# nipponjo/tts-arabic-pytorch

Hardware: AMD Instinct MI355X
Metric: audio samples/sec (FastPitch+HiFi-GAN, synthetic 64-phoneme inputs) (higher is better)
Workload: dtype f32

## Files before the change

include/ttsamd.h:

```cpp
#ifndef TTSAMD_H
#define TTSAMD_H

#include <stdint.h>

#ifdef __cplusplus
extern "C" {
#endif

#define TTSAMD_OK 0
#define TTSAMD_EINVAL (-1)
#define TTSAMD_EHIP (-2)
#define TTSAMD_ENOMEM (-3)

typedef struct ttsamd_tensor {
    const char* name;
    const float* data;
    int32_t ndim;
    int64_t shape[4];
} ttsamd_tensor;

typedef struct ttsamd_hifigan_cfg {
    int32_t num_mels;
    int32_t upsample_initial_channel;
    int32_t n_ups;
// ... 121 lines not shown
                       int32_t batch, int32_t n_max, const float* bias_spec, float strength,
                       void* workspace, int64_t workspace_bytes, void* stream);
int32_t ttsamd_denoise_rows(void* handle, float* wave, int64_t wave_stride, const int64_t* nsamples,
                            int32_t batch, int32_t n_max, const float* bias_spec, const float* strength_rows,
                            void* workspace, int64_t workspace_bytes, void* stream);

int32_t ttsamd_vocos_create(const ttsamd_tensor* weights, int32_t n_weights, int32_t input_channels,
                            int32_t dim, int32_t intermediate_dim, int32_t num_layers, void** handle);
int32_t ttsamd_vocos_destroy(void* handle);
int64_t ttsamd_vocos_workspace_bytes(void* handle, int32_t batch, int32_t t_max);
int32_t ttsamd_vocos_bias_vec(void* handle, float* bias_vec, void* workspace, int64_t workspace_bytes,
                              void* stream);
int32_t ttsamd_vocos_forward(void* handle, const float* mel, const int64_t* lens, int32_t batch,
                             int32_t t_max, float denoise, const float* bias_vec, float* wave,
                             void* workspace, int64_t workspace_bytes, void* stream);
int32_t ttsamd_vocos_forward_rows(void* handle, const float* mel, const int64_t* lens, int32_t batch,
                                  int32_t t_max, const float* denoise_rows, const float* bias_vec, float* wave,
                                  void* workspace, int64_t workspace_bytes, void* stream);

int32_t ttsamd_vocos_set_padding(void* handle, int32_t mode);

int32_t ttsamd_melspec_create(const float* fbank, int32_t n_mels, int32_t n_fft, int32_t hop_length, int32_t framing,
                              int32_t mag_mode, float log_clip, void** handle);
int32_t ttsamd_melspec_destroy(void* handle);
int32_t ttsamd_melspec_forward(void* handle, const float* wave, int64_t wave_stride, const int64_t* nsamples, int32_t batch,
                               int32_t t_max, float* mel, int64_t* frames_out, void* stream);

#define TTSAMD_OVERSMOOTH_MAX_FRAMES 4096
int32_t ttsamd_cepstral_series(const float* mel, const int64_t* lens, int32_t batch, int32_t n_mels, int32_t t_max, int32_t center,
                               int32_t hann, int32_t q_c, float hqer_scale, float* power, float* series, void* stream);
int32_t ttsamd_cepstral_series_from_power(const float* power, const int64_t* lens, int32_t batch, int32_t n_q, int32_t t_max, int32_t q_c,
                                          int32_t q1, int32_t q2, double eps, double roll_p, float hqer_scale, float* series,
                                          void* stream);
int32_t ttsamd_series_summary(const float* series, const int64_t* lens, int32_t batch, int32_t n_series, int32_t t_max, float* stats,
                              float* feat, void* stream);
int64_t ttsamd_dtw_workspace_bytes(int32_t batch, int32_t ta_max, int32_t tb_max, int32_t channels);
int32_t ttsamd_dtw(const float* a, const int64_t* lens_a, const float* b, const int64_t* lens_b, int32_t batch, int32_t channels,
                   int32_t ta_max, int32_t tb_max, int32_t metric, int32_t window, float* cost, int32_t* path, int32_t* path_len,
                   void* workspace, int64_t workspace_bytes, void* stream);
int32_t ttsamd_dtw_aligned_mae(const float* pred, const float* ref, int32_t batch, int32_t ta_max, int32_t tb_max, const int32_t* path,
                               const int32_t* path_len, float* mae, void* stream);

int32_t ttsamd_mel_cepstrum(const float* logmel, const int64_t* lens, int32_t batch, int32_t n_mels, int32_t t_max, int32_t n_coef, float* cep,
                            void* stream);
#define TTSAMD_EVAL_STATS 8
int32_t ttsamd_dtw_aligned_eval(const float* cep_a, const float* cep_b, int32_t n_coef, int32_t first_coef, const float* mel_a,
                                const float* mel_b, int32_t n_mels, const float* f0_a, const float* f0_b, int32_t batch, int32_t ta_max,
                                int32_t tb_max, const int32_t* path, const int32_t* path_len, double scale, double* stats, void* stream);

#define TTSAMD_MAS_MAX_TOKENS 1024
typedef struct ttsamd_aligner_cfg {
    int32_t n_mel;
    int32_t d_text;
    int32_t n_att;
    int32_t n_symbols;
    int32_t padding_idx;
} ttsamd_aligner_cfg;
int32_t ttsamd_aligner_create(const ttsamd_tensor* weights, int32_t n_weights, const ttsamd_aligner_cfg* cfg, void** handle);
int32_t ttsamd_aligner_destroy(void* handle);
int64_t ttsamd_aligner_workspace_bytes(void* handle, int32_t batch, int32_t n_tokens, int32_t n_frames);
int32_t ttsamd_aligner_forward(void* handle, const int64_t* ids, const int64_t* in_lens, const float* mel, const int64_t* mel_lens,
                               const float* attn_prior, int32_t batch, int32_t n_tokens, int32_t n_frames, float* attn_soft,
                               float* attn_logprob, void* workspace, int64_t workspace_bytes, void* stream);
int64_t ttsamd_mas_workspace_bytes(int32_t batch, int32_t n_frames, int32_t n_tokens);
int32_t ttsamd_mas(const float* attn, int32_t is_log, const int64_t* in_lens, const int64_t* out_lens, int32_t batch, int32_t n_frames,
                   int32_t n_tokens, float* dur, float* attn_hard, void* workspace, int64_t workspace_bytes, void* stream);
int32_t ttsamd_average_pitch(const float* pitch, const float* dur, int32_t batch, int32_t n_formants, int32_t n_frames, int32_t n_tokens,
                             float* out, void* stream);

#define TTSAMD_ATTN_PRIOR_F64 2
int32_t ttsamd_attn_prior(const int64_t* in_lens, const int64_t* mel_lens, int32_t batch, int32_t n_tokens, int32_t n_frames, int32_t mode,
                          double scaling, void* out, void* stream);
int32_t ttsamd_attn_prior_tables(int32_t n, double* lf);
int64_t ttsamd_attn_ctc_loss_workspace_bytes(int32_t batch, int32_t n_frames, int32_t n_tokens);
int32_t ttsamd_attn_ctc_loss(const float* attn_logprob, const int64_t* in_lens, const int64_t* out_lens, int32_t batch, int32_t n_frames,
                             int32_t n_tokens, double blank_logprob, double* nll, void* workspace, int64_t workspace_bytes, void* stream);
int32_t ttsamd_attn_bin_loss(const float* attn_hard, const float* attn_soft, int32_t batch, int32_t n_frames, int32_t n_tokens, double eps,
                             double* sum_log, double* count, void* stream);

#define TTSAMD_PYIN_MAX_FRAMES 8192
typedef struct ttsamd_pyin_cfg {
    int32_t sample_rate;
    int32_t frame_length;
    int32_t win_length;
    int32_t hop_length;
    double fmin, fmax;
    int32_t n_thresholds;
    int32_t beta_a, beta_b;
    double boltzmann;
    double resolution;
    double max_transition_rate;
    double switch_prob;
    double no_trough_prob;
    int32_t pad_mode;
} ttsamd_pyin_cfg;
int32_t ttsamd_pyin_tables(const ttsamd_pyin_cfg* cfg, int32_t* dims, double* beta, double* expn, double* norm, double* trans,
                           float* logtrans, float* f0);
int32_t ttsamd_pyin_create(const ttsamd_pyin_cfg* cfg, void** handle);
int32_t ttsamd_pyin_destroy(void* handle);
int64_t ttsamd_pyin_workspace_bytes(void* handle, int32_t batch, int32_t n_frames);
int32_t ttsamd_pyin_forward(void* handle, const float* wave, int64_t wave_stride, const int64_t* nsamples, int32_t batch, int32_t t_max,
                            float* f0, uint8_t* voiced_flag, double* voiced_prob, int32_t* states, int64_t* frames_out,
                            void* workspace, int64_t workspace_bytes, void* stream);
int32_t ttsamd_pyin_obs_offsets(void* handle, int32_t batch, int32_t n_frames, int64_t* obs_offsets);

int32_t ttsamd_resample_create(const float* taps, int32_t o, int32_t n, int32_t width, void** handle);
int32_t ttsamd_resample_destroy(void* handle);
int64_t ttsamd_resample_out_len(void* handle, int64_t nsamples);
int32_t ttsamd_resample_mfma_eligible(void* handle);
int32_t ttsamd_resample_forward(void* handle, const float* wave, int64_t wave_stride, const int64_t* nsamples, int32_t batch, float* out,
                                int64_t out_stride, int64_t* nout, int32_t route, void* stream);

int64_t ttsamd_trim_workspace_bytes(int32_t batch, int64_t wave_stride, int32_t hop_length);
int32_t ttsamd_trim_bounds(const float* wave, int64_t wave_stride, const int64_t* nsamples, int32_t batch, float top_db,
                           int32_t frame_length, int32_t hop_length, float gain, int64_t* bounds, float* peak, void* workspace,
                           int64_t workspace_bytes, void* stream);
int32_t ttsamd_trim_apply(const float* wave, int64_t wave_stride, const int64_t* bounds, const float* peak, float gain, int64_t tail,
                          int32_t batch, float* out, int64_t out_stride, int64_t* lens_out, void* stream);
int32_t ttsamd_frames_compact(const float* mel, const float* extra, const int64_t* lens, int32_t batch, int32_t n_channels,
                              int32_t n_extra, int32_t t_max, float thresh, float* mel_out, float* extra_out, int64_t* lens_out,
                              void* stream);

int32_t ttsamd_tacotron2_create(const ttsamd_tensor* weights, int32_t n_weights,
                                const ttsamd_tacotron2_cfg* cfg, void** handle);
int32_t ttsamd_tacotron2_destroy(void* handle);
int64_t ttsamd_tacotron2_workspace_bytes(void* handle, int32_t batch, int32_t n_tokens, int32_t max_step);
int32_t ttsamd_tacotron2_infer(void* handle, const int64_t* tokens, const int64_t* lengths,
                               const int64_t* speaker_ids, int32_t batch, int32_t n_tokens, int32_t max_step,
                               int64_t dropout_seed, float* mel_post, int32_t* mel_lens, float* alignments,
                               float* mel_raw, int32_t* n_steps, void* workspace, int64_t workspace_bytes,
                               void* stream);

int32_t ttsamd_tagger_create(const ttsamd_tensor* weights, int32_t n_weights, const ttsamd_tagger_cfg* cfg,
                             void** handle);
int32_t ttsamd_tagger_destroy(void* handle);
int64_t ttsamd_tagger_workspace_bytes(void* handle, int32_t batch, int32_t n_chars);
int32_t ttsamd_tagger_forward(void* handle, const int64_t* ids, int32_t batch, int32_t n_chars, float* probs,
                              void* workspace, int64_t workspace_bytes, void* stream);


int64_t ttsamd_conv1d_packed_floats(int32_t cout, int32_t cin, int32_t k);
int32_t ttsamd_conv1d(const float* x, const float* w, const float* bias, const int64_t* lens,
                      int32_t batch, int32_t cin, int32_t cout, int32_t k, int32_t dilation,
                      int32_t lin, float in_slope, int32_t relu_out, float* y, float* packed,
                      void* stream);
int32_t ttsamd_conv1d_ex(const float* x, const float* w, const float* bias, const float* res, const int64_t* lens, int32_t batch,
                         int32_t cin, int32_t cout, int32_t k, int32_t dilation, int32_t lin, float in_slope,
                         int32_t relu_out, int32_t mode, float div, float* y, float* packed, void* stream);
int32_t ttsamd_conv1d_splitk(const float* x, const float* w, const float* bias, const float* res, const int64_t* lens, int32_t batch,
                             int32_t cin, int32_t cout, int32_t k, int32_t dilation, int32_t lin, float in_slope,
                             int32_t relu_out, int32_t mode, float div, float* y, float* packed, float* splitk_ws, int64_t splitk_floats,
                             void* stream);
int32_t ttsamd_conv_last_launch(int32_t* route, int32_t* ksplit);
int64_t ttsamd_convt_packed_floats(int32_t cin, int32_t cout, int32_t u);
int32_t ttsamd_conv_transpose1d(const float* x, const float* w, const float* bias, const int64_t* lens, int32_t batch, int32_t cin,
                                int32_t cout, int32_t u, int32_t lin, float in_slope, float* y, float* packed, void* stream);

int64_t ttsamd_resblock_pair_packed_floats(int32_t channels, int32_t k, int32_t variant);
int32_t ttsamd_resblock_pair(const float* x, float* y, const float* w1, const float* b1, const float* w2, const float* b2,
                             int32_t channels, int32_t k, int32_t dil, const int64_t* lens, int32_t len_mul, int32_t L,
                             int32_t batch, int32_t mode, float div, float slope, int32_t variant, float* packed, int64_t packed_floats,
                             void* stream);

int64_t ttsamd_resblock2_packed_floats(int32_t channels, int32_t k, int32_t variant);
int32_t ttsamd_resblock2(const float* x, float* y, const float* w1, const float* b1, const float* w2, const float* b2, int32_t channels,
                         int32_t k, int32_t dil1, int32_t dil2, const int64_t* lens, int32_t len_mul, int32_t L, int32_t batch, int32_t mode,
                         float div, float slope, int32_t variant, float* packed, int64_t packed_floats, void* stream);

int32_t ttsamd_bfo_pack(const float* x, int32_t batch, int32_t channels, int32_t len, float slope, void* out, void* stream);
int32_t ttsamd_bfo_unpack(const void* in, int32_t batch, int32_t channels, int32_t len, float slope, float* out, void* stream);
int64_t ttsamd_bfo_weight_elems(int32_t cout, int32_t cin, int32_t k, int32_t up);
int32_t ttsamd_bfo_pack_weight(const float* w, int32_t cout, int32_t cin, int32_t k, int32_t up, uint16_t* out);
int32_t ttsamd_bfo_conv1d(const void* x, const void* w_packed, const float* bias, const void* res, const void* sum_in,
                          const int64_t* lens, int32_t len_mul, int32_t batch, int32_t cin, int32_t cout, int32_t k,
                          int32_t dilation, int32_t up, int32_t len_in, int32_t mode, float div, float res_slope,
                          float out_slope, void* y, float* y_f32, const float* res_f32, void* stream);
int32_t ttsamd_bfo_resblock_pair(const void* x, const void* w1, const float* b1, const void* w2, const float* b2,
                                 const void* sum_in, const int64_t* lens, int32_t len_mul, int32_t batch, int32_t channels,
                                 int32_t k, int32_t dilation, int32_t len, int32_t mode, float div, float in_slope,
                                 float mid_slope, float out_slope, void* y, void* stream);
int32_t ttsamd_bfo_resblock_chain(const void* x, const void* const* w1, const float* const* b1, const void* const* w2,
                                  const float* const* b2, const int32_t* dilations, const void* sum_in, const int64_t* lens,
                                  int32_t len_mul, int32_t batch, int32_t channels, int32_t len, int32_t mode, float div,
                                  float in_slope, float mid_slope, float out_slope, void* y, void* stream, int32_t k);
int32_t ttsamd_bfo_conv_post(const void* x, const float* w, const float* bias, const int64_t* lens, int32_t len_mul,
                             int32_t batch, int32_t channels, int32_t len, float* wave, int64_t wave_stride, void* stream);

int32_t ttsamd_bfo3_pack(const float* x, int32_t batch, int32_t channels, int32_t len, float slope, void* out, void* stream);
int32_t ttsamd_bfo3_unpack(const void* in, int32_t batch, int32_t channels, int32_t len, float slope, float* out, void* stream);
int64_t ttsamd_bfo3_weight_elems(int32_t cout, int32_t cin, int32_t k, int32_t up);
int32_t ttsamd_bfo3_pack_weight(const float* w, int32_t cout, int32_t cin, int32_t k, int32_t up, uint16_t* out);
int32_t ttsamd_bfo3_conv1d(const void* x, const void* w_packed, const float* bias, const void* res, const void* sum_in,
                           const int64_t* lens, int32_t len_mul, int32_t batch, int32_t cin, int32_t cout, int32_t k,
                           int32_t dilation, int32_t up, int32_t len_in, int32_t mode, float div, float res_slope,
                           float out_slope, void* y, float* y_f32, const float* res_f32, void* stream);
int32_t ttsamd_bfo3_resblock_pair(const void* x, const void* w1, const float* b1, const void* w2, const float* b2,
                                  const void* sum_in, const int64_t* lens, int32_t len_mul, int32_t batch, int32_t channels,
                                  int32_t k, int32_t dilation, int32_t len, int32_t mode, float div, float in_slope,
                                  float mid_slope, float out_slope, void* y, void* stream);
int32_t ttsamd_bfo3_resblock_chain(const void* x, const void* const* w1, const float* const* b1, const void* const* w2,
                                   const float* const* b2, const int32_t* dilations, const void* sum_in, const int64_t* lens,
                                   int32_t len_mul, int32_t batch, int32_t channels, int32_t len, int32_t mode, float div,
                                   float in_slope, float mid_slope, float out_slope, void* y, void* stream);
int32_t ttsamd_bfo3_conv_post(const void* x, const float* w, const float* bias, const int64_t* lens, int32_t len_mul,
                              int32_t batch, int32_t channels, int32_t len, float* wave, int64_t wave_stride, void* stream);

int32_t ttsamd_set_precision(int32_t precision);
int32_t ttsamd_get_precision(void);

#define TTSAMD_DP_ID_BYTES 128
#define TTSAMD_DP_HIFIGAN 0
#define TTSAMD_DP_FASTPITCH 1
int32_t ttsamd_dp_unique_id(void* id128 );
int32_t ttsamd_dp_init(int32_t rank, int32_t world, const void* id128 , void** comm);
int32_t ttsamd_dp_destroy(void* comm);
int32_t ttsamd_dp_rank(void* comm);
int32_t ttsamd_dp_world(void* comm);
int32_t ttsamd_dp_broadcast(void* comm, void* buf, int64_t nbytes, int32_t root, void* stream);
int32_t ttsamd_dp_broadcast_weights(void* comm, int32_t kind, void* handle, int32_t root, void* stream);
int32_t ttsamd_dp_allgather(void* comm, const void* send, void* recv, int64_t nbytes_per_rank, void* stream);
int32_t ttsamd_dp_pack_audio(const float* wave, int64_t wave_stride, const int64_t* nsamples, int32_t batch,
                             int64_t n_max, float* packed, void* stream);
int32_t ttsamd_dp_gather_audio(void* comm, const float* packed, float* recv, const int64_t* counts,
                               const int64_t* offsets, int32_t root, void* stream);

int32_t ttsamd_hifigan_halo_frames(void* handle, int32_t* left , int32_t* right );
int32_t ttsamd_denoiser_halo_frames(void);
#define TTSAMD_STREAM_MAX_WINDOWS 64
int32_t ttsamd_stream_gather(const float* pool, int32_t n_slots, int32_t num_mels, int32_t t_cap, const int32_t* slot ,
                             const int32_t* start , const int32_t* len , int32_t n_windows, int32_t w_max,
                             float* batch, int64_t* lens, void* stream);
int32_t ttsamd_stream_emit(const float* wave, int32_t n_windows, int32_t w_max, int32_t hop, const int32_t* core_off ,
                           const int32_t* core_len , int32_t c_max, int32_t format, void* out, void* stream);
int32_t ttsamd_stream_emit_resampled(void* resample_handle, const float* wave, int32_t n_windows, int32_t w_max, int32_t hop,
                                     const int32_t* win_start , const int32_t* win_len ,
                                     const int32_t* utt_len , const int32_t* core_start ,
                                     const int32_t* core_end , int32_t c_max, int32_t format, void* out,
                                     int32_t* nout , void* stream);
int32_t ttsamd_vocos_halo_frames(void* handle, int32_t* left , int32_t* right );
int32_t ttsamd_vocos_forward_windows(void* handle, const float* mel, const int64_t* lens, int32_t n_windows, int32_t w_max,
                                     const int32_t* need_start , const int32_t* need_len ,
                                     const float* denoise_rows , const float* bias_vec, float* wave,
                                     void* workspace, int64_t workspace_bytes, void* stream);
int32_t ttsamd_wave_encode(const float* wave, int64_t wave_stride, const int64_t* nsamples, int32_t batch, int32_t format, void* out,
                           int64_t out_stride, void* stream);

int32_t ttsamd_loudness_coefficients(int32_t sample_rate, double* out);
int64_t ttsamd_loudness_workspace_bytes(int32_t batch, int64_t wave_stride, int32_t sample_rate);
int32_t ttsamd_loudness_measure(const float* wave, int64_t wave_stride, const int64_t* nsamples, int32_t batch, int32_t sample_rate,
                                double* loudness, float* peak, void* workspace, int64_t workspace_bytes, void* stream);
int32_t ttsamd_wave_level(float* wave, int64_t wave_stride, const int64_t* nsamples, int32_t batch, const int32_t* mode,
                          const float* target, float ceiling, const double* loudness, const float* peak, float* gain_out, void* stream);

int32_t ttsamd_profile_enable(int32_t on);
int32_t ttsamd_profile_read(double* out3);

#ifdef __cplusplus
}
#endif
#endif
```

profiles/launch_classes.py:

```python
import csv
import re
import sys
from collections import defaultdict


def classes(path):
    d = defaultdict(lambda: [0, 0])
    other = 0
    with open(path) as f:
        for r in csv.DictReader(f):
            dur = int(r['End_Timestamp']) - int(r['Start_Timestamp'])
            m = re.search(r'conv1d_wino4_f32<(\d+), (\d+), (\d+), (\d+), (\d+), (\d+)>', r['Kernel_Name'])
            if not m:
                other += dur
                continue
            k, noct, nst, epi, lp, pt = map(int, m.groups())
            key = (pt, k, lp, 'residual' if epi == 3 else 'plain', int(r['Grid_Size_X']) // int(r['Workgroup_Size_X']))
            d[key][0] += 1
            d[key][1] += dur
    return d, other


a, oa = classes(sys.argv[1])
b, ob = classes(sys.argv[2])
print(f'{"groups":>6} {"k":>3} {"window":>7} {"epilogue":>9} {"blocks":>7} {"calls":>6} {"us parent":>10} {"us tree":>9} {"ratio":>6}')
ta = tb = 0
for key in sorted(set(a) | set(b), key=lambda t: (-t[0], t[1], t[2], t[3], t[4])):
    ca, da = a.get(key, (0, 0))
    cb, db = b.get(key, (0, 0))
    ta += da
    tb += db
    ua, ub = (da / ca / 1e3 if ca else float('nan')), (db / cb / 1e3 if cb else float('nan'))
    print(f'{"seven" if key[0] == 7 else "six":>6} {key[1]:3d} {"vector" if key[2] == 1 else "strip":>7} {key[3]:>9} {key[4]:7d} {max(ca, cb):6d} '
          f'{ua:10.1f} {ub:9.1f} {ub / ua:6.3f}')
print(f'sum over the conv1d_wino4_f32 launches: {ta / 1e6:.2f} -> {tb / 1e6:.2f} ms; every other kernel: {oa / 1e6:.2f} -> {ob / 1e6:.2f} ms (whole trace)')
```

tts-arabic-pytorch_amd/csrc/api.hip:

```cpp
#include <cerrno>
#include <cstdio>
#include <cstdlib>
#include <cstring>
#include <algorithm>
#include <atomic>
#include <mutex>
#include <string>
#include <vector>

#include "kernels.hpp"

namespace ttsamd {

static thread_local std::string g_err;

void set_error(const char* fmt, ...) {
    char buf[1024];
    va_list ap;
    va_start(ap, fmt);
    vsnprintf(buf, sizeof(buf), fmt, ap);
    va_end(ap);
    g_err = buf;
}

// ... 49 lines not shown
struct Vocos;
int32_t vocos_create(const ttsamd_tensor*, int32_t, int32_t, int32_t, int32_t, int32_t, Vocos**);
void vocos_destroy(Vocos*);
int64_t vocos_workspace_bytes(const Vocos*, int32_t, int32_t);
int64_t vocos_bias_workspace_bytes(const Vocos*);
int32_t vocos_bias_vec(const Vocos*, float*, void*, int64_t, hipStream_t);
int32_t vocos_forward(const Vocos*, const float*, const int64_t*, int32_t, int32_t, float, const float*, const float*, float*, void*,
                      int64_t, hipStream_t);
int32_t vocos_set_padding(Vocos*, int32_t);
int32_t vocos_halo_frames(const Vocos*, int32_t*, int32_t*);
int32_t vocos_forward_windows(const Vocos*, const float*, const int64_t*, int32_t, int32_t, const int32_t*, const int32_t*, const float*,
                              const float*, float*, void*, int64_t, hipStream_t);
struct MelSpec;
int32_t melspec_create(const float*, int32_t, int32_t, int32_t, int32_t, int32_t, float, MelSpec**);
void melspec_destroy(MelSpec*);
int32_t melspec_forward(const MelSpec*, const float*, int64_t, const int64_t*, int32_t, int32_t, float*, int64_t*, hipStream_t);
int32_t cepstral_series(const float*, const int64_t*, int32_t, int32_t, int32_t, int32_t, int32_t, int32_t, float, float*, float*, hipStream_t);
int32_t cepstral_series_from_power(const float*, const int64_t*, int32_t, int32_t, int32_t, int32_t, int32_t, int32_t, double, double, float,
                                   float*, hipStream_t);
int32_t series_summary(const float*, const int64_t*, int32_t, int32_t, int32_t, float*, float*, hipStream_t);
int64_t dtw_workspace_bytes(int32_t, int32_t, int32_t, int32_t);
int32_t dtw(const float*, const int64_t*, const float*, const int64_t*, int32_t, int32_t, int32_t, int32_t, int32_t, int32_t, float*,
            int32_t*, int32_t*, void*, int64_t, hipStream_t);
int32_t dtw_aligned_mae(const float*, const float*, int32_t, int32_t, int32_t, const int32_t*, const int32_t*, float*, hipStream_t);
int32_t mel_cepstrum(const float*, const int64_t*, int32_t, int32_t, int32_t, int32_t, float*, hipStream_t);
int32_t dtw_aligned_eval(const float*, const float*, int32_t, int32_t, const float*, const float*, int32_t, const float*, const float*, int32_t,
                         int32_t, int32_t, const int32_t*, const int32_t*, double, double*, hipStream_t);
struct Aligner;
int32_t aligner_create(const ttsamd_tensor*, int32_t, const ttsamd_aligner_cfg*, Aligner**);
void aligner_destroy(Aligner*);
int64_t aligner_workspace_bytes(const Aligner*, int32_t, int32_t, int32_t);
int32_t aligner_forward(const Aligner*, const int64_t*, const int64_t*, const float*, const int64_t*, const float*, int32_t, int32_t, int32_t,
                        float*, float*, void*, int64_t, hipStream_t);
int64_t mas_workspace_bytes(int32_t, int32_t, int32_t);
int32_t mas(const float*, int32_t, const int64_t*, const int64_t*, int32_t, int32_t, int32_t, float*, float*, void*, int64_t, hipStream_t);
int32_t average_pitch(const float*, const float*, int32_t, int32_t, int32_t, int32_t, float*, hipStream_t);
int32_t attn_prior(const int64_t*, const int64_t*, int32_t, int32_t, int32_t, int32_t, double, void*, hipStream_t);
int32_t attn_prior_tables_host(int32_t, double*);
int64_t attn_ctc_workspace_bytes(int32_t, int32_t, int32_t);
int32_t attn_ctc_loss(const float*, const int64_t*, const int64_t*, int32_t, int32_t, int32_t, double, double*, void*, int64_t, hipStream_t);
int32_t attn_bin_loss(const float*, const float*, int32_t, int32_t, int32_t, double, double*, double*, hipStream_t);
struct Pyin;
int32_t pyin_tables_host(const ttsamd_pyin_cfg*, int32_t*, double*, double*, double*, double*, float*, float*);
int32_t pyin_create(const ttsamd_pyin_cfg*, Pyin**);
void pyin_destroy(Pyin*);
int64_t pyin_workspace_bytes(const Pyin*, int32_t, int32_t);
int32_t pyin_obs_offsets(const Pyin*, int32_t, int32_t, int64_t*);
int32_t pyin_forward(const Pyin*, const float*, int64_t, const int64_t*, int32_t, int32_t, float*, uint8_t*, double*, int32_t*, int64_t*, void*,
                     int64_t, hipStream_t);
struct Taco2;
int32_t tacotron2_create(const ttsamd_tensor*, int32_t, const ttsamd_tacotron2_cfg*, Taco2**);
void tacotron2_destroy(Taco2*);
int64_t tacotron2_workspace_bytes(const Taco2*, int32_t, int32_t, int32_t);
int32_t tacotron2_infer(const Taco2*, const int64_t*, const int64_t*, const int64_t*, int32_t, int32_t, int32_t, int64_t,
                        float*, int32_t*, float*, float*, int32_t*, void*, int64_t, hipStream_t);
struct Tagger;
int32_t tagger_create(const ttsamd_tensor*, int32_t, const ttsamd_tagger_cfg*, Tagger**);
void tagger_destroy(Tagger*);
int64_t tagger_workspace_bytes(const Tagger*, int32_t, int32_t);
int32_t tagger_forward(const Tagger*, const int64_t*, int32_t, int32_t, float*, void*, int64_t, hipStream_t);
int32_t denoiser_create(Denoiser**);
void denoiser_destroy(Denoiser*);
int64_t denoiser_workspace_bytes(int32_t, int32_t);
int32_t denoiser_bias_spec(const Denoiser*, const float*, const int64_t*, int32_t, float*, void*, int64_t, hipStream_t);
int32_t denoise(const Denoiser*, float*, int64_t, const int64_t*, int32_t, int32_t, const float*, float, const float*, void*, int64_t,
                hipStream_t);
int32_t hifigan_halo_frames(const HifiGan*, int32_t*, int32_t*);
int32_t stream_gather(const float*, int32_t, int32_t, int32_t, const int32_t*, const int32_t*, const int32_t*, int32_t, int32_t, float*,
                      int64_t*, hipStream_t);
int32_t stream_emit(const float*, int32_t, int32_t, int32_t, const int32_t*, const int32_t*, int32_t, int32_t, void*, hipStream_t);
int32_t stream_emit_resampled(const Resample*, const float*, int32_t, int32_t, int32_t, const int32_t*, const int32_t*, const int32_t*,
                              const int32_t*, const int32_t*, int32_t, int32_t, void*, int32_t*, hipStream_t);
int32_t wave_encode(const float*, int64_t, const int64_t*, int32_t, int32_t, void*, int64_t, hipStream_t);
int32_t hifigan_create(const ttsamd_tensor*, int32_t, const ttsamd_hifigan_cfg*, HifiGan**);
void hifigan_destroy(HifiGan*);
int64_t hifigan_workspace_bytes(const HifiGan*, int32_t, int32_t);
int32_t hifigan_forward(const HifiGan*, const float*, const int64_t*, int32_t, int32_t, float*, void*, int64_t,
                        hipStream_t);
int32_t fastpitch_create(const ttsamd_tensor*, int32_t, const ttsamd_fastpitch_cfg*, int32_t, FastPitch**);
void fastpitch_destroy(FastPitch*);
int64_t fastpitch_encode_workspace_bytes(const FastPitch*, int32_t, int32_t);
int64_t fastpitch_decode_workspace_bytes(const FastPitch*, int32_t, int32_t);
int32_t fastpitch_encode(const FastPitch*, const int64_t*, int32_t, int32_t, int32_t, float, const float*,
                         const float*, const float*, float, float, float, float*, float*, float*, float*, int64_t*,
                         int64_t*, void*, int64_t, hipStream_t);
void fastpitch_set_batch_mode(const FastPitch*, int);
int32_t fastpitch_decode(const FastPitch*, float*, const int64_t*, int32_t, int32_t, float*, void*, int64_t,
                         hipStream_t);
int32_t fastpitch_encode_rows(const FastPitch*, const int64_t*, int32_t, int32_t, int32_t, float, const float*,
                              const float*, const float*, float, float, float, float*, float*, float*, float*, int64_t*,
                              int64_t*, void*, int64_t, const int32_t*, const float*, const float*, const float*, int32_t, hipStream_t);
int32_t fastpitch_decode_rows(const FastPitch*, float*, const int64_t*, int32_t, int32_t, float*, void*, int64_t, int32_t,
                              hipStream_t);

__global__ void pack_conv_weight_kernel(const float* __restrict__ w, int cout, int cin, int k, int cp,
                                        float* __restrict__ out) {
    const int64_t i = (int64_t)blockIdx.x * 256 + threadIdx.x;
    const int64_t n = (int64_t)cin * k * cp;
    if (i >= n) return;
    const int pq = (int)(i % 4);
    const int co = (int)((i / 4) % cp);
    const int kk = (int)((i / (4 * (int64_t)cp)) % 2);
    const int t = (int)((i / (8 * (int64_t)cp)) % k);
    const int o = (int)(i / (8 * (int64_t)cp * k));
    out[i] = co < cout ? w[((int64_t)co * cin + (8 * o + 2 * pq + kk)) * k + t] : 0.f;
}

__global__ void pack_convt_weight_kernel(const float* __restrict__ w, int cin, int cout, int u, int cp, float* __restrict__ out) {
    const int64_t i = (int64_t)blockIdx.x * 256 + threadIdx.x;
    const int64_t n = (int64_t)u * cin * 2 * cp;
    if (i >= n) return;
    const int pq = (int)(i % 4);
    const int co = (int)((i / 4) % cp);
    const int kk = (int)((i / (4 * (int64_t)cp)) % 2);
    const int t = (int)((i / (8 * (int64_t)cp)) % 2);
    const int o = (int)((i / (16 * (int64_t)cp)) % (cin / 8));
    const int rho = (int)(i / (16 * (int64_t)cp * (cin / 8)));
    const int kidx = (rho + u / 2) % u + t * u;
    out[i] = co < cout ? w[((int64_t)(8 * o + 2 * pq + kk) * cout + co) * (2 * u) + kidx] : 0.f;
}

__global__ void split_bf16_kernel(const float* __restrict__ packed, int64_t n, unsigned short* __restrict__ out) {
    const int64_t i = (int64_t)blockIdx.x * 256 + threadIdx.x;
    if (i >= n) return;
    const float f = packed[i];
    unsigned u = __float_as_uint(f);
    u += 0x7fffu + ((u >> 16) & 1u);
    const unsigned h = u >> 16;
    const float r = f - __uint_as_float(h << 16);
    unsigned v = __float_as_uint(r);
    v += 0x7fffu + ((v >> 16) & 1u);
    out[i] = (unsigned short)h;
    out[n + i] = (unsigned short)(v >> 16);
}

namespace {
struct OptDesc { const char* name; int kind; long long lo, hi; };
const OptDesc kOpts[OPT_COUNT] = {
#define TTS_OPT_DESC(name, kind, lo, hi) {"TTSAMD_" #name, kind, lo, hi},
    TTS_OPTIONS(TTS_OPT_DESC)
#undef TTS_OPT_DESC
};
std::atomic<const char*> g_opt[OPT_COUNT];
std::once_flag g_opt_once;
std::string g_opt_env_error;

bool opt_valid(const OptDesc& d, const char* v) {
    if (!v || !*v) return false;
    char* end = nullptr;
    errno = 0;
    const long long x = std::strtoll(v, &end, d.kind == 1 ? 16 : 10);
    if (!(errno == 0 && end != v && *end == '\0' && x >= d.lo && x <= d.hi)) return false;
    if (&d == &kOpts[OPT_WINO4] && (((x & 32) && !(x & 2)) || ((x & 64) && !(x & 4)))) return false;
    return true;
}
void opt_init() {
    std::call_once(g_opt_once, [] {
        for (int i = 0; i < OPT_COUNT; ++i) {
            const char* e = std::getenv(kOpts[i].name);
            if (!e || !*e) continue;
            if (!opt_valid(kOpts[i], e)) {
                if (g_opt_env_error.empty()) {
                    char buf[256];
                    std::snprintf(buf, sizeof buf, "%s='%s' in the environment is not a valid value (%s in [%llx, %llx])", kOpts[i].name, e,
                                  kOpts[i].kind == 1 ? "hex mask" : "integer", kOpts[i].lo, kOpts[i].hi);
                    g_opt_env_error = buf;
                }
                continue;
            }
            g_opt[i].store(strdup(e), std::memory_order_release);
        }
    });
}
int opt_find(const char* name) {
    if (!name) return -1;
    for (int i = 0; i < OPT_COUNT; ++i)
        if (std::strcmp(name, kOpts[i].name) == 0 || std::strcmp(name, kOpts[i].name + 7) == 0) return i;
    return -1;
}
}

int64_t opt_int(Opt o, int64_t unset) {
    opt_init();
    const char* v = g_opt[o].load(std::memory_order_acquire);
    return v ? (int64_t)std::strtoll(v, nullptr, kOpts[o].kind == 1 ? 16 : 10) : unset;
}

}

using namespace ttsamd;

extern "C" {

const char* ttsamd_last_error(void) { return g_err.c_str(); }
int32_t ttsamd_version(void) { return TTSAMD_ABI_VERSION; }

int32_t ttsamd_set_option(const char* name, const char* value) {
    opt_init();
    const int i = opt_find(name);
    TTS_REQUIRE(i >= 0, "set_option: unknown option '%s' (ttsamd_option_name lists them)", name ? name : "(null)");
    if (!value || !*value) {
        g_opt[i].store(nullptr, std::memory_order_release);
        return 0;
    }
    TTS_REQUIRE(opt_valid(kOpts[i], value), "set_option: %s='%s' is not a valid value (%s in [%llx, %llx])", kOpts[i].name, value,
                kOpts[i].kind == 1 ? "hex mask" : "integer", kOpts[i].lo, kOpts[i].hi);
    g_opt[i].store(strdup(value), std::memory_order_release);
    return 0;
}
int32_t ttsamd_get_option(const char* name, char* value, int32_t capacity) {
    opt_init();
    const int i = opt_find(name);
    TTS_REQUIRE(i >= 0 && value && capacity > 0, "get_option: unknown option '%s' or no buffer", name ? name : "(null)");
    const char* v = g_opt[i].load(std::memory_order_acquire);
    std::snprintf(value, (size_t)capacity, "%s", v ? v : "");
    return 0;
}
const char* ttsamd_option_name(int32_t index) { return (index >= 0 && index < OPT_COUNT) ? kOpts[index].name : nullptr; }
int32_t ttsamd_options_check(void) {
    opt_init();
    TTS_REQUIRE(g_opt_env_error.empty(), "%s", g_opt_env_error.c_str());
    return 0;
}

int32_t ttsamd_device_ok(void) {
    int n = 0;
    if (hipGetDeviceCount(&n) != hipSuccess || n <= 0) return 0;
    hipDeviceProp_t prop;
    if (hipGetDeviceProperties(&prop, 0) != hipSuccess) return 0;
    return std::string(prop.gcnArchName).rfind("gfx950", 0) == 0 ? 1 : 0;
}

int32_t ttsamd_hifigan_create(const ttsamd_tensor* weights, int32_t n, const ttsamd_hifigan_cfg* cfg, void** handle) {
    HifiGan* h = nullptr;
    const int32_t rc = hifigan_create(weights, n, cfg, &h);
    if (rc == 0) *handle = h;
    return rc;
}
int32_t ttsamd_hifigan_destroy(void* handle) {
    hifigan_destroy((HifiGan*)handle);
    return 0;
}
int64_t ttsamd_hifigan_workspace_bytes(void* handle, int32_t batch, int32_t t_max) {
    if (!handle || batch < 1 || t_max < 1) return 0;
    return hifigan_workspace_bytes((HifiGan*)handle, batch, t_max);
}
int32_t ttsamd_hifigan_forward(void* handle, const float* mel, const int64_t* lens, int32_t batch, int32_t t_max,
                               float* wave, void* workspace, int64_t workspace_bytes, void* stream) {
    return hifigan_forward((HifiGan*)handle, mel, lens, batch, t_max, wave, workspace, workspace_bytes,
                           (hipStream_t)stream);
}

int32_t ttsamd_hifigan_halo_frames(void* handle, int32_t* left, int32_t* right) {
    return hifigan_halo_frames((HifiGan*)handle, left, right);
}
int32_t ttsamd_denoiser_halo_frames(void) { return 3; }
int32_t ttsamd_stream_gather(const float* pool, int32_t n_slots, int32_t num_mels, int32_t t_cap, const int32_t* slot, const int32_t* start,
                             const int32_t* len, int32_t n_windows, int32_t w_max, float* batch, int64_t* lens, void* stream) {
    return stream_gather(pool, n_slots, num_mels, t_cap, slot, start, len, n_windows, w_max, batch, lens, (hipStream_t)stream);
}
int32_t ttsamd_stream_emit(const float* wave, int32_t n_windows, int32_t w_max, int32_t hop, const int32_t* core_off, const int32_t* core_len,
                           int32_t c_max, int32_t format, void* out, void* stream) {
    return stream_emit(wave, n_windows, w_max, hop, core_off, core_len, c_max, format, out, (hipStream_t)stream);
}
int32_t ttsamd_stream_emit_resampled(void* resample_handle, const float* wave, int32_t n_windows, int32_t w_max, int32_t hop,
                                     const int32_t* win_start, const int32_t* win_len, const int32_t* utt_len, const int32_t* core_start,
                                     const int32_t* core_end, int32_t c_max, int32_t format, void* out, int32_t* nout, void* stream) {
    return stream_emit_resampled((const Resample*)resample_handle, wave, n_windows, w_max, hop, win_start, win_len, utt_len, core_start,
                                 core_end, c_max, format, out, nout, (hipStream_t)stream);
}
int32_t ttsamd_wave_encode(const float* wave, int64_t wave_stride, const int64_t* nsamples, int32_t batch, int32_t format, void* out,
                           int64_t out_stride, void* stream) {
    return wave_encode(wave, wave_stride, nsamples, batch, format, out, out_stride, (hipStream_t)stream);
}

int32_t ttsamd_fastpitch_create(const ttsamd_tensor* weights, int32_t n, const ttsamd_fastpitch_cfg* cfg,
                                void** handle) {
    FastPitch* h = nullptr;
    const int32_t rc = fastpitch_create(weights, n, cfg, 16384, &h);
    if (rc == 0) *handle = h;
    return rc;
}
int32_t ttsamd_fastpitch_destroy(void* handle) {
    fastpitch_destroy((FastPitch*)handle);
    return 0;
}
int64_t ttsamd_fastpitch_encode_workspace_bytes(void* handle, int32_t batch, int32_t n_tokens) {
    if (!handle || batch < 1 || n_tokens < 1) return 0;
    return fastpitch_encode_workspace_bytes((FastPitch*)handle, batch, n_tokens);
}
int64_t ttsamd_fastpitch_decode_workspace_bytes(void* handle, int32_t batch, int32_t t_max) {
    if (!handle || batch < 1 || t_max < 1) return 0;
    return fastpitch_decode_workspace_bytes((FastPitch*)handle, batch, t_max);
}
int32_t ttsamd_fastpitch_encode(void* handle, const int64_t* ids, int32_t batch, int32_t n_tokens, int32_t speaker,
                                float pace, const float* dur_tgt, const float* pitch_tgt, const float* energy_tgt,
                                float pitch_mul, float pitch_add, float max_duration, float* enc_cond,
                                float* dur_pred, float* pitch_pred, float* energy_pred, int64_t* reps,
                                int64_t* dec_lens, void* workspace, int64_t workspace_bytes, void* stream) {
    return fastpitch_encode((FastPitch*)handle, ids, batch, n_tokens, speaker, pace, dur_tgt, pitch_tgt, energy_tgt,
                            pitch_mul, pitch_add, max_duration, enc_cond, dur_pred, pitch_pred, energy_pred, reps,
                            dec_lens, workspace, workspace_bytes, (hipStream_t)stream);
}
int32_t ttsamd_length_regulate(const float* enc, const int64_t* reps, int32_t batch, int32_t n_tokens,
                               int32_t channels, int32_t t_max, float* out, int32_t* idx, void* stream) {
    TTS_REQUIRE(enc && reps && out && batch >= 1 && n_tokens >= 1 && channels >= 1 && t_max >= 0,
// ... 325 lines not shown
    const int ng = k == 3 ? 6 : (k == 7 ? 16 : 24), nsf = k == 3 ? 1 : (k == 7 ? 2 : 4);
    const int64_t i = (int64_t)blockIdx.x * 256 + threadIdx.x;
    const int64_t n = (int64_t)cin * ng * cp;
    if (i >= n) return;
    const int pq = (int)(i & 3);
    const int64_t r = i >> 2;
    const int co = (int)(r % cp);
    const int64_t r2 = r / cp;
    const int kk = (int)(r2 & 1);
    const int64_t r3 = r2 >> 1;
    const int t = (int)(r3 % ng), o = (int)(r3 / ng);
    float v = 0.f;
    if (co < cout) {
        const float* g = w + ((int64_t)co * cin + (8 * o + 2 * pq + kk)) * k;
        if (t < 6 * nsf) {
            const int s = t / 6, j = t % 6;
            const double g0 = g[3 * s], g1 = 3 * s + 1 < k ? g[3 * s + 1] : 0.0, g2 = 3 * s + 2 < k ? g[3 * s + 2] : 0.0;
            v = j == 0 ? (float)(g0 / 4) : (j == 1 ? (float)(-(g0 + g1 + g2) / 6) : (j == 2 ? (float)(-(g0 - g1 + g2) / 6) :
                (j == 3 ? (float)(g0 / 24 + g1 / 12 + g2 / 6) : (j == 4 ? (float)(g0 / 24 - g1 / 12 + g2 / 6) : (float)g2))));
        } else {
            v = g[6];
        }
    }
    out[i] = v;
}

__global__ void pack_wino44_weight_kernel(const float* __restrict__ w, int cout, int cin, int k, int cp, float* __restrict__ out) {
    const int ng = k == 7 ? 13 : 20;
    const int64_t i = (int64_t)blockIdx.x * 256 + threadIdx.x;
    const int64_t n = (int64_t)cin * ng * cp;
    if (i >= n) return;
    const int pq = (int)(i & 3);
    const int64_t r = i >> 2;
    const int co = (int)(r % cp);
    const int64_t r2 = r / cp;
    const int kk = (int)(r2 & 1);
    const int64_t r3 = r2 >> 1;
    const int t = (int)(r3 % ng), o = (int)(r3 / ng);
    float v = 0.f;
    if (co < cout) {
        const float* g = w + ((int64_t)co * cin + (8 * o + 2 * pq + kk)) * k;
        const int s = t / 7, j = t % 7;
        const double g0 = g[4 * s], g1 = g[4 * s + 1], g2 = g[4 * s + 2], g3 = 4 * s + 3 < k ? g[4 * s + 3] : 0.0;
        v = j == 0 ? (float)(g0 / 4) : (j == 1 ? (float)((g0 + g1 + g2 + g3) / 6) : (j == 2 ? (float)((g0 - g1 + g2 - g3) / 18) :
            (j == 3 ? (float)((g0 + 2 * g1 + 4 * g2 + 8 * g3) / 72) : (j == 4 ? (float)((g0 - 2 * g1 + 4 * g2 - 8 * g3) / 120) :
            (j == 5 ? (float)((32 * g0 + 16 * g1 + 8 * g2 + 4 * g3) / 45) : (float)(g3 / 2))))));
    }
    out[i] = v;
}

__global__ void pack_wino2_weight_kernel(const float* __restrict__ w, int cout, int cin, int k, int cp, float* __restrict__ out) {
    const int ns = k / 3, ng = 4 * ns + 2 * (k - 3 * ns);
    const int64_t i = (int64_t)blockIdx.x * 256 + threadIdx.x;
    const int64_t n = (int64_t)cin * ng * cp;
    if (i >= n) return;
    const int pq = (int)(i & 3);
    const int64_t r = i >> 2;
    const int co = (int)(r % cp);
    const int64_t r2 = r / cp;
    const int kk = (int)(r2 & 1);
    const int64_t r3 = r2 >> 1;
    const int t = (int)(r3 % ng), o = (int)(r3 / ng);
    float v = 0.f;
    if (co < cout) {
        const float* g = w + ((int64_t)co * cin + (8 * o + 2 * pq + kk)) * k;
        if (t < 4 * ns) {
            const int s = t >> 2, j = t & 3;
            const double g0 = g[3 * s], g1 = g[3 * s + 1], g2 = g[3 * s + 2];
            v = j == 0 ? (float)g0 : (j == 1 ? (float)((g0 + g1 + g2) * 0.5) : (j == 2 ? (float)((g0 - g1 + g2) * 0.5) : (float)g2));
        } else {
            const int l = (t - 4 * ns) >> 1;
            v = ((t - 4 * ns) & 1) ? -g[3 * ns + l] : g[3 * ns + l];
        }
    }
    out[i] = v;
}

int32_t ttsamd_conv1d_ex(const float* x, const float* w, const float* bias, const float* res, const int64_t* lens, int32_t batch,
                         int32_t cin, int32_t cout, int32_t k, int32_t dilation, int32_t lin, float in_slope,
                         int32_t relu_out, int32_t mode, float div, float* y, float* packed, void* stream) {
    return ttsamd_conv1d_splitk(x, w, bias, res, lens, batch, cin, cout, k, dilation, lin, in_slope, relu_out, mode, div, y, packed, nullptr,
                                0, stream);
}

int32_t ttsamd_conv1d_splitk(const float* x, const float* w, const float* bias, const float* res, const int64_t* lens, int32_t batch,
                             int32_t cin, int32_t cout, int32_t k, int32_t dilation, int32_t lin, float in_slope,
                             int32_t relu_out, int32_t mode, float div, float* y, float* packed, float* splitk_ws, int64_t splitk_floats,
                             void* stream) {
    TTS_REQUIRE(x && w && y && packed, "conv1d: null argument");
    TTS_REQUIRE(splitk_floats >= 0 && (splitk_ws != nullptr || splitk_floats == 0), "conv1d: %lld split-K floats without a workspace",
                (long long)splitk_floats);
    TTS_REQUIRE(mode >= 0 && mode <= 2 && (mode != 2 || div != 0.f), "conv1d: bad mode / div");
    TTS_REQUIRE(relu_out == 0 || mode == 0, "conv1d: relu_out with an accumulate mode (mode %d) is not defined", mode);
    hipStream_t s = (hipStream_t)stream;
    const int cp = cout_padded(cout);
    const int64_t n = (int64_t)cin * k * cp;
    hipLaunchKernelGGL(pack_conv_weight_kernel, dim3((unsigned)((n + 255) / 256)), dim3(256), 0, s, w, cout, cin, k,
                       cp, packed);
    TTS_CHECK_HIP(hipGetLastError());
    ConvParams p;
    std::memset(&p, 0, sizeof(p));
    p.x = x; p.x_bs = (int64_t)cin * lin; p.x_cs = lin;
    p.w = packed; p.bias = bias;
    p.precision = default_precision();
    if (p.precision != 0) {
        unsigned short* planes = reinterpret_cast<unsigned short*>(packed + n);
        hipLaunchKernelGGL(split_bf16_kernel, dim3((unsigned)((n + 255) / 256)), dim3(256), 0, s, packed, n, planes);
        TTS_CHECK_HIP(hipGetLastError());
        p.w_bf16 = planes;
    }
    if ((k == 3 || k == 7 || k == 11) && p.precision == 0 && cin % 8 == 0) {
        float* wino = packed + 2 * n;
        const int64_t nw = (int64_t)cin * wino2_groups(k) * cp;
        hipLaunchKernelGGL(pack_wino2_weight_kernel, dim3((unsigned)((nw + 255) / 256)), dim3(256), 0, s, w, cout, cin, k, cp, wino);
        TTS_CHECK_HIP(hipGetLastError());
        p.w_wino = wino;
        float* wino4 = wino + nw;
        const int64_t nw4 = (int64_t)cin * wino4_groups(k) * cp;
        hipLaunchKernelGGL(pack_wino4_weight_kernel, dim3((unsigned)((nw4 + 255) / 256)), dim3(256), 0, s, w, cout, cin, k, cp, wino4);
        TTS_CHECK_HIP(hipGetLastError());
        p.w_wino4 = wino4;
        if (wino44_groups(k) != 0) {
            float* wino44 = wino4 + nw4;
            const int64_t nw44 = (int64_t)cin * wino44_groups(k) * cp;
            hipLaunchKernelGGL(pack_wino44_weight_kernel, dim3((unsigned)((nw44 + 255) / 256)), dim3(256), 0, s, w, cout, cin, k, cp, wino44);
            TTS_CHECK_HIP(hipGetLastError());
            p.w_wino44 = wino44;
        }
    }
    p.y = y; p.y_bs = (int64_t)cout * lin; p.y_cs = lin; p.y_ts = 1;
    p.lens_in = lens; p.lens_out = lens; p.len_in_mul = 1; p.len_out_mul = 1;
    p.Lin = lin; p.Nout = lin; p.Cin = cin; p.Cout = cout; p.CoutP = cp; p.K = k;
    p.dil = dilation; p.pad = (k * dilation - dilation) / 2;
    p.res = res; p.r_bs = (int64_t)cout * lin; p.r_cs = lin;
    p.n_phase = 1; p.in_slope = in_slope; p.relu_out = relu_out; p.mode = mode; p.div = div; p.batch = batch;
    if (splitk_ws != nullptr && splitk_floats > 0) { p.splitk_ws = splitk_ws; p.splitk_floats = splitk_floats; }
    prof_begin(s, 2.0 * cout * cin * k);
    const int32_t rc = launch_conv(p, s);
    prof_end(s);
    return rc;
}

int32_t ttsamd_conv1d(const float* x, const float* w, const float* bias, const int64_t* lens, int32_t batch,
                      int32_t cin, int32_t cout, int32_t k, int32_t dilation, int32_t lin, float in_slope,
                      int32_t relu_out, float* y, float* packed, void* stream) {
    return ttsamd_conv1d_ex(x, w, bias, nullptr, lens, batch, cin, cout, k, dilation, lin, in_slope, relu_out, 0, 1.f, y, packed, stream);
}

int32_t ttsamd_conv_last_launch(int32_t* route, int32_t* ksplit) {
    TTS_REQUIRE(route && ksplit, "conv_last_launch: null argument");
    last_conv_launch(route, ksplit);
    return 0;
}

int64_t ttsamd_convt_packed_floats(int32_t cin, int32_t cout, int32_t u) {
    if (cin < 1 || cout < 1 || u < 1) return 0;
    return 2 * (int64_t)u * cin * 2 * cout_padded(cout);
}

int32_t ttsamd_conv_transpose1d(const float* x, const float* w, const float* bias, const int64_t* lens, int32_t batch, int32_t cin,
                                int32_t cout, int32_t u, int32_t lin, float in_slope, float* y, float* packed, void* stream) {
    TTS_REQUIRE(x && w && y && packed, "conv_transpose1d: null argument");
    TTS_REQUIRE(batch >= 1 && cin >= 8 && cin % 8 == 0 && cout >= 1 && lin >= 1, "conv_transpose1d: batch %d, cin %d (a multiple of 8), cout %d, lin %d",
                batch, cin, cout, lin);
    TTS_REQUIRE(u >= 2 && u % 2 == 0, "conv_transpose1d: stride %d (kernel 2 u, padding u / 2: u even)", u);
    TTS_REQUIRE((int64_t)lin * u < ((int64_t)1 << 31) / 4 / cout, "conv_transpose1d: %d x %d x %d outputs per row", cout, lin, u);
    hipStream_t s = (hipStream_t)stream;
    const int cp = cout_padded(cout);
    const int64_t n = (int64_t)u * cin * 2 * cp;
    hipLaunchKernelGGL(pack_convt_weight_kernel, dim3((unsigned)((n + 255) / 256)), dim3(256), 0, s, w, cin, cout, u, cp, packed);
    TTS_CHECK_HIP(hipGetLastError());
    unsigned short* planes = nullptr;
    if (default_precision() != 0) {
        planes = reinterpret_cast<unsigned short*>(packed + n);
        hipLaunchKernelGGL(split_bf16_kernel, dim3((unsigned)((n + 255) / 256)), dim3(256), 0, s, packed, n, planes);
        TTS_CHECK_HIP(hipGetLastError());
    }
    ConvParams p;
    std::memset(&p, 0, sizeof(p));
    p.batch = batch;
    p.lens_in = lens; p.lens_out = lens;
    prof_begin(s, 2.0 * cout * cin * 2 * u);
    const int32_t rc = launch_upsampler(p, x, packed, planes, bias, y, cin, cout, u, 2 * u, lin, 1, in_slope, opt_int(OPT_CONVT, 1) != 0, s);
    prof_end(s);
    return rc;
}

int64_t ttsamd_resblock_pair_packed_floats(int32_t channels, int32_t k, int32_t variant) {
    if (channels < 1 || k < 1) return 0;
    const int64_t n = 2 * (int64_t)channels * k * channels;
    const int nwino = (variant == 4 ? 1 : (variant == 5 ? 2 : 0));
    if (variant == 6) return n + ((k == 3 || k == 7 || k == 11) ? 2 * (int64_t)channels * wino4_groups(k) * channels : 0);
    return n + ((k == 3 || k == 7 || k == 11) ? nwino * (int64_t)channels * wino2_groups(k) * channels : 0);
}

int32_t ttsamd_resblock_pair(const float* x, float* y, const float* w1, const float* b1, const float* w2, const float* b2,
                             int32_t channels, int32_t k, int32_t dil, const int64_t* lens, int32_t len_mul, int32_t L,
                             int32_t batch, int32_t mode, float div, float slope, int32_t variant, float* packed, int64_t packed_floats,
                             void* stream) {
    TTS_REQUIRE(x && y && w1 && b1 && w2 && b2 && packed && channels % 32 == 0 && k >= 1 && batch >= 1 && L >= 1 && len_mul >= 1 &&
                mode >= 0 && mode <= 2, "resblock_pair: bad argument");
    TTS_REQUIRE(packed_floats >= ttsamd_resblock_pair_packed_floats(channels, k, variant),
                "resblock_pair: `packed` holds %lld floats, variant %d at C = %d, k = %d needs %lld (ttsamd_resblock_pair_packed_floats)",
                (long long)packed_floats, variant, channels, k, (long long)ttsamd_resblock_pair_packed_floats(channels, k, variant));
    hipStream_t s = (hipStream_t)stream;
    const int64_t n = (int64_t)channels * k * channels;
    for (int i = 0; i < 2; ++i) {
        hipLaunchKernelGGL(pack_conv_weight_kernel, dim3((unsigned)((n + 255) / 256)), dim3(256), 0, s, i == 0 ? w1 : w2, channels,
                           channels, k, channels, packed + i * n);
        TTS_CHECK_HIP(hipGetLastError());
    }
    const double fl = 2.0 * (2.0 * channels * channels * k);
    int32_t rc;
    prof_begin(s, fl);
    if (variant == 1) {
        rc = launch_fused_pair(channels, x, y, packed, b1, packed + n, b2, k, dil, lens, len_mul, L, batch, mode, div, slope, s);
    } else if (variant >= 2 && variant <= 5) {
        const float *w2w = nullptr, *w1w = nullptr;
        if (variant >= 4) {
            TTS_REQUIRE((k == 3 || k == 7 || k == 11) && (channels <= 64 || (variant == 5 && channels == 128)),
                        "resblock_pair: variants 4 / 5 are built for C = 32 / 64 (5: and 128), k = 3 / 7 / 11");
            const int64_t nw = (int64_t)channels * wino2_groups(k) * channels;
            for (int i = 0; i < (variant == 5 ? 2 : 1); ++i) {
                float* wino = packed + 2 * n + i * nw;
                hipLaunchKernelGGL(pack_wino2_weight_kernel, dim3((unsigned)((nw + 255) / 256)), dim3(256), 0, s, i == 0 ? w2 : w1, channels,
                                   channels, k, channels, wino);
                TTS_CHECK_HIP(hipGetLastError());
                (i == 0 ? w2w : w1w) = wino;
            }
        }
        rc = launch_fused_pair2(channels, x, y, packed, b1, packed + n, b2, k, dil, lens, len_mul, L, batch, mode, div, slope,
                                variant == 3 ? 1 : 2, s, w2w, w1w);
    } else if (variant == 6) {
        TTS_REQUIRE(channels == 32 && (k == 3 || k == 7 || k == 11), "resblock_pair: variant 6 is built for C = 32, k = 3 / 7 / 11");
        const int64_t nw4 = (int64_t)channels * wino4_groups(k) * channels;
        for (int i = 0; i < 2; ++i) {
            hipLaunchKernelGGL(pack_wino4_weight_kernel, dim3((unsigned)((nw4 + 255) / 256)), dim3(256), 0, s, i == 0 ? w1 : w2, channels,
                               channels, k, channels, packed + 2 * n + i * nw4);
            TTS_CHECK_HIP(hipGetLastError());
        }
        rc = launch_fused_pair4(channels, x, y, packed + 2 * n, b1, packed + 2 * n + nw4, b2, k, dil, lens, len_mul, L, batch, mode, div,
                                slope, s);
    } else if (variant == -1) {
        rc = 0;
    } else {
        set_error("resblock_pair: variant %d (1: first generation, 2 / 3: second generation with 256- / 128-column blocks, 4 / 5: 256 columns + Winograd phase B / both phases, 6: C = 32 with both phases on Winograd F(4,3))", variant);
        rc = TTSAMD_EINVAL;
    }
    prof_end(s);
    return rc;
}

int64_t ttsamd_resblock2_packed_floats(int32_t channels, int32_t k, int32_t variant) {
    if (channels < 1 || k < 1 || (variant != 1 && variant != 2)) return 0;
    return 2 * (int64_t)channels * k * channels;
}

int32_t ttsamd_resblock2(const float* x, float* y, const float* w1, const float* b1, const float* w2, const float* b2, int32_t channels,
                         int32_t k, int32_t dil1, int32_t dil2, const int64_t* lens, int32_t len_mul, int32_t L, int32_t batch, int32_t mode,
                         float div, float slope, int32_t variant, float* packed, int64_t packed_floats, void* stream) {
    TTS_REQUIRE(x && y && w1 && b1 && w2 && b2 && packed && channels % 32 == 0 && channels >= 32 && k >= 1 && batch >= 1 && L >= 1 &&
                len_mul >= 1 && mode >= 0 && mode <= 2 && x != y, "resblock2: bad argument");
    TTS_REQUIRE(variant == 1 || variant == 2, "resblock2: variant %d (1: two single-conv launches, 2: both convs in one launch)", variant);
    TTS_REQUIRE(packed_floats >= ttsamd_resblock2_packed_floats(channels, k, variant),
                "resblock2: `packed` holds %lld floats, C = %d, k = %d needs %lld (ttsamd_resblock2_packed_floats)", (long long)packed_floats,
                channels, k, (long long)ttsamd_resblock2_packed_floats(channels, k, variant));
    if (variant == 1) {
        TTS_REQUIRE(resblock2_conv_supported(channels, k, dil1, L, x, y) && resblock2_conv_supported(channels, k, dil2, L, x, y),
                    "resblock2: variant 1 does not cover C = %d, k = %d, dilations %d / %d (C = 32 / 64 / 128, k = 3 / 5 / 7 / 11, "
                    "dilation 1..16)", channels, k, dil1, dil2);
    } else {
        TTS_REQUIRE(resblock2_pair_supported(channels, k, dil1, dil2, L, x, y),
                    "resblock2: variant 2 does not cover C = %d, k = %d, dilations %d / %d (C = 32 / 64, k = 3 / 5 / 7 / 11, dilation "
                    "1..16, (k - 1) * dil2 <= 256)", channels, k, dil1, dil2);
    }
    hipStream_t s = (hipStream_t)stream;
    const int64_t n = (int64_t)channels * k * channels;
    for (int i = 0; i < 2; ++i) {
        hipLaunchKernelGGL(pack_conv_weight_kernel, dim3((unsigned)((n + 255) / 256)), dim3(256), 0, s, i == 0 ? w1 : w2, channels,
                           channels, k, channels, packed + i * n);
        TTS_CHECK_HIP(hipGetLastError());
    }
    prof_begin(s, 2.0 * (2.0 * channels * channels * k));
    int32_t rc;
    if (variant == 2) {
        rc = launch_resblock2_pair(channels, x, y, packed, b1, packed + n, b2, k, dil1, dil2, lens, len_mul, L, batch, mode, div, slope, s);
    } else {
        float* x1 = nullptr;
        TTS_CHECK_HIP(hipMallocAsync((void**)&x1, (size_t)batch * channels * L * sizeof(float), s));
        rc = launch_resblock2_conv(channels, x, x1, packed, b1, k, dil1, lens, len_mul, L, batch, 0, 1.f, slope, s);
        if (rc == 0) rc = launch_resblock2_conv(channels, x1, y, packed + n, b2, k, dil2, lens, len_mul, L, batch, mode, div, slope, s);
        const hipError_t e = hipFreeAsync(x1, s);
        if (rc == 0 && e != hipSuccess) {
            set_error("resblock2: hipFreeAsync failed: %s", hipGetErrorString(e));
            rc = TTSAMD_EHIP;
        }
    }
    prof_end(s);
    return rc;
}

int32_t ttsamd_set_precision(int32_t precision) {
    TTS_REQUIRE(precision >= 0 && precision <= 2, "set_precision: 0 = fp32 MFMA, 1 = bf16 MFMA, 2 = split-bf16 MFMA");
    g_precision = precision;
    return 0;
}
// ... 43 lines not shown
```

tts-arabic-pytorch_amd/csrc/common.hpp:

```cpp
#pragma once
#include <hip/hip_runtime.h>
#include <stdint.h>
#include <atomic>
#include <cstdarg>
#include <cstdio>
#include <cstdlib>
#include <string>

#include "../../include/ttsamd.h"

namespace ttsamd {

void set_error(const char* fmt, ...);

#define TTS_CHECK_HIP(expr)                                                         \
    do {                                                                            \
        hipError_t e_ = (expr);                                                     \
        if (e_ != hipSuccess) {                                                     \
            ttsamd::set_error("%s failed: %s (%s:%d)", #expr, hipGetErrorString(e_), \
                              __FILE__, __LINE__);                                  \
            return TTSAMD_EHIP;                                                     \
        }                                                                           \
    } while (0)

#define TTS_REQUIRE(cond, ...)              \
    do {                                    \
        if (!(cond)) {                      \
            ttsamd::set_error(__VA_ARGS__); \
            return TTSAMD_EINVAL;           \
        }                                   \
    } while (0)

#define TTS_TRY(expr)               \
    do {                            \
        int32_t rc_ = (expr);       \
        if (rc_ != 0) return rc_;   \
    } while (0)

inline int64_t align_up(int64_t x, int64_t a) { return (x + a - 1) / a * a; }

inline hipError_t lds_opt_in(const void* fn, int bytes, std::atomic<uint64_t>& done) {
    int dev = 0;
    hipError_t e = hipGetDevice(&dev);
    if (e != hipSuccess) return e;
    if (dev >= 0 && dev < 64 && ((done.load(std::memory_order_acquire) >> dev) & 1)) return hipSuccess;
    e = hipFuncSetAttribute(fn, hipFuncAttributeMaxDynamicSharedMemorySize, bytes);
    if (e == hipSuccess && dev >= 0 && dev < 64) done.fetch_or(1ull << dev, std::memory_order_release);
    return e;
}

#define TTS_OPTIONS(X)                                                                                     \
    X(HIFIGAN_STREAMS, 0, 0, 1)    \
    X(WINO, 0, 0, 1)                                              \
    X(WINO2, 0, 0, 31)             \
    X(WINO4, 0, 0, 127)            \
    X(FUSED_PAIR, 0, 0, 1)                   \
    X(FUSED2, 0, 0, 1)                                           \
    X(FUSED2_MASK, 1, 0, 0x1ff)               \
    X(FUSED2_MASK_N1, 1, 0, 0x1ff)          \
    X(FUSED2_WB, 0, 0, 2)                     \
    X(PAIR4, 0, 0, 1)              \
    X(CONVT, 0, 0, 1)                              \
    X(BFO, 0, 0, 1)                \
    X(BFO_CHAIN, 0, 0, 1)                           \
    X(BFO_CHAIN7, 0, 0, 1)                                 \
    X(BFO_FF, 0, 0, 1)                              \
    X(BFO_SPLITK, 0, 0, 1)                                              \
    X(BFO_SMALL_TILES, 0, 0, 1)            \
    X(BF16_ATTN, 0, 0, 1)                                         \
    X(BF16_PACKED_T, 0, 0, 1)                   \
    X(ATT_RA, 0, 1, 4)                             \
    X(ATT_SPLIT, 0, 0, 1)                      \
    X(XCD_W, 0, 0, 1)                            \
    X(XCD_WMAX_KB, 0, 0, 1 << 20)     \
    X(DEEP_SPLITK, 0, 0, 1)        \
    X(TACO_PERSISTENT, 0, 0, 2)    \
    X(TACO_SEG, 0, 8, 1 << 20)     \
    X(RESBLOCK2_PAIR, 1, 0, 0x3f)
enum Opt : int {
#define TTS_OPT_ENUM(name, kind, lo, hi) OPT_##name,
    TTS_OPTIONS(TTS_OPT_ENUM)
#undef TTS_OPT_ENUM
    OPT_COUNT
};
int64_t opt_int(Opt o, int64_t unset);

struct Arena {
    char* base;
    int64_t size;
    int64_t off = 0;
    bool ok = true;
    Arena(void* p, int64_t n) : base((char*)p), size(n) {}
    template <typename T>
    T* take(int64_t count) {
        int64_t bytes = align_up(count * (int64_t)sizeof(T), 256);
        if (base != nullptr && off + bytes > size) ok = false;
        T* r = base ? (T*)(base + off) : nullptr;
        off += bytes;
        return r;
    }
};

struct ConvParams {
    const float* x;
    int64_t x_bs;
    int32_t x_cs;
    const float* w;
    const void* w_bf16;
    const float* w_wino;
    const float* w_wino4;
    int32_t precision;
    const float* bias;
    float* y;
    int64_t y_bs;
    int32_t y_cs, y_ts;
    const float* res;
    int64_t r_bs;
    int32_t r_cs;
    const int64_t* lens_in;
    const int64_t* lens_out;
    int32_t len_in_mul, len_out_mul;
    int32_t Lin, Nout;
    int32_t Cin, Cout, CoutP, K;
    int32_t dil, pad;
    int32_t n_phase;
    int32_t phase_p;
    float in_slope;
    const float* scale;
    int32_t relu_out;
    int32_t mode;
    float div;
    int32_t batch;
    float* splitk_ws;
    int64_t splitk_floats;
    int32_t ksplit;
    int32_t y_packed;
    float pack_slope;
    int32_t x_packed;
    int32_t xcd_w;
    int32_t tile_major;
    int32_t compact;
    unsigned long long* timing;
    const float* w_wino44;
};
constexpr int64_t kSplitKFloats = 4 << 20;
constexpr int64_t kSplitKFloatsFp = 8 << 20;

void conv_log(const char* kind, int K, int cin, int cout, int nout, int batch, int has_res, int mode, int len_mul, int ragged,
              int n_phase);
bool compact_order(const void* lens, int batch);
int32_t launch_conv(const ConvParams& p, hipStream_t stream);
void note_conv_launch(int32_t route, int32_t ksplit);
void last_conv_launch(int32_t* route, int32_t* ksplit);
bool convt_supported(const ConvParams& p);
int32_t launch_convt(const ConvParams& p, hipStream_t stream);
int32_t launch_upsampler(ConvParams& p, const float* x, const float* w, const void* w_bf16, const float* bias, float* y, int cin, int cout,
                         int u, int kt, int L, int len_mul, float in_slope, bool convt_ok, hipStream_t stream);
bool fused_pair_supported(int32_t channels, int32_t k, int32_t dil, int32_t L, const float* x, const float* y);
int32_t launch_fused_pair(int32_t channels, const float* x, float* y, const float* w1, const float* b1, const float* w2,
                          const float* b2, int32_t k, int32_t dil, const int64_t* lens, int32_t len_mul, int32_t L, int32_t batch,
                          int32_t mode, float div, float slope, hipStream_t stream);
bool fused_pair2_supported(int32_t channels, int32_t k, int32_t dil, int32_t L, const float* x, const float* y, int32_t ntw);
int32_t launch_fused_pair2(int32_t channels, const float* x, float* y, const float* w1, const float* b1, const float* w2,
                           const float* b2, int32_t k, int32_t dil, const int64_t* lens, int32_t len_mul, int32_t L, int32_t batch,
                           int32_t mode, float div, float slope, int32_t ntw, hipStream_t stream, const float* w2_wino = nullptr,
                           const float* w1_wino = nullptr);
bool fused_pair4_supported(int32_t channels, int32_t k, int32_t dil, int32_t L, const float* x, const float* y);
int32_t launch_fused_pair4(int32_t channels, const float* x, float* y, const float* w1_wino4, const float* b1, const float* w2_wino4,
                           const float* b2, int32_t k, int32_t dil, const int64_t* lens, int32_t len_mul, int32_t L, int32_t batch,
                           int32_t mode, float div, float slope, hipStream_t stream);
bool resblock2_conv_supported(int32_t channels, int32_t k, int32_t dil, int32_t L, const float* x, const float* y);
int32_t launch_resblock2_conv(int32_t channels, const float* x, float* y, const float* w, const float* b, int32_t k, int32_t dil,
                              const int64_t* lens, int32_t len_mul, int32_t L, int32_t batch, int32_t mode, float div, float slope,
                              hipStream_t stream);
bool resblock2_pair_supported(int32_t channels, int32_t k, int32_t d1, int32_t d2, int32_t L, const float* x, const float* y);
int32_t launch_resblock2_pair(int32_t channels, const float* x, float* y, const float* w1, const float* b1, const float* w2,
                              const float* b2, int32_t k, int32_t d1, int32_t d2, const int64_t* lens, int32_t len_mul, int32_t L,
                              int32_t batch, int32_t mode, float div, float slope, hipStream_t stream);
int wino_route(const ConvParams& p);
int32_t launch_wino(const ConvParams& p, hipStream_t stream);
void pack_wino_weight(const float* w, int cout, int cin, float* out);
int wino2_groups(int k);
int wino2_block_outputs(int coutp, int dil);
int32_t launch_wino2(const ConvParams& p, hipStream_t stream);
void pack_wino2_weight(const float* w, int cout, int cin, int k, float* out);
int wino4_groups(int k);
int wino44_groups(int k);
constexpr int kWino4Default = 127;
bool wino44_wanted(const ConvParams& p);
int wino4_block_outputs(int dil);
int wino4_ksplit(const ConvParams& p);
int32_t launch_splitk_reduce(const ConvParams& q, hipStream_t stream);
int32_t launch_wino4(const ConvParams& p, hipStream_t stream);
void wino4_filter_groups(const float* g, int k, float* o);
void pack_wino4_weight(const float* w, int cout, int cin, int k, float* out);
void wino44_filter_groups(const float* g, int k, float* o);
void pack_wino44_weight(const float* w, int cout, int cin, int k, float* out);
void pack_conv_weight(const float* w, int cout, int cin, int k, float* out);
void pack_convt_weight(const float* w, int cin, int cout, int kt, int u, int p, float* out);
inline int cout_padded(int cout) { return (int)align_up(cout, 32); }
void split_packed_bf16(const float* packed, int64_t n, uint16_t* out);
int32_t default_precision();

#ifdef __HIPCC__
__device__ __forceinline__ bool live_tile(const int64_t* __restrict__ lens, const int mul, const int n_max, const int tile_w,
                                          const int batch, const unsigned lin, int& b, int& tile) {
    const int lane = threadIdx.x & 63;
    unsigned base = 0;
    for (int u0 = 0; u0 < batch; u0 += 64) {
        int n = 0;
        if (u0 + lane < batch) n = (max(min(n_max, (int)lens[u0 + lane] * mul), 0) + tile_w - 1) / tile_w;
        int incl = n;
#pragma unroll
        for (int d = 1; d < 64; d <<= 1) {
            const int t = __shfl_up(incl, d, 64);
            if (lane >= d) incl += t;
        }
        const unsigned total = (unsigned)__shfl(incl, 63, 64);
        if (lin < base + total) {
            const unsigned long long m = __ballot(base + (unsigned)incl > lin);
            const int l = __ffsll((long long)m) - 1;
            b = u0 + l;
            tile = (int)(lin - base) - (__shfl(incl, l, 64) - __shfl(n, l, 64));
            return true;
        }
        base += total;
    }
    return false;
}
#endif

}
```

tts-arabic-pytorch_amd/csrc/conv_mfma.hip:

```cpp
#include <cstdio>
#include <cstdlib>
#include <cstring>

#include <algorithm>

#include "conv_mfma_common.hpp"

namespace ttsamd {



template <int K, int NT_BLK, int CO_BLK>
struct Geo {
    static constexpr int NOCT = (K == 3 && NT_BLK == 128 && CO_BLK == 128) ? 2 : OctsOf<K>::NOCT;
    static constexpr int KC = 8 * NOCT;
    static constexpr int WS = NT_BLK + (K - 1) * DMAX;
    static constexpr int XI = 2 * NOCT * WS;
    static constexpr int NXI = (XI + 255) / 256;
    static constexpr int W4 = NOCT * K * 2 * CO_BLK;
    static constexpr int NW = (W4 + 255) / 256;
    static constexpr int BUF4 = XI + W4;
    static constexpr int NSTAGE = (CO_BLK > 32 && 3 * BUF4 * 16 <= 80 * 1024 && !(K == 7 && CO_BLK == 64 && NT_BLK >= 128)) ? 3 : 2;
    static constexpr int NGRP = NOCT * K;
};
// ... 335 lines not shown
                            if (rp) { const float4 t = *reinterpret_cast<const float4*>(rp); rr4[0] = t.x; rr4[1] = t.y; rr4[2] = t.z; rr4[3] = t.w; }
                            if (mode != 0) { const float4 t = *reinterpret_cast<const float4*>(yp); pp4[0] = t.x; pp4[1] = t.y; pp4[2] = t.z; pp4[3] = t.w; }
                        } else {
#pragma unroll
                            for (int e = 0; e < 4; ++e)
                                if (q + e < n_out) {
                                    if (rp) rr4[e] = rp[e];
                                    if (mode != 0) pp4[e] = yp[e];
                                }
                        }
#pragma unroll
                        for (int e = 0; e < 4; ++e) {
                            float x = v[e] + bsv;
                            if constexpr (EPI == 1) { if (relu_out == 2) x = 0.5f * x * (1.0f + erff(x * 0.70710678118654752440f)); }
                            x = x * scv + rr4[e];
                            if (relu_out == 1) x = fmaxf(x, 0.f);
                            if constexpr (EPI == 1) { if (relu_out == 3) x = tanhf(x); }
                            if (mode == 1) x = pp4[e] + x;
                            else if (mode == 2) x = (pp4[e] + x) / div;
                            v[e] = x;
                        }
                        if (full) {
                            *reinterpret_cast<float4*>(yp) = make_float4(v[0], v[1], v[2], v[3]);
                        } else {
#pragma unroll
                            for (int e = 0; e < 4; ++e)
                                if (q + e < n_out) yp[e] = v[e];
                        }
                    }
                }
                }
            }
            return;
        }
    } else {
    if (!wave_active) return;
    if (p.ksplit > 1) {
        float* __restrict__ pb = p.splitk_ws + ((int64_t)ks * p.batch + b) * p.Cout * p.Nout;
#pragma unroll
        for (int i = 0; i < MT; ++i)
#pragma unroll
            for (int j = 0; j < NTL; ++j) {
                const int q = q0 + qw0 + j * 32 + l31;
#pragma unroll
                for (int r = 0; r < 16; ++r) {
                    const int co = co_w0 + i * 32 + (r & 3) + 8 * (r >> 2) + 4 * kk;
                    if (q < n_out && co < p.Cout) pb[(int64_t)co * p.Nout + q] = acc[i][j][r];
                }
            }
        return;
    }
    float* __restrict__ yb = p.y + (int64_t)b * p.y_bs + phase;
    const float* __restrict__ rb = p.res ? p.res + (int64_t)b * p.r_bs + phase : nullptr;
    const float* __restrict__ bias = p.bias;
    const float* __restrict__ scale = p.scale;
    const int mode = p.mode, relu_out = p.relu_out, Cout = p.Cout;
    const int y_cs = p.y_cs, y_ts = p.y_ts, r_cs = p.r_cs;
    const float div = p.div;
#pragma unroll
    for (int i = 0; i < MT; ++i) {
#pragma unroll
        for (int j = 0; j < NTL; ++j) {
            const int q = q0 + qw0 + j * 32 + l31;
            const bool q_ok = q < n_out;
            const int qc = q_ok ? q : 0;
#pragma unroll
            for (int h = 0; h < 2; ++h) {
                float bv[8], rv[8], pv[8], sv[8];
#pragma unroll
                for (int r8 = 0; r8 < 8; ++r8) {
                    const int r = h * 8 + r8;
                    const int co = co_w0 + i * 32 + (r & 3) + 8 * (r >> 2) + 4 * kk;
                    const int coc = min(co, Cout - 1);
                    bv[r8] = bias ? bias[coc] : 0.f;
                    sv[r8] = scale ? scale[coc] : 1.f;
                    rv[r8] = rb ? rb[(int64_t)coc * r_cs + (int64_t)qc * y_ts] : 0.f;
                    pv[r8] = mode != 0 ? yb[(int64_t)coc * y_cs + (int64_t)qc * y_ts] : 0.f;
                }
#pragma unroll
                for (int r8 = 0; r8 < 8; ++r8) {
                    const int r = h * 8 + r8;
                    const int co = co_w0 + i * 32 + (r & 3) + 8 * (r >> 2) + 4 * kk;
                    float v = acc[i][j][r] + bv[r8];
                    if constexpr (K == 1 || K == 5) { if (relu_out == 2) v = 0.5f * v * (1.0f + erff(v * 0.70710678118654752440f)); }
                    v = v * sv[r8] + rv[r8];
                    if (relu_out == 1) v = fmaxf(v, 0.f);
                    if constexpr (K == 1 || K == 5) { if (relu_out == 3) v = tanhf(v); }
                    if (mode == 1) v = pv[r8] + v;
                    else if (mode == 2) v = (pv[r8] + v) / div;
                    if (q_ok && co < Cout) yb[(int64_t)co * y_cs + (int64_t)q * y_ts] = v;
                }
            }
        }
    }
    }
}

template <int K, int MT, int NTL, int WM, int WN, int EPI>
__global__ __launch_bounds__(256, kConvMinWaves) void conv1d_mfma_f32(const ConvParams p) {
    extern __shared__ __attribute__((aligned(16))) float4 smem4[];
    constexpr int NT_BLK = WN * NTL * 32;
    unsigned bx_ = blockIdx.x, by_ = blockIdx.y, bz_ = blockIdx.z;
    if (p.xcd_w) {
        const unsigned lin = bx_ + gridDim.x * (by_ + gridDim.y * bz_), xcd = lin & 7u, slot = lin >> 3;
        const unsigned nct = gridDim.y, g = (unsigned)p.xcd_w & 0xffu, per = nct / g;
        unsigned rest;
        if (p.xcd_w & 0x100) {
            rest = (slot / per) * (8u / g) + xcd / g;
            by_ = xcd % g + g * (slot % per);
        } else {
            const unsigned idx2 = slot * (8u / g) + xcd / g;
            rest = idx2 / per;
            by_ = xcd % g + g * (idx2 % per);
        }
        bx_ = rest % gridDim.x; bz_ = rest / gridDim.x;
    }
    int b = p.tile_major ? (int)((bx_ + bz_) % (unsigned)p.batch) : (int)bz_;
    int q0 = (p.tile_major ? bz_ : bx_) * NT_BLK;
    if (p.compact) {
        int tile = 0;
        if (!live_tile(p.lens_out, p.len_out_mul, p.Nout, NT_BLK, p.batch, bz_ * gridDim.x + bx_, b, tile)) return;
        b = __builtin_amdgcn_readfirstlane(b);
        q0 = __builtin_amdgcn_readfirstlane(tile) * NT_BLK;
    }
    conv_tile<K, MT, NTL, WM, WN, EPI>(p, smem4, b, q0, by_);
}

__global__ __launch_bounds__(256) void splitk_reduce_kernel(const ConvParams p) {
    const int b = blockIdx.z, co = blockIdx.y, q = blockIdx.x * 256 + threadIdx.x;
    int n_out = p.Nout;
    if (p.lens_out) n_out = min(n_out, (int)p.lens_out[b] * p.len_out_mul);
    if (q >= n_out) return;
    const int64_t per = (int64_t)p.batch * p.Cout * p.Nout;
    const float* __restrict__ pp = p.splitk_ws + ((int64_t)b * p.Cout + co) * p.Nout + q;
    float v = 0.f;
    for (int k0 = 0; k0 < p.ksplit; k0 += 8) {
        float tq[8];
#pragma unroll
        for (int j = 0; j < 8; ++j) tq[j] = pp[(int64_t)min(k0 + j, p.ksplit - 1) * per];
#pragma unroll
        for (int j = 0; j < 8; ++j) v = (k0 + j < p.ksplit) ? v + tq[j] : v;
    }
    v += p.bias ? p.bias[co] : 0.f;
    if (p.relu_out == 2) v = 0.5f * v * (1.0f + erff(v * 0.70710678118654752440f));
    v = v * (p.scale ? p.scale[co] : 1.f) + (p.res ? p.res[(int64_t)b * p.r_bs + (int64_t)co * p.r_cs + q] : 0.f);
    if (p.relu_out == 1) v = fmaxf(v, 0.f);
    else if (p.relu_out == 3) v = tanhf(v);
    float* yp = p.y + (int64_t)b * p.y_bs + (int64_t)co * p.y_cs + q;
    if (p.mode == 1) v = *yp + v;
    else if (p.mode == 2) v = (*yp + v) / p.div;
    *yp = v;
}

static thread_local int32_t t_last_route = -1, t_last_ksplit = 0;
void note_conv_launch(int32_t route, int32_t ksplit) { t_last_route = route; t_last_ksplit = ksplit; }
void last_conv_launch(int32_t* route, int32_t* ksplit) { *route = t_last_route; *ksplit = t_last_ksplit; }

int32_t launch_splitk_reduce(const ConvParams& q, hipStream_t stream) {
    dim3 rg((q.Nout + 255) / 256, q.Cout, q.batch);
    hipLaunchKernelGGL(splitk_reduce_kernel, rg, dim3(256), 0, stream, q);
    TTS_CHECK_HIP(hipGetLastError());
    return 0;
}

template <int K, int MT, int NTL, int WM, int WN, int EPI>
static int32_t launch_epi(const ConvParams& q, dim3 grid, size_t lds, hipStream_t stream) {
    static std::atomic<uint64_t> lds_done{0};
    const auto kern = conv1d_mfma_f32<K, MT, NTL, WM, WN, EPI>;
    TTS_CHECK_HIP(lds_opt_in((const void*)kern, (int)lds, lds_done));
    hipLaunchKernelGGL(kern, grid, dim3(256), lds, stream, q);
    TTS_CHECK_HIP(hipGetLastError());
    return 0;
}

bool compact_order(const void* lens, int batch) { return lens != nullptr && batch > 1; }

constexpr int kXcdWeightKB = 3000;

template <int K, int MT, int NTL, int WM, int WN>
static int32_t launch_cfg(const ConvParams& p, hipStream_t stream) {
    constexpr int CO_BLK = WM * MT * 32, NT_BLK = WN * NTL * 32;
    using G = Geo<K, NT_BLK, CO_BLK>;
    TTS_REQUIRE(p.Cin % G::KC == 0, "conv: Cin=%d must be a multiple of %d for K=%d", p.Cin, G::KC, K);
    const size_t lds = (size_t)G::NSTAGE * G::BUF4 * sizeof(float4);
    dim3 grid((p.Nout + NT_BLK - 1) / NT_BLK, (p.CoutP / CO_BLK) * p.n_phase, p.batch);
    ConvParams q = p;
    q.ksplit = 1;
    q.tile_major = 0;
    q.compact = compact_order(p.lens_out, p.batch) ? 1 : 0;
    {
        const bool xw = opt_int(OPT_XCD_W, 1) != 0;
        const unsigned nct = grid.y;
        const unsigned g = (nct % 8 == 0) ? 8 : (nct % 4 == 0 ? 4 : (nct % 2 == 0 ? 2 : 1));
        const bool can = xw && p.n_phase == 1 && ((int64_t)grid.x * grid.y * grid.z) % 8 == 0;
        q.xcd_w = (can && g > 1) ? (int)g : 0;
        const int64_t wmax = opt_int(OPT_XCD_WMAX_KB, kXcdWeightKB) * 1024;
        if (can && wmax > 0 && nct > 1) {
            const int64_t wbytes = (int64_t)p.CoutP * p.Cin * K * 4;
            unsigned g2 = g;
            while (g2 > 1 && wbytes / (g2 / 2) <= wmax) g2 /= 2;
            if (nct / g2 > 1 && ((int64_t)grid.x * grid.z * g2) % 8 == 0)
                q.xcd_w = (int)g2 | 0x100 | (q.xcd_w << 16);
        }
    }
    const int64_t nblk = (int64_t)grid.x * grid.y * grid.z, per = (int64_t)p.batch * p.Cout * p.Nout;
    const int n_chunks = p.Cin / G::KC;
    constexpr int sk_blocks = 320, sk_target = 640, sk_chunks = 8;
    if (p.splitk_ws && p.n_phase == 1 && p.y_ts == 1 && nblk < sk_blocks && n_chunks >= sk_chunks) {
        int64_t ks = std::min<int64_t>((sk_target + nblk - 1) / nblk, n_chunks / 4);
        ks = std::min<int64_t>(ks, p.splitk_floats / per);
        if (ks >= 2) q.ksplit = (int)ks;
        if (ks >= 2 && (q.xcd_w & 0x100)) q.xcd_w >>= 16;
    }
    if (q.xcd_w & 0x100) q.xcd_w &= 0x1ff;
    grid.y *= q.ksplit;
    note_conv_launch(0, q.ksplit);
    const bool vec_ok = q.ksplit == 1 && p.y_ts == 1 && p.n_phase == 1 && (p.y_cs & 3) == 0 && (p.y_bs & 3) == 0 &&
                        ((uintptr_t)p.y & 15) == 0 &&
                        (!p.res || ((p.r_cs & 3) == 0 && (p.r_bs & 3) == 0 && ((uintptr_t)p.res & 15) == 0));
    TTS_REQUIRE(p.relu_out < 2 || K == 1 || K == 5, "conv: GELU / tanh epilogues are built for kernel sizes 1 and 5 only (K=%d)", K);
    const bool pre_ok = p.res != nullptr && p.scale == nullptr && p.relu_out < 2 &&
                        (int64_t)p.Cout * std::max(p.r_cs, p.y_cs) * 4 < ((int64_t)1 << 31);
    const int epi = !vec_ok ? 2 : (p.relu_out >= 2 ? 1 : (pre_ok ? 3 : 0));
    int32_t rc;
    if (epi == 3) rc = launch_epi<K, MT, NTL, WM, WN, 3>(q, grid, lds, stream);
    else if (epi == 0) rc = launch_epi<K, MT, NTL, WM, WN, 0>(q, grid, lds, stream);
    else if (epi == 1) rc = launch_epi<K, MT, NTL, WM, WN, (K == 1 || K == 5) ? 1 : 2>(q, grid, lds, stream);
    else rc = launch_epi<K, MT, NTL, WM, WN, 2>(q, grid, lds, stream);
    if (rc != 0) return rc;
    if (q.ksplit > 1) return launch_splitk_reduce(q, stream);
    return 0;
}

template <int K>
static int32_t launch_k(const ConvParams& p, hipStream_t stream) {
    auto blocks = [&](int co_blk, int nt_blk) -> int64_t {
        return (int64_t)((p.Nout + nt_blk - 1) / nt_blk) * (p.CoutP / co_blk) * p.n_phase * p.batch;
    };
    const int64_t want = blocks(64, 64) <= 1024 ? (int64_t)200 : (int64_t)768;
    const bool tiny = p.Nout <= 96;
    if (p.CoutP % 128 == 0) {
        const bool few_long = p.Cin >= 256 && p.CoutP <= p.Cin && !tiny && blocks(128, 128) < 4 * want;
        if (few_long && K == 3 && blocks(128, 64) >= want) return launch_cfg<K, 1, 2, 4, 1>(p, stream);
        if (few_long && K >= 7 && blocks(64, 128) >= want) return launch_cfg<K, 1, 2, 2, 2>(p, stream);
        if (K < 11 && !tiny && blocks(128, 128) >= want && (K != 3 || p.Cin % 16 == 0))
            return launch_cfg<K, 2, 2, 2, 2>(p, stream);
        if (K == 11 && !tiny && blocks(64, 256) >= want) return launch_cfg<K, 2, 2, 1, 4>(p, stream);
        if (p.splitk_ws && p.Cin >= 1024 && !tiny && blocks(128, 64) >= 160 && blocks(128, 64) < 320 &&
            (int64_t)2 * p.batch * p.Cout * p.Nout <= p.splitk_floats) {
            if (opt_int(OPT_DEEP_SPLITK, 1) != 0) return launch_cfg<K, 1, 2, 4, 1>(p, stream);
        }
        if (blocks(128, 64) >= want || (tiny && blocks(64, 64) < 2 * want)) return launch_cfg<K, 1, 2, 4, 1>(p, stream);
        return launch_cfg<K, 1, 1, 2, 2>(p, stream);
    }
    if (p.CoutP % 64 == 0) {
        if (!tiny && blocks(64, 256) >= want) return launch_cfg<K, 2, 2, 1, 4>(p, stream);
        return launch_cfg<K, 1, 1, 2, 2>(p, stream);
    }
    if (!tiny && blocks(32, 256) >= want) return launch_cfg<K, 1, 2, 1, 4>(p, stream);
    return launch_cfg<K, 1, 1, 1, 4>(p, stream);
}

void conv_log(const char* kind, int K, int cin, int cout, int nout, int batch, int has_res, int mode, int len_mul, int ragged,
              int n_phase) {
    static FILE* f = [] { const char* e = getenv("TTSAMD_CONV_LOG"); return e ? fopen(e, "a") : (FILE*)nullptr; }();
    if (!f) return;
    fprintf(f, "%s,%d,%d,%d,%d,%d,%d,%d,%d,%d,%d\n", kind, K, cin, cout, nout, batch, has_res, mode, len_mul, ragged, n_phase);
    fflush(f);
}

int32_t launch_conv(const ConvParams& p, hipStream_t stream) {
    TTS_REQUIRE(p.CoutP % 32 == 0 && p.CoutP >= p.Cout, "conv: bad CoutP=%d", p.CoutP);
    TTS_REQUIRE(p.n_phase >= 1 && p.batch >= 1, "conv: bad n_phase/batch");
    TTS_REQUIRE(p.dil >= -DMAX && p.dil <= DMAX && p.dil != 0, "conv: dilation %d outside [-%d,%d]", p.dil, DMAX, DMAX);
    if (p.Nout <= 0) return 0;
    const int wino = wino_route(p);
    conv_log(p.precision == 0 ? (wino == 3 ? "f32_wino4" : (wino ? "f32_wino" : "f32")) : "bf16", p.K, p.Cin, p.Cout, p.Nout, p.batch, p.res != nullptr, p.mode, p.len_out_mul,
             p.lens_out != nullptr, p.n_phase);
    if (p.precision != 0) return launch_conv_bf16_any(p, stream);
    TTS_REQUIRE(!p.x_packed && !p.y_packed, "conv: packed bf16 activations exist only in the bf16 mode");
    if (wino) return wino == 3 ? launch_wino4(p, stream) : (wino == 2 ? launch_wino2(p, stream) : launch_wino(p, stream));
    switch (p.K) {
        case 1: return launch_k<1>(p, stream);
        case 2: return launch_k<2>(p, stream);
        case 3: return launch_k<3>(p, stream);
        case 5: return launch_k<5>(p, stream);
        case 7: return launch_k<7>(p, stream);
        case 11: return launch_k<11>(p, stream);
        default:
            set_error("conv: kernel size %d not instantiated (1,2,3,5,7,11)", p.K);
            return TTSAMD_EINVAL;
    }
}

void pack_conv_weight(const float* w, int cout, int cin, int k, float* out) {
    const int cp = cout_padded(cout);
    for (int o = 0; o < cin / 8; ++o)
        for (int t = 0; t < k; ++t)
            for (int kk = 0; kk < 2; ++kk) {
                float* dst = out + (((int64_t)o * k + t) * 2 + kk) * cp * 4;
                for (int co = 0; co < cp; ++co)
                    for (int pq = 0; pq < 4; ++pq)
                        dst[co * 4 + pq] = co < cout ? w[((int64_t)co * cin + (8 * o + 2 * pq + kk)) * k + t] : 0.f;
            }
}

static inline uint16_t host_bf16_rne(float f) {
    uint32_t u;
    memcpy(&u, &f, 4);
// ... 39 lines not shown
```

tts-arabic-pytorch_amd/csrc/conv_wino4.hip:

```cpp
#include <cstdlib>
#include <cstring>

#include <algorithm>
#include <vector>

#include "conv_mfma_common.hpp"
#include "bfo.hpp"

namespace ttsamd {

typedef float w4_f32x4 __attribute__((ext_vector_type(4)));
typedef float w4_f32x2 __attribute__((ext_vector_type(2)));

template <int K, int NOCT_, int NSTAGE_, int PT_ = 6, int LP_ = 1>
struct Wino4Geo {
    static constexpr bool PT7 = PT_ == 7;
    static_assert(PT_ == 6 || (PT7 && (K == 7 || K == 11)), "seven-point groups: k = 7 / 11");
    static constexpr int WM = 2, WN = 2;
    static constexpr int NSF = K == 1 ? 0 : (K == 3 ? 1 : (K == 7 ? 2 : (PT7 ? 3 : 4)));
    static constexpr int NL = (!PT7 && (K == 7 || K == 1)) ? 1 : 0;
    static constexpr int GSF = PT7 ? 7 : 6;
    static constexpr int SSF = PT7 ? 4 : 3;
    static constexpr int NG = PT7 ? (K == 7 ? 13 : 20) : (K == 1 ? 4 : (K == 3 ? 6 : (K == 7 ? 16 : 23)));
    static constexpr int NGQ = PT7 ? NG : ((NG + 1) & ~1);
    static constexpr bool WSHARE = K == 1;
    static constexpr int NGW = WSHARE ? 1 : NGQ;
    static constexpr int NPL = PT7 ? 7 : (NL ? 8 : 6);
    static constexpr int NPOS = K == 1 ? 4 : (K == 3 ? 6 : (K == 7 ? 10 : 14));
    static constexpr int NOCT = NOCT_, NSTAGE = NSTAGE_;
    static constexpr int NPH = PT7 ? ((K == 11 && LP_ == 2) ? 2 : 1) : (K == 11 ? 2 : 1);
    static constexpr int PH0 = PT7 ? 8 : 12;
    static constexpr int NGPM = NPH == 1 ? NG : 12;
    static_assert(NPH == 1 || (PH0 <= NGPM && NG - PH0 <= NGPM), "phase sizes");
    static constexpr int CO_BLK = WM * 32;
    static constexpr int NTUP = WN * 32;
    static constexpr int NT_BLK = 4 * NTUP;
    static constexpr int BUF4 = NOCT * 2 * NGPM * NTUP;
    static constexpr int PF = 4;
    static constexpr int NM = 4;
    __host__ __device__ static constexpr int glo(int ph) { return NPH == 1 ? 0 : PH0 * ph; }
    __host__ __device__ static constexpr int ngp(int ph) { return NPH == 1 ? NG : (ph == 0 ? PH0 : NG - PH0); }
    __host__ __device__ static constexpr int ngq(int ph) { return NPH == 1 ? NGQ : (PT7 ? ngp(ph) : 12); }
    __host__ __device__ static constexpr int gfirst(int g) {
        return g < GSF * NSF ? SSF * (g / GSF) : 3 * NSF + (g - 6 * NSF);
    }
    __host__ __device__ static constexpr int glast(int g) {
        if (PT7) return 4 * (g / 7) + (g % 7 == 6 ? 6 : 5);
        return g < 6 * NSF ? (3 * (g / 6) + 5 < NPOS ? 3 * (g / 6) + 5 : NPOS - 1) : 3 * NSF + (g - 6 * NSF);
    }
    __host__ __device__ static constexpr int plane(int g) {
        if (PT7) return g % 7;
        return g < 6 * NSF ? g % 6 : ((g - 6 * NSF) == 0 ? 0 : ((g - 6 * NSF) == 1 ? 6 : ((g - 6 * NSF) == 2 ? 7 : 5)));
    }
    __host__ __device__ static constexpr int mlo(int ph) { return gfirst(glo(ph)); }
    __host__ __device__ static constexpr int mhi(int ph) {
        int m = 0;
        for (int g = glo(ph); g < glo(ph) + ngp(ph); ++g) m = glast(g) > m ? glast(g) : m;
        return m;
    }
    static_assert(mhi(NPH - 1) == NPOS - 1 && mlo(0) == 0, "the groups cover the window and nothing past it");
    __host__ __device__ static constexpr int npos(int ph) { return mhi(ph) - mlo(ph) + 1; }
    static constexpr int NPOSP = npos(0) > npos(NPH - 1) ? npos(0) : npos(NPH - 1);
    __host__ __device__ static constexpr int ngap(int ph) { return NOCT * ngp(ph) * NM; }
    __host__ __device__ static constexpr int sph(int ph) { return ((ph - (NSTAGE - 1)) % NPH + NPH) % NPH; }
    __host__ __device__ static constexpr int sgap(int ph) { return ngap(sph(ph)); }
    static constexpr int JSF = 10;
    __host__ __device__ static constexpr int sflo(int ph) { return glo(ph) / 7; }
    __host__ __device__ static constexpr bool inph(int ph, int g) { return g >= glo(ph) && g < glo(ph) + ngp(ph); }
    __host__ __device__ static constexpr int glast_ph(int ph) { return glo(ph) + ngp(ph) - 1; }
    __host__ __device__ static constexpr int nwj(int ph) {
        return PT7 ? JSF * (glast_ph(ph) / 7 - sflo(ph)) + (glast_ph(ph) % 7 == 0 ? 3 : JSF) : NOCT * ngp(ph);
    }
    static_assert(!PT7 || (NOCT == 1 && glo(0) % 7 <= 1 && glo(NPH - 1) % 7 <= 1 &&
                           (glast_ph(0) % 7 == 0 || glast_ph(0) % 7 >= 5) && glast_ph(NPH - 1) % 7 >= 5),
                  "seven-point phases: start on V0 / V1 of a sub-filter (the partial sums are formed per phase), end on V0 or the last row");
    __host__ __device__ static constexpr int fdiv4(int e) { return e >= 0 ? e / 4 : -((3 - e) / 4); }
    __host__ __device__ static constexpr int vlo(int ph) { return fdiv4(mlo(ph) - (K - 1) / 2); }
    __host__ __device__ static constexpr int nvec(int ph) { return fdiv4(mhi(ph) - (K - 1) / 2) - vlo(ph) + 1; }
    static constexpr int NVP = nvec(0) > nvec(NPH - 1) ? nvec(0) : nvec(NPH - 1);
    __host__ __device__ static constexpr int nljv(int ph) { return NOCT * 2 * nvec(ph); }
    static constexpr int DAV = (K == 3 || K == 1) ? 8 : 16;
    __host__ __device__ static constexpr int tw0v(int ph) { return DAV + 2 * nljv(ph); }
    __host__ __device__ static constexpr int wsv(int ph) { return (sgap(ph) - tw0v(ph)) / nwj(ph); }
    static_assert(LP_ != 1 || (wsv(0) >= 1 && wsv(NPH - 1) >= 1), "one write job per gap at most (vector loads)");
    static constexpr int RAWW = 320;
    static constexpr int NROW = 2 * NOCT;
    static constexpr int RAW_BYTES = 4 * (NROW * RAWW * 4 + 16);
    static constexpr int DAT = K == 7 ? 16 : (K == 11 ? 12 : 8);
    __host__ __device__ static constexpr int nrj(int ph) { return NROW * ((npos(ph) + 1) / 2); }
    __host__ __device__ static constexpr bool loads_in(int ph) { return ph == 0; }
    __host__ __device__ static constexpr int tr_r0(int ph) { return loads_in(ph) ? DAT + 2 * NROW : 0; }
    __host__ __device__ static constexpr int tw0t(int ph) { return tr_r0(ph) + nrj(ph) + 1; }
    __host__ __device__ static constexpr int wst(int ph) { return (sgap(ph) - tw0t(ph)) / nwj(ph); }
    static_assert(LP_ != 2 || (wst(0) >= 1 && wst(NPH - 1) >= 1), "one write job per gap at most (strip path)");
    static constexpr int QX = WSHARE ? 0 : (NOCT * ngq(0)) % PF;
    static constexpr int QMAIN = NOCT * ngq(0) - QX;
    static_assert(QX == 0 || (NPH == 1 && NOCT == 1 && QMAIN >= 2 * PF), "extra queue slots: one phase, one octet");
    static_assert((WSHARE ? NOCT : NOCT * ngq(NPH - 1)) % PF == 0 || QX != 0, "queue slots line up across steps");
    static_assert((size_t)NSTAGE * BUF4 * 16 + (LP_ == 2 ? RAW_BYTES : 0) <= 80 * 1024, "two blocks per CU");
    static_assert(NPH == 1 || NOCT == 1, "phases split an octet's groups");
};

__device__ __host__ constexpr int wino4_tile(int d, int ntup) { return (4 * ntup / (4 * d)) * (4 * d); }

template <int K, int NOCT_, int NSTAGE_, int EPI, int LP, int PT = 6>
__global__ __launch_bounds__(256, kConvMinWaves) void conv1d_wino4_f32(const ConvParams p) {
    extern __shared__ __attribute__((aligned(16))) float4 smem4[];
    using G = Wino4Geo<K, NOCT_, NSTAGE_, PT, LP>;
    constexpr bool PT7 = G::PT7;
    constexpr int WN = G::WN, NSF = G::NSF, NOCT = G::NOCT, NSTAGE = G::NSTAGE, NPL = G::NPL, NGPM = G::NGPM;
    constexpr int CO_BLK = G::CO_BLK, NTUP = G::NTUP, NT_BLK = G::NT_BLK, PF = G::PF;
    constexpr int NPH = G::NPH, NPOSP = G::NPOSP, NM = G::NM;
    constexpr bool D1 = LP == 1, TR = LP == 2;
    static_assert(D1 || TR, "window path");
    const int dil = D1 ? 1 : p.dil;
    const int nt_eff = wino4_tile(dil, NTUP), ntup_eff = nt_eff / 4;
    const int tiles_y = p.CoutP / CO_BLK;
    const int per_tile = tiles_y * p.ksplit;
    const unsigned sidx = blockIdx.x, xcd = sidx & 7u, u = sidx >> 3;
    const int yk = (int)(u % (unsigned)per_tile);
    const unsigned gt = (u / (unsigned)per_tile) * 8u + xcd;
    const int n_tiles_x = (p.Nout + nt_eff - 1) / nt_eff;
    int b = (int)(gt / (unsigned)n_tiles_x);
    int q0 = (int)(gt % (unsigned)n_tiles_x) * nt_eff;
    if (p.compact) {
        int tile = 0;
        if (!live_tile(p.lens_out, p.len_out_mul, p.Nout, nt_eff, p.batch, gt, b, tile)) return;
        b = __builtin_amdgcn_readfirstlane(b);
        q0 = __builtin_amdgcn_readfirstlane(tile) * nt_eff;
    } else if (b >= p.batch) {
        return;
    }
    const int tid = threadIdx.x, lane = tid & 63, wid = tid >> 6;
    const int wm = wid / WN, wn = wid % WN;
    const int ks = yk / tiles_y;
    const int co_blk0 = (yk - ks * tiles_y) * CO_BLK;
    int n_out = p.Nout;
    if (p.lens_out) n_out = min(n_out, (int)p.lens_out[b] * p.len_out_mul);
    if (q0 >= n_out) return;
    int in_len = p.Lin;
    if (p.lens_in) in_len = min(in_len, (int)p.lens_in[b] * p.len_in_mul);

    const int x_cs = p.x_cs, CoutP = p.CoutP;
    const int chunks_all = p.Cin / (8 * NOCT);
    const int c_beg = (int)((int64_t)ks * chunks_all / p.ksplit), n_chunks = (int)((int64_t)(ks + 1) * chunks_all / p.ksplit);
    const int n_groups = (p.Cin / 8) * G::NGW;
    const float* __restrict__ xb = p.x + (int64_t)b * p.x_bs;
    const float in_slope = p.in_slope;

    constexpr bool REG = EPI >= 3, RES = EPI == 3;
    static_assert(!REG || (LP == 1 && K != 1), "register epilogue: dilation 1, k = 3 / 7 / 11");
    float ep_bias = 0.f;
    if constexpr (!REG) {
        if (tid < CO_BLK && p.bias) ep_bias = p.bias[min(co_blk0 + tid, p.Cout - 1)];
    }

    const int kk = lane >> 5, l31 = lane & 31;
    const int pe = wn * 32 + l31;
    const int col_e = dil == 1 ? 4 * pe : (pe / dil) * 4 * dil + pe % dil;
    f32x16 acc[NPL];
#pragma unroll
    for (int g = 0; g < NPL; ++g)
#pragma unroll
        for (int r = 0; r < 16; ++r) acc[g][r] = 0.f;
    const int ep_row0 = REG ? co_blk0 + __builtin_amdgcn_readfirstlane(wm) * 32 : 0;
    const int ep_voff = (q0 + col_e < n_out ? q0 + col_e : 0) * 4;
    const int ep_rrow = ep_row0 + 4 * kk;
    const bfo_i4 ep_rs = bfo_rsrc(RES ? p.res + (int64_t)b * p.r_bs : nullptr, RES ? (unsigned)p.Cout * (unsigned)p.r_cs * 4u : 0u);
    const bfo_i4 ep_bs = bfo_rsrc(p.bias, (REG && p.bias) ? (unsigned)p.Cout * 4u : 0u);
    w4_f32x4 rq[RES ? 16 : 1], bsq[REG ? 4 : 1];
    constexpr int EP_T0 = RES ? 16 : 0;
#define TTS_EPLOAD_JOB(T)                                                                            \
    {                                                                                                \
        if (RES && (T) < 16)                                                                         \
            rq[RES ? (T) : 0] = __builtin_bit_cast(w4_f32x4, bfo_ld16(ep_rs, ep_voff + (ep_rrow + ((T) & 3) + 8 * ((T) >> 2)) * p.r_cs * 4, 0, 0)); \
        if ((T) >= EP_T0 && (T) < EP_T0 + 4)                                                         \
            bsq[REG ? (T) - EP_T0 : 0] = __builtin_bit_cast(w4_f32x4, bfo_ld16(ep_bs, (ep_rrow + 8 * ((T) - EP_T0)) * 4, 0, 0)); \
    }

    const bfo_i4 wrs = bfo_rsrc(K == 1 ? p.w : (PT7 ? p.w_wino44 : p.w_wino4), (unsigned)n_groups * 2u * (unsigned)CoutP * 16u);
    const int wv = (kk * CoutP + co_blk0 + wm * 32 + l31) * 16;
    const int wstep = 2 * CoutP * 16, wlast = (n_groups - 1) * wstep;
    int wso = c_beg * NOCT * G::NGW * wstep;
    w4_f32x4 aq[PF + G::QX];
    if constexpr (G::QX == 0) {
#pragma unroll
        for (int g = 0; g < PF; ++g) {
            aq[g] = __builtin_bit_cast(w4_f32x4, bfo_ld16(wrs, wv, wso, 0));
            wso = min(wso + wstep, wlast);
        }
    } else {
#pragma unroll
        for (int g = 0; g < PF + G::QX; ++g)
            aq[g] = __builtin_bit_cast(w4_f32x4, bfo_ld16(wrs, wv, min(wso + (g < PF ? g : G::QMAIN + g - PF) * wstep, wlast), 0));
    }

    const int sh = __builtin_amdgcn_readfirstlane((tid >> 7) & 1), skk = __builtin_amdgcn_readfirstlane((tid >> 6) & 1);
    w4_f32x2 sx[D1 ? 1 : NOCT][D1 ? 1 : NPOSP];
    w4_f32x4 sv[D1 ? NOCT : 1][2][D1 ? G::NVP : 1];
    w4_f32x2 ta[NOCT], tb[NOCT];
    w4_f32x2 tf[PT7 ? 5 : 1], te[PT7 ? 4 : 1], td[PT7 ? 3 : 1], th[PT7 ? 2 : 1];
    const int spe = min(lane, ntup_eff - 1);
    const int xw0 = (q0 + 4 * lane) * 4;
    constexpr int pad_c = (K - 1) / 2;
    const int ch_off = (4 * sh + skk) * x_cs;

#define TTS_VJOB_IDX(PH, J)                                                                          \
        const int nv_ = G::nvec(PH);                                                                 \
        const int ol_ = (J) / (2 * nv_), pp_ = ((J) / nv_) % 2, vi_ = (J) % nv_;
#define TTS_VLOAD_JOB(PH, J, XSO)                                                                    \
    {                                                                                                \
        TTS_VJOB_IDX(PH, J)                                                                          \
        const bfo_i4 xrs_ = bfo_rsrc(xb + ((XSO) + ch_off + (8 * ol_ + 2 * pp_) * x_cs), (unsigned)in_len * 4u);     \
        sv[ol_][pp_][vi_] = __builtin_bit_cast(w4_f32x4, bfo_ld16(xrs_, xw0 + 16 * (G::vlo(PH) + vi_), 0, 0));      \
    }
#define TTS_VACT_JOB(PH, A)                                                                          \
    {                                                                                                \
        TTS_VJOB_IDX(PH, (A) / 2)                                                                    \
        if ((A) % 2 == 0) {                                                                          \
            sv[ol_][pp_][vi_].x = bfo_lrelu(sv[ol_][pp_][vi_].x, in_slope);                          \
            sv[ol_][pp_][vi_].y = bfo_lrelu(sv[ol_][pp_][vi_].y, in_slope);                          \
        } else {                                                                                     \
            sv[ol_][pp_][vi_].z = bfo_lrelu(sv[ol_][pp_][vi_].z, in_slope);                          \
            sv[ol_][pp_][vi_].w = bfo_lrelu(sv[ol_][pp_][vi_].w, in_slope);                          \
        }                                                                                            \
    }
    float* const strip = reinterpret_cast<float*>(smem4 + NSTAGE * G::BUF4) + wid * (G::NROW * G::RAWW + 4);
    const int tr_a = (q0 - pad_c * dil) & ~3;
    const int tr_off = q0 + (dil == 1 ? 4 * spe : (spe / dil) * 4 * dil + spe % dil) - pad_c * dil - tr_a;
    w4_f32x4 rv[TR ? G::NROW : 1][2];
#define TTS_TLOAD_JOB(J, XSO)                                                                        \
    {                                                                                                \
        const int pp_ = (J) / 2, vs_ = (J) % 2;                                                      \
        const bfo_i4 xrs_ = bfo_rsrc(xb + ((XSO) + ch_off + (8 * (pp_ / 2) + 2 * (pp_ % 2)) * x_cs), (unsigned)in_len * 4u); \
        const int v_ = lane + 64 * vs_;                                                              \
        rv[pp_][vs_] = __builtin_bit_cast(w4_f32x4, bfo_ld16(xrs_, (vs_ == 1 && lane >= 16) ? BFO_OOB : (tr_a + 4 * v_) * 4, 0, 0)); \
    }
#define TTS_TSTORE_JOB(J)                                                                            \
    {                                                                                                \
        const int pp_ = (J) / 2, vs_ = (J) % 2;                                                      \
        w4_f32x4 a_ = rv[pp_][vs_];                                                                  \
        a_.x = bfo_lrelu(a_.x, in_slope); a_.y = bfo_lrelu(a_.y, in_slope);                          \
        a_.z = bfo_lrelu(a_.z, in_slope); a_.w = bfo_lrelu(a_.w, in_slope);                          \
        const int v_ = lane + 64 * vs_;                                                              \
        float* dst_ = (vs_ == 1 && lane >= 16) ? strip + G::NROW * G::RAWW : strip + pp_ * G::RAWW + 4 * v_;    \
        *reinterpret_cast<w4_f32x4*>(dst_) = a_;                                                     \
    }
#define TTS_TREAD_JOB(PH, J)                                                                         \
    {                                                                                                \
        const int npr_ = (G::npos(PH) + 1) / 2;                                                      \
        const int pp_ = (J) / npr_, jp_ = (J) % npr_;                                                \
        const float* src_ = strip + pp_ * G::RAWW + tr_off + (G::mlo(PH) + 2 * jp_) * dil;           \
        sx[pp_ / 2][2 * jp_][pp_ % 2] = src_[0];                                                     \
        if (2 * jp_ + 1 < G::npos(PH)) sx[pp_ / 2][2 * jp_ + 1][pp_ % 2] = src_[dil];                \
    }
#define TTS_SXV(M) (w4_f32x2{sv[ol_][0][G::fdiv4((M) - pad_c) - G::vlo(PH_)][((M) - pad_c) - 4 * G::fdiv4((M) - pad_c)],     \
                             sv[ol_][1][G::fdiv4((M) - pad_c) - G::vlo(PH_)][((M) - pad_c) - 4 * G::fdiv4((M) - pad_c)]})
#define TTS_SX(M) (D1 ? TTS_SXV(M) : sx[D1 ? 0 : ol_][D1 ? 0 : (M) - G::mlo(PH_)])
#define TTS_WRITE_JOB(PH, J, WR)                                                                     \
    {                                                                                                \
        const int PH_ = (PH);                                                                        \
        const int ol_ = PT7 ? 0 : (J) / G::ngp(PH_), gl_ = (J) % G::ngp(PH_), g_ = G::glo(PH_) + gl_;                          \
        w4_f32x2 v2;                                                                                 \
        if constexpr (PT7) {                                                                         \
             \
            const int sf_ = G::sflo(PH_) + (J) / G::JSF, kd_ = (J) % G::JSF, s4 = 4 * sf_, g0_ = 7 * sf_;                      \
            const bool v0_ = G::inph(PH_, g0_), tap4_ = g0_ + 6 < G::NG;                             \
            int row_ = -1;                                                                           \
            if (kd_ == 0) {                         \
                if (v0_) tf[0] = sf_ > G::sflo(PH_) ? tf[4] : TTS_SX(s4 + 2) - 4.f * TTS_SX(s4);    \
                tf[1] = TTS_SX(s4 + 3) - 4.f * TTS_SX(s4 + 1);                                       \
                tf[2] = TTS_SX(s4 + 4) - 4.f * TTS_SX(s4 + 2);                                       \
            } else if (kd_ == 1) {                                                                   \
                tf[3] = TTS_SX(s4 + 5) - 4.f * TTS_SX(s4 + 3);                                       \
                if (v0_) te[0] = tf[0] - 2.f * tf[1];                                                \
            } else if (kd_ == 2) {                                                                   \
                te[2] = tf[2] - 2.f * tf[3];                                                         \
                if (v0_) { v2 = te[2] - te[0]; row_ = 0; }                                           \
            } else if (kd_ == 3) {                                                                   \
                te[1] = tf[1] - 2.f * tf[2];                                                         \
                v2 = te[1] + te[2]; row_ = 1;                                                        \
            } else if (kd_ == 4) {                                                                   \
                v2 = te[1] - te[2]; row_ = 2;                                                        \
            } else if (kd_ == 5) {                                                                   \
                v2 = tf[3] - tf[1]; row_ = 5;                                                        \
            } else if (kd_ == 6) {                                                                   \
                if (tap4_) {                                                                         \
                    tf[4] = TTS_SX(s4 + 6) - 4.f * TTS_SX(s4 + 4);                                   \
                    te[3] = tf[3] - 2.f * tf[4];                                                     \
                    v2 = te[1] - te[3]; row_ = 6;                                                    \
                }                                                                                    \
            } else if (kd_ == 7) {                                                                   \
                td[0] = TTS_SX(s4 + 1) - TTS_SX(s4 + 3);                                             \
                td[1] = TTS_SX(s4 + 2) - TTS_SX(s4 + 4);                                             \
                td[2] = TTS_SX(s4 + 3) - TTS_SX(s4 + 5);                                             \
            } else if (kd_ == 8) {                                                                   \
                th[0] = td[0] - 2.f * td[1];                                                         \
                th[1] = td[1] - 2.f * td[2];                                                         \
                v2 = 2.f * th[0] + th[1]; row_ = 3;                                                  \
            } else {                                                                                 \
                v2 = 2.f * th[0] - th[1]; row_ = 4;                                                  \
            }                                                                                        \
            if (row_ >= 0) (WR)[2 * ((g0_ + row_ - G::glo(PH_)) * NTUP)] = v2;                       \
        } else if (g_ < 6 * NSF) {                                                                   \
            const int s3 = 3 * (g_ / 6), i_ = g_ % 6;                                                \
             \
            if (i_ == 0) v2 = 4.f * TTS_SX(s3) + (TTS_SX(s3 + 4) - 5.f * TTS_SX(s3 + 2));           \
            else if (i_ == 1) {                                                                      \
                ta[ol_] = TTS_SX(s3 + 4) - 4.f * TTS_SX(s3 + 2);                                     \
                tb[ol_] = TTS_SX(s3 + 3) - 4.f * TTS_SX(s3 + 1);                                     \
                v2 = ta[ol_] + tb[ol_];                                                              \
            } else if (i_ == 2) v2 = ta[ol_] - tb[ol_];                                              \
            else if (i_ == 3) {                                                                      \
                ta[ol_] = TTS_SX(s3 + 4) - TTS_SX(s3 + 2);                                           \
                tb[ol_] = 2.f * (TTS_SX(s3 + 3) - TTS_SX(s3 + 1));                                   \
                v2 = ta[ol_] + tb[ol_];                                                              \
            } else if (i_ == 4) v2 = ta[ol_] - tb[ol_];                                              \
            else v2 = 4.f * TTS_SX(s3 + 1) + (TTS_SX(s3 + 5 < G::NPOS ? s3 + 5 : s3) - 5.f * TTS_SX(s3 + 3));           \
        } else {                                                                                     \
            v2 = TTS_SX(3 * NSF + (g_ - 6 * NSF));                                                   \
        }                                                                                            \
        if constexpr (!PT7) (WR)[2 * ((ol_ * 2 * NGPM + gl_) * NTUP)] = v2;                          \
    }

    const float4* sB = smem4 + kk * NGPM * NTUP + wn * 32 + l31;
    w4_f32x2* sW = reinterpret_cast<w4_f32x2*>(smem4 + skk * NGPM * NTUP + lane) + sh;
    float4 bq[2];

    {
#pragma unroll
        for (int st = 0; st < NSTAGE - 1; ++st) {
            const int ph = st % NPH;
            const int xso = min(c_beg + st / NPH, n_chunks - 1) * 8 * NOCT * x_cs;
            if constexpr (D1) {
#pragma unroll
                for (int J = 0; J < G::nljv(ph); ++J) TTS_VLOAD_JOB(ph, J, xso)
#pragma unroll
                for (int J = 0; J < 2 * G::nljv(ph); ++J) TTS_VACT_JOB(ph, J)
            } else {
                if (G::loads_in(ph)) {
#pragma unroll
                    for (int J = 0; J < 2 * G::NROW; ++J) TTS_TLOAD_JOB(J, xso)
#pragma unroll
                    for (int J = 0; J < 2 * G::NROW; ++J) TTS_TSTORE_JOB(J)
                }
#pragma unroll
                for (int J = 0; J < G::nrj(ph); ++J) TTS_TREAD_JOB(ph, J)
            }
            w4_f32x2* wr = sW + 2 * st * G::BUF4;
#pragma unroll
            for (int J = 0; J < G::nwj(ph); ++J) TTS_WRITE_JOB(ph, J, wr)
        }
    }
    __syncthreads();
    bq[0] = sB[0];

    int stage = 0;
#define TTS_CHUNK_STEPS(LAST, C) \
        _Pragma("unroll")                                                                                                                                    \
        for (int ph = 0; ph < NPH; ++ph) {                                                                                                                   \
            const bool peel = (LAST) && ph == NPH - 1;                                                                                                       \
                                      \
            const int tph = (ph + NSTAGE - 1) % NPH;                                                                                                         \
            const int xso = min((C) + (ph + NSTAGE - 1) / NPH, n_chunks - 1) * 8 * NOCT * x_cs;                                                                \
            const int stage_next = (stage + 1 == NSTAGE) ? 0 : stage + 1;                                                                                    \
            const int stage_fill = (stage == 0) ? NSTAGE - 1 : stage - 1;                                                                                    \
            w4_f32x2* wr = sW + 2 * stage_fill * G::BUF4;                                                                                                    \
            const float4* rd = sB + stage * G::BUF4;                                                                                                         \
            const int sn = ((C) + 1 < n_chunks || ph + 1 < NPH) ? stage_next : stage;                                                                          \
        _Pragma("unroll")                                                                                                                                    \
            for (int gs = 0; gs < NOCT * G::ngq(ph); ++gs) {                                                                                                 \
                const int ol = gs / G::ngq(ph), gl = gs % G::ngq(ph);                                                                                        \
                const int qs = G::WSHARE ? ol % PF : ((G::QX && gs >= G::QMAIN) ? PF + gs - G::QMAIN : gs % PF);                                             \
                const w4_f32x4 a4 = aq[qs];                                                                                                                  \
                                          \
                if constexpr (G::QX != 0) {                                                                                                                  \
                                            \
                    const int nx = gs < G::QMAIN - PF ? gs + PF : (gs < G::QMAIN ? G::NGQ + gs + PF - G::QMAIN : G::NGQ + gs);                               \
                    if (!peel || nx < G::NGQ) aq[qs] = __builtin_bit_cast(w4_f32x4, bfo_ld16(wrs, wv, min(wso + nx * wstep, wlast), 0));                     \
                    if (gs == G::NGQ - 1) wso += G::NGQ * wstep;                                                                                             \
                } else if ((!G::WSHARE || gl == G::ngq(ph) - 1) && (!peel || gs + PF < NOCT * G::ngq(ph))) {                                                 \
                    aq[qs] = __builtin_bit_cast(w4_f32x4, bfo_ld16(wrs, wv, wso, 0));                                                                        \
                    wso = min(wso + wstep, wlast);                                                                                                           \
                }                                                                                                                                            \
                if (gl >= G::ngp(ph)) continue;                                                     \
                const int r = ol * G::ngp(ph) + gl;                                                                \
                const int cur = r & 1, nxt = cur ^ 1;                                                                                                        \
                const int plane = G::plane(G::glo(ph) + gl);                                                                                                 \
                                                    \
                if (r + 1 < NOCT * G::ngp(ph)) bq[nxt] = rd[(((r + 1) / G::ngp(ph)) * 2 * NGPM + (r + 1) % G::ngp(ph)) * NTUP];                              \
                else if (NSTAGE >= 3 && !peel) bq[nxt] = sB[sn * G::BUF4];        \
                __builtin_amdgcn_sched_barrier(0);                                                                                                           \
                const float bv[4] = {bq[cur].x, bq[cur].y, bq[cur].z, bq[cur].w};                                                                            \
        _Pragma("unroll")                                                                                                                                    \
                for (int m = 0; m < NM; ++m) {                                                                                                               \
                    acc[plane] = __builtin_amdgcn_mfma_f32_32x32x2f32(a4[m], bv[m], acc[plane], 0, 0, 0);                                                    \
                                   \
                                                                                             \
                    const int t = r * NM + m;                                                                                                                \
                    if (peel) {                                                                                                                              \
                        TTS_EPLOAD_JOB(t)                                                                                                                    \
                    } else if constexpr (D1) {                                                                                                               \
                        if (t < G::nljv(tph)) TTS_VLOAD_JOB(tph, t, xso)                                                                                     \
                        if (t >= G::DAV && t - G::DAV < 2 * G::nljv(tph)) TTS_VACT_JOB(tph, t - G::DAV)                                                      \
                        if (t >= G::tw0v(tph) && (t - G::tw0v(tph)) % G::wsv(tph) == 0 &&                                                                    \
                            (t - G::tw0v(tph)) / G::wsv(tph) < G::nwj(tph))                                                                                  \
                            TTS_WRITE_JOB(tph, (t - G::tw0v(tph)) / G::wsv(tph), wr)                                                                         \
                    } else {                                                                                                                                 \
                        if (G::loads_in(tph) && t < 2 * G::NROW) TTS_TLOAD_JOB(t, xso)                                                                       \
                        if (G::loads_in(tph) && t >= G::DAT && t < G::DAT + 2 * G::NROW) TTS_TSTORE_JOB(t - G::DAT)                                          \
                        if (t >= G::tr_r0(tph) && t - G::tr_r0(tph) < G::nrj(tph)) TTS_TREAD_JOB(tph, t - G::tr_r0(tph))                                     \
                        if (t >= G::tw0t(tph) && (t - G::tw0t(tph)) % G::wst(tph) == 0 && (t - G::tw0t(tph)) / G::wst(tph) < G::nwj(tph))                    \
                            TTS_WRITE_JOB(tph, (t - G::tw0t(tph)) / G::wst(tph), wr)                                                                         \
                    }                                                                                                                                        \
                    __builtin_amdgcn_sched_barrier(0);                                                                                                       \
                }                                                                                                                                            \
            }                                                                                                                                                \
            if (peel) break;                                                                                                                                 \
            __syncthreads();                                                                                                                                 \
            if (NSTAGE < 3) bq[0] = sB[sn * G::BUF4];                                      \
            else if ((NOCT * G::ngp(ph)) % 2 != 0) bq[0] = bq[1];                                                                                            \
            stage = stage_next;                                                                                                                              \
        }
    for (int c = c_beg; c < n_chunks - (REG ? 1 : 0); ++c) {
        TTS_CHUNK_STEPS(false, c)
    }
    if constexpr (REG) {
        const int c = n_chunks - 1;
        TTS_CHUNK_STEPS(true, c)
    }
#undef TTS_CHUNK_STEPS
#undef TTS_EPLOAD_JOB
#undef TTS_TLOAD_JOB
#undef TTS_TSTORE_JOB
#undef TTS_TREAD_JOB
#undef TTS_VLOAD_JOB
#undef TTS_VACT_JOB
#undef TTS_VJOB_IDX
#undef TTS_SXV
#undef TTS_SX
#undef TTS_WRITE_JOB

#define TTS_OUT_QUAD(R)                                                                              \
        const float s12 = acc[1][R] + acc[2][R], d12 = acc[1][R] - acc[2][R];                        \
        const float s34 = acc[3][R] + acc[4][R], d34 = acc[3][R] - acc[4][R];                        \
        float y0 = acc[0][R] + s12 + s34;                                                            \
        float y1 = d12 + 2.f * d34;                                                                  \
        float y2 = s12 + 4.f * s34;                                                                  \
        float y3 = d12 + 8.f * d34 + acc[PT7 ? 6 : 5][R];                                            \
        if constexpr (NSF == 0) { y0 = acc[0][R]; y1 = 0.f; y2 = 0.f; y3 = acc[5][R]; }               \
        if constexpr (PT7) {                                                                   \
            y0 += acc[5][R];                                                                         \
            y1 += 0.5f * acc[5][R];                                                                  \
            y2 += 0.25f * acc[5][R];                                                                 \
            y3 += 0.125f * acc[5][R];                                                                \
        } else if constexpr (NPL == 8) {                                                             \
            y1 += acc[6][R];                                                                         \
            y2 += acc[7][R];                                                                         \
        }
    float* __restrict__ yb = p.y + (int64_t)b * p.y_bs;
    const int mode = p.mode, relu_out = p.relu_out, Cout = p.Cout;
    const float div = p.div;
    if constexpr (REG) {
        const int q = q0 + col_e, y_cs = p.y_cs;
        if (q >= n_out) return;
        const bool full = q + 3 < n_out;
        const bfo_i4 ys = bfo_rsrc(yb, (unsigned)Cout * (unsigned)y_cs * 4u);
        const float lo = relu_out == 1 ? 0.f : -__builtin_inff();
        constexpr int PB = NPL >= 8 ? 4 : 8;
#pragma unroll
        for (int h = 0; h < 16 / PB; ++h) {
            w4_f32x4 pq[PB];
#pragma unroll
            for (int i = 0; i < PB; ++i) {
                const int r = PB * h + i;
                pq[i] = w4_f32x4{0.f, 0.f, 0.f, 0.f};
                if (mode != 0)
                    pq[i] = __builtin_bit_cast(w4_f32x4, bfo_ld16(ys, ep_voff + (ep_rrow + (r & 3) + 8 * (r >> 2)) * y_cs * 4, 0, 0));
            }
#pragma unroll
            for (int i = 0; i < PB; ++i) {
                const int r = PB * h + i;
                const int co = ep_rrow + (r & 3) + 8 * (r >> 2);
                TTS_OUT_QUAD(r)
                w4_f32x4 v = {y0, y1, y2, y3};
                const float bsv = bsq[REG ? r >> 2 : 0][r & 3];
#pragma unroll
                for (int e = 0; e < 4; ++e) {
                    float x = v[e] + bsv;
                    if constexpr (RES) x += rq[RES ? r : 0][e];
                    v[e] = fmaxf(x, lo);
                }
                if (mode != 0) {
                    v = pq[i] + v;
                    if (mode == 2) {
#pragma unroll
                        for (int e = 0; e < 4; ++e) v[e] = v[e] / div;
                    }
                }
                if (co >= Cout) continue;
                float* yp = yb + (int64_t)co * y_cs + q;
                if (full) {
                    *reinterpret_cast<w4_f32x4*>(yp) = v;
                } else {
#pragma unroll
                    for (int e = 0; e < 4; ++e)
                        if (q + e < n_out) yp[e] = v[e];
                }
            }
        }
        return;
    }
    constexpr int LDS_F = CO_BLK * NT_BLK + CO_BLK;
    constexpr int LPR = NT_BLK / 4;
    static_assert(LPR == 64, "one wave instruction per row");
    float* ep = reinterpret_cast<float*>(smem4);
    float* epb = ep + LDS_F - CO_BLK;
    const float* __restrict__ rb = p.res ? p.res + (int64_t)b * p.r_bs : nullptr;
    __syncthreads();
    if (tid < CO_BLK) epb[tid] = ep_bias;
#pragma unroll
    for (int r = 0; r < 16; ++r) {
        const int row = wm * 32 + (r & 3) + 8 * (r >> 2) + 4 * kk;
        TTS_OUT_QUAD(r)
        if (pe < ntup_eff) {
            if (dil == 1) {
                *reinterpret_cast<float4*>(ep + row * NT_BLK + col_e) = make_float4(y0, y1, y2, y3);
            } else {
                ep[row * NT_BLK + col_e] = y0;
                ep[row * NT_BLK + col_e + dil] = y1;
                ep[row * NT_BLK + col_e + 2 * dil] = y2;
                ep[row * NT_BLK + col_e + 3 * dil] = y3;
            }
        }
    }
#undef TTS_OUT_QUAD
    __syncthreads();
    constexpr int NR = CO_BLK / 4;
    const int col = lane * 4, q = q0 + col;
    if (q >= n_out || col >= nt_eff) return;
    const bool full = q + 3 < n_out;
    if (p.ksplit > 1) {
        float* __restrict__ pb = p.splitk_ws + ((int64_t)ks * p.batch + b) * Cout * p.Nout;
#pragma unroll 4
        for (int it = 0; it < NR; ++it) {
            const int rl = wid + it * 4;
            const int co = co_blk0 + rl;
            if (co >= Cout) continue;
            const float4 a4 = *reinterpret_cast<const float4*>(ep + rl * NT_BLK + col);
            float* yp = pb + (int64_t)co * p.Nout + q;
            if (full && (p.Nout & 3) == 0) {
                *reinterpret_cast<float4*>(yp) = a4;
            } else {
                const float v[4] = {a4.x, a4.y, a4.z, a4.w};
#pragma unroll
                for (int e = 0; e < 4; ++e)
                    if (q + e < n_out) yp[e] = v[e];
            }
        }
        return;
    }
    const float* __restrict__ scale = K == 1 ? p.scale : nullptr;
    const bool plain_act = K != 1 || (relu_out < 2 && scale == nullptr);
    if (plain_act && !rb && mode == 0) {
        const float lo = relu_out == 1 ? 0.f : -__builtin_inff();
#pragma unroll 4
        for (int it = 0; it < NR; ++it) {
            const int rl = wid + it * 4;
            const int co = co_blk0 + rl;
            if (co >= Cout) continue;
            const float bsv = epb[rl];
            const float4 a4 = *reinterpret_cast<const float4*>(ep + rl * NT_BLK + col);
            float v[4] = {fmaxf(a4.x + bsv, lo), fmaxf(a4.y + bsv, lo), fmaxf(a4.z + bsv, lo), fmaxf(a4.w + bsv, lo)};
            float* yp = yb + (int64_t)co * p.y_cs + q;
            if (full) {
                *reinterpret_cast<float4*>(yp) = make_float4(v[0], v[1], v[2], v[3]);
            } else {
#pragma unroll
                for (int e = 0; e < 4; ++e)
                    if (q + e < n_out) yp[e] = v[e];
            }
        }
        return;
    }
#pragma unroll 2
    for (int it = 0; it < NR; ++it) {
        const int rl = wid + it * 4;
        const int co = co_blk0 + rl;
        if (co >= Cout) continue;
        const float bsv = epb[rl];
        const float4 a4 = *reinterpret_cast<const float4*>(ep + rl * NT_BLK + col);
        float v[4] = {a4.x, a4.y, a4.z, a4.w};
        float* yp = yb + (int64_t)co * p.y_cs + q;
        const float* rp = rb ? rb + (int64_t)co * p.r_cs + q : nullptr;
        float rr4[4] = {0.f, 0.f, 0.f, 0.f}, pp4[4] = {0.f, 0.f, 0.f, 0.f};
        if (full) {
            if (rp) { const float4 t = *reinterpret_cast<const float4*>(rp); rr4[0] = t.x; rr4[1] = t.y; rr4[2] = t.z; rr4[3] = t.w; }
            if (mode != 0) { const float4 t = *reinterpret_cast<const float4*>(yp); pp4[0] = t.x; pp4[1] = t.y; pp4[2] = t.z; pp4[3] = t.w; }
        } else {
#pragma unroll
            for (int e = 0; e < 4; ++e)
                if (q + e < n_out) {
                    if (rp) rr4[e] = rp[e];
                    if (mode != 0) pp4[e] = yp[e];
                }
        }
        const float scv = (K == 1 && scale) ? scale[co] : 1.f;
#pragma unroll
        for (int e = 0; e < 4; ++e) {
            float x = v[e] + bsv;
            if constexpr (K == 1) {
                if (relu_out == 2) x = 0.5f * x * (1.0f + erff(x * 0.70710678118654752440f));
                x = x * scv;
            }
            x += rr4[e];
            if (relu_out == 1) x = fmaxf(x, 0.f);
            if constexpr (K == 1) { if (relu_out == 3) x = tanhf(x); }
            if (mode == 1) x = pp4[e] + x;
            else if (mode == 2) x = (pp4[e] + x) / div;
            v[e] = x;
        }
        if (full) {
            *reinterpret_cast<float4*>(yp) = make_float4(v[0], v[1], v[2], v[3]);
        } else {
#pragma unroll
            for (int e = 0; e < 4; ++e)
                if (q + e < n_out) yp[e] = v[e];
        }
    }
}

template <int K, int NOCT, int NSTAGE, int EPI, int LP, int PT = 6>
static int32_t launch_wino4_epi(const ConvParams& p, hipStream_t stream) {
    using G = Wino4Geo<K, NOCT, NSTAGE, PT, LP>;
    constexpr size_t ring = (size_t)G::NSTAGE * G::BUF4 * sizeof(float4);
    constexpr size_t epi = ((size_t)G::CO_BLK * G::NT_BLK + G::CO_BLK) * sizeof(float);
    constexpr size_t strip = LP == 2 ? (size_t)G::RAW_BYTES : 0;
    constexpr size_t lds = (EPI >= 3 || ring + strip > epi) ? ring + strip : epi;
    static_assert(lds <= 80 * 1024, "two blocks per CU");
    static_assert(EPI < 3 || lds == ring, "register epilogue: the ring sets the LDS size");
    static std::atomic<uint64_t> lds_done{0};
    const auto kern = conv1d_wino4_f32<K, NOCT, NSTAGE, EPI, LP, PT>;
    TTS_CHECK_HIP(lds_opt_in((const void*)kern, (int)lds, lds_done));
    const int nt = wino4_tile(p.dil, G::NTUP);
    ConvParams q = p;
    q.ksplit = EPI == 0 ? wino4_ksplit(p) : 1;
    note_conv_launch(PT == 7 ? 4 : 3, q.ksplit);
    const int64_t n_tiles = (int64_t)((p.Nout + nt - 1) / nt) * p.batch;
    const int64_t n_blocks = ((n_tiles + 7) / 8) * 8 * (p.CoutP / G::CO_BLK) * q.ksplit;
    TTS_REQUIRE(n_blocks < ((int64_t)1 << 31), "wino4: %lld blocks", (long long)n_blocks);
    dim3 grid((unsigned)n_blocks, 1, 1);
    q.compact = compact_order(p.lens_out, p.batch) ? 1 : 0;
    hipLaunchKernelGGL(kern, grid, dim3(256), lds, stream, q);
    TTS_CHECK_HIP(hipGetLastError());
    if (q.ksplit > 1) return launch_splitk_reduce(q, stream);
    return 0;
}

template <int K, int NOCT, int NSTAGE>
static int32_t launch_wino4_cfg(const ConvParams& p, hipStream_t stream) {
    if (p.dil == 1) {
        if (wino4_ksplit(p) != 1) return launch_wino4_epi<K, NOCT, NSTAGE, 0, 1>(p, stream);
        if (p.res != nullptr) return launch_wino4_epi<K, NOCT, NSTAGE, 3, 1>(p, stream);
        return launch_wino4_epi<K, NOCT, NSTAGE, 4, 1>(p, stream);
    }
    return launch_wino4_epi<K, NOCT, 2, 0, 2>(p, stream);
}

template <int K>
static int32_t launch_wino44_cfg(const ConvParams& p, hipStream_t stream) {
    if (p.dil == 1) {
        if (wino4_ksplit(p) != 1) return launch_wino4_epi<K, 1, 2, 0, 1, 7>(p, stream);
        if (p.res != nullptr) return launch_wino4_epi<K, 1, 2, 3, 1, 7>(p, stream);
        return launch_wino4_epi<K, 1, 2, 4, 1, 7>(p, stream);
    }
    return launch_wino4_epi<K, 1, 2, 0, 2, 7>(p, stream);
}

bool wino44_wanted(const ConvParams& p) {
    if (p.w_wino44 == nullptr || (p.K != 7 && p.K != 11)) return false;
    return ((int)opt_int(OPT_WINO4, kWino4Default) & (p.K == 7 ? 32 : 64)) != 0;
}

int32_t launch_wino4(const ConvParams& p, hipStream_t stream) {
    if (wino44_wanted(p)) return p.K == 7 ? launch_wino44_cfg<7>(p, stream) : launch_wino44_cfg<11>(p, stream);
    if (p.K == 1) return launch_wino4_epi<1, 4, 2, 0, 1>(p, stream);
    if (p.K == 3) return launch_wino4_cfg<3, 2, 3>(p, stream);
    if (p.K == 7) return launch_wino4_cfg<7, 1, 2>(p, stream);
    if (p.K == 11) return launch_wino4_cfg<11, 1, 3>(p, stream);
    set_error("wino4: kernel size %d not built (1, 3, 7, 11)", p.K);
    return TTSAMD_EINVAL;
}

int wino4_block_outputs(int dil) { return wino4_tile(dil, 64); }

int wino4_ksplit(const ConvParams& p) {
    const int bo = wino4_block_outputs(p.dil);
    const int64_t blocks = (int64_t)((p.Nout + bo - 1) / bo) * (p.CoutP / 64) * p.batch;
    constexpr int sk_blocks = 192, sk_target = 224;
    if (blocks >= sk_blocks || p.splitk_ws == nullptr) return 1;
    const int n_chunks = p.Cin / (p.K == 1 ? 32 : (p.K == 3 ? 16 : 8));
    const int64_t per = (int64_t)p.batch * p.Cout * p.Nout;
    int64_t ks = std::min<int64_t>((sk_target + blocks - 1) / blocks, n_chunks / 8);
    ks = std::min<int64_t>(ks, p.splitk_floats / std::max<int64_t>(per, 1));
    return ks >= 2 ? (int)ks : 1;
}

int wino4_groups(int k) { return k == 3 ? 6 : (k == 7 ? 16 : 24); }
int wino44_groups(int k) { return k == 7 ? 13 : (k == 11 ? 20 : 0); }

void wino4_filter_groups(const float* g, int k, float* o) {
    const int nsf = k == 3 ? 1 : (k == 7 ? 2 : 4);
    for (int s = 0; s < nsf; ++s) {
        const double g0 = g[3 * s], g1 = 3 * s + 1 < k ? g[3 * s + 1] : 0.0, g2 = 3 * s + 2 < k ? g[3 * s + 2] : 0.0;
        o[6 * s] = (float)(g0 / 4);
        o[6 * s + 1] = (float)(-(g0 + g1 + g2) / 6);
        o[6 * s + 2] = (float)(-(g0 - g1 + g2) / 6);
        o[6 * s + 3] = (float)(g0 / 24 + g1 / 12 + g2 / 6);
        o[6 * s + 4] = (float)(g0 / 24 - g1 / 12 + g2 / 6);
        o[6 * s + 5] = (float)g2;
    }
    if (k == 7)
        for (int j = 0; j < 4; ++j) o[12 + j] = g[6];
}

void pack_wino4_weight(const float* w, int cout, int cin, int k, float* out) {
    const int ng = wino4_groups(k);
    std::vector<float> u((size_t)cout * cin * ng);
    for (int64_t i = 0; i < (int64_t)cout * cin; ++i) wino4_filter_groups(w + i * k, k, u.data() + i * ng);
    pack_conv_weight(u.data(), cout, cin, ng, out);
}

void wino44_filter_groups(const float* g, int k, float* o) {
    const int nsf = (k + 3) / 4;
    for (int s = 0; s < nsf; ++s) {
        const double g0 = g[4 * s], g1 = g[4 * s + 1], g2 = g[4 * s + 2], g3 = 4 * s + 3 < k ? g[4 * s + 3] : 0.0;
        o[7 * s] = (float)(g0 / 4);
        o[7 * s + 1] = (float)((g0 + g1 + g2 + g3) / 6);
        o[7 * s + 2] = (float)((g0 - g1 + g2 - g3) / 18);
        o[7 * s + 3] = (float)((g0 + 2 * g1 + 4 * g2 + 8 * g3) / 72);
        o[7 * s + 4] = (float)((g0 - 2 * g1 + 4 * g2 - 8 * g3) / 120);
        o[7 * s + 5] = (float)((32 * g0 + 16 * g1 + 8 * g2 + 4 * g3) / 45);
        if (4 * s + 3 < k) o[7 * s + 6] = (float)(g3 / 2);
    }
}

void pack_wino44_weight(const float* w, int cout, int cin, int k, float* out) {
    const int ng = wino44_groups(k);
    std::vector<float> u((size_t)cout * cin * ng);
    for (int64_t i = 0; i < (int64_t)cout * cin; ++i) wino44_filter_groups(w + i * k, k, u.data() + i * ng);
    pack_conv_weight(u.data(), cout, cin, ng, out);
}

}
```

tts-arabic-pytorch_amd/ttsamd/engine.py:

```python
import ctypes as C

import numpy as np
import torch

from . import lib as L
from .config import NET_CONFIG, HIFIGAN_CONFIG, VOCOS_22K_CONFIG, TACOTRON2_CONFIG


def _require_gpu():
    if not torch.cuda.is_available():
        raise L.TtsAmdError('no ROCm device visible: the ttsamd engines run only on an MI355X (gfx950); '
                            'there is no CPU fallback')
    lib = L.load()
    if not lib.ttsamd_device_ok():
        raise L.TtsAmdError('device 0 is not gfx950')
    return lib


PRECISIONS = {'f32': 0, 'bf16': 1, 'bf16x3': 2}


def set_precision(name):
    lib = L.load()
    L.check(lib.ttsamd_set_precision(PRECISIONS[name]), 'set_precision')
# ... 378 lines not shown
        lens = lens.to(device=self.device, dtype=torch.int64).contiguous()
        n0 = self.hop * (T0 - 1) if self.center else self.hop * T0
        if T0 == 0 or n0 == 0:
            return torch.zeros(B, 0, dtype=torch.float32, device=self.device)
        T = (T0 + 3) & ~3
        if T != T0:
            mel = torch.nn.functional.pad(mel, (0, T - T0))
        wave = torch.zeros(B, self.hop * T, dtype=torch.float32, device=self.device)
        bias = self.bias_vec().reshape(-1) if rows is not None or denoise != 0 else None
        with torch.cuda.device(self.device):
            nb = self.lib.ttsamd_vocos_workspace_bytes(self.handle, B, T)
            ws = self.ws.get(nb, self.device)
            if rows is not None:
                L.check(self.lib.ttsamd_vocos_forward_rows(self.handle, _ptr(mel), _ptr(lens), B, T, _ptr(rows), _ptr(bias),
                                                           _ptr(wave), _ptr(ws), nb, _stream()), 'vocos_forward_rows')
            else:
                L.check(self.lib.ttsamd_vocos_forward(self.handle, _ptr(mel), _ptr(lens), B, T, float(denoise), _ptr(bias),
                                                      _ptr(wave), _ptr(ws), nb, _stream()), 'vocos_forward')
        return wave if wave.shape[1] == n0 else wave[:, :n0]


class Tacotron2Engine:

    def __init__(self, state_dict, config=None, device='cuda'):
        self.lib = _require_gpu()
        self.device = torch.device(device if device != 'cuda' else 'cuda:0')
        c = dict(TACOTRON2_CONFIG if config is None else config)
        self.config = c
        cfg = L.Tacotron2Cfg()
        for name, _ in L.Tacotron2Cfg._fields_:
            setattr(cfg, name, int(bool(c.get(name, True))) if name == 'decoder_early_stopping' else c[name])
        arr, keep = L.make_tensors(state_dict)
        handle = C.c_void_p()
        with torch.cuda.device(self.device):
            L.check(self.lib.ttsamd_tacotron2_create(arr, len(arr), C.byref(cfg), C.byref(handle)), 'tacotron2_create')
        self.handle = handle
        self.ws = _Workspace()
        self.n_mels = c['n_mels']
        self.max_decoder_steps = c.get('decoder_max_step', 2000)

    def __del__(self):
        if getattr(self, 'handle', None):
            self.lib.ttsamd_tacotron2_destroy(self.handle)
            self.handle = None

    def infer(self, tokens, speaker_ids=None, lengths=None, max_step=None, dropout_seed=-1):
        _check_ids(tokens, self.config['n_symbol'], 'Tacotron2 tokens')
        if speaker_ids is not None and self.config['num_speakers'] > 1:
            _check_ids(speaker_ids, self.config['num_speakers'], 'Tacotron2 speaker_ids')
        tokens = tokens.to(device=self.device, dtype=torch.int64).contiguous()
        B, Ltok = tokens.shape
        if lengths is None:
            lengths = torch.full((B,), Ltok, dtype=torch.int64)
        lengths = lengths.to(device=self.device, dtype=torch.int64).contiguous()
        if self.config['num_speakers'] > 1:
            if speaker_ids is None:
                speaker_ids = torch.zeros(B, dtype=torch.int64)
            speaker_ids = speaker_ids.to(device=self.device, dtype=torch.int64).contiguous()
        else:
            speaker_ids = None
        max_step = int(self.max_decoder_steps if max_step is None else max_step)
        if dropout_seed is None:
            dropout_seed = int(torch.randint(0, 2 ** 31 - 1, (1,)).item())
        mel_post = torch.zeros(B, self.n_mels, max_step, dtype=torch.float32, device=self.device)
        mel_raw = torch.zeros(B, self.n_mels, max_step, dtype=torch.float32, device=self.device)
        mel_lens = torch.zeros(B, dtype=torch.int32, device=self.device)
        align = torch.zeros(B, max_step, Ltok, dtype=torch.float32, device=self.device)
        n_steps = C.c_int32(0)
        with torch.cuda.device(self.device):
            nb = self.lib.ttsamd_tacotron2_workspace_bytes(self.handle, B, Ltok, max_step)
            ws = self.ws.get(nb, self.device)
            L.check(self.lib.ttsamd_tacotron2_infer(self.handle, _ptr(tokens), _ptr(lengths), _ptr(speaker_ids), B, Ltok,
                                                    max_step, int(dropout_seed), _ptr(mel_post), _ptr(mel_lens),
                                                    _ptr(align), _ptr(mel_raw), C.byref(n_steps), _ptr(ws), nb,
                                                    _stream()), 'tacotron2_infer')
        T = n_steps.value
        return mel_post[:, :, :T], mel_lens, align[:, :T]


class TaggerEngine:

    RENAME = {'emb0.weight': 'emb.weight', 'emb_input.weight': 'emb.weight'}

    def __init__(self, state_dict, config, device='cuda'):
        self.lib = _require_gpu()
        self.device = torch.device(device if device != 'cuda' else 'cuda:0')
        c = dict(config)
        cfg = L.TaggerCfg()
        cfg.n_vocab, cfg.emb_dim = c['n_vocab'], c['emb_dim']
        cfg.n_lstm, cfg.n_dense = len(c['lstm_hidden']), len(c['dense_dim'])
        for i, v in enumerate(c['lstm_hidden']):
            cfg.lstm_hidden[i] = v
        for i, v in enumerate(c['dense_dim']):
            cfg.dense_dim[i] = v
        cfg.hard_sigmoid, cfg.bn_after_lstm0, cfg.bn_eps = c['hard_sigmoid'], c['bn_after_lstm0'], c['bn_eps']
        self.n_classes = c['dense_dim'][-1]
        self.n_vocab = c['n_vocab']
        arr, keep = L.make_tensors({self.RENAME.get(k, k): v for k, v in state_dict.items()})
        handle = C.c_void_p()
        with torch.cuda.device(self.device):
            L.check(self.lib.ttsamd_tagger_create(arr, len(arr), C.byref(cfg), C.byref(handle)), 'tagger_create')
        self.handle = handle
        self.ws = _Workspace()

    def __del__(self):
        if getattr(self, 'handle', None):
            self.lib.ttsamd_tagger_destroy(self.handle)
            self.handle = None

    def forward(self, ids):
        ids = torch.as_tensor(ids)
        _check_ids(ids, self.n_vocab, 'tagger ids')
        ids = ids.to(device=self.device, dtype=torch.int64).contiguous()
        B, T = ids.shape
        probs = torch.empty(B, T, self.n_classes, dtype=torch.float32, device=self.device)
        if T == 0:
            return probs
        with torch.cuda.device(self.device):
            nb = self.lib.ttsamd_tagger_workspace_bytes(self.handle, B, T)
            ws = self.ws.get(nb, self.device)
            L.check(self.lib.ttsamd_tagger_forward(self.handle, _ptr(ids), B, T, _ptr(probs), _ptr(ws), nb, _stream()),
                    'tagger_forward')
        return probs


def conv1d(x, w, bias=None, lens=None, dilation=1, in_slope=1.0, relu_out=False, res=None, mode=0, div=1.0, y=None, splitk_floats=None):
    lib = _require_gpu()
    x = x.contiguous().float()
    w = w.contiguous().float()
    B, cin, lin = x.shape
    cout, cin2, k = w.shape
    assert cin == cin2
    if y is None:
        y = torch.zeros(B, cout, lin, dtype=torch.float32, device=x.device)
    packed = torch.empty(lib.ttsamd_conv1d_packed_floats(cout, cin, k), dtype=torch.float32, device=x.device)
    with torch.cuda.device(x.device):
        if splitk_floats is None:
            L.check(lib.ttsamd_conv1d_ex(_ptr(x), _ptr(w), _ptr(bias), _ptr(res), _ptr(lens), B, cin, cout, k, dilation, lin,
                                         float(in_slope), int(relu_out), int(mode), float(div), _ptr(y), _ptr(packed), _stream()), 'conv1d')
        else:
            ws = torch.full((max(int(splitk_floats), 1),), float('nan'), dtype=torch.float32, device=x.device)
            L.check(lib.ttsamd_conv1d_splitk(_ptr(x), _ptr(w), _ptr(bias), _ptr(res), _ptr(lens), B, cin, cout, k, dilation, lin,
                                             float(in_slope), int(relu_out), int(mode), float(div), _ptr(y), _ptr(packed), _ptr(ws),
                                             int(splitk_floats), _stream()), 'conv1d_splitk')
    return y


def last_conv_launch():
    route, ksplit = C.c_int32(-1), C.c_int32(0)
    L.check(L.load().ttsamd_conv_last_launch(C.byref(route), C.byref(ksplit)), 'conv_last_launch')
    return route.value, ksplit.value


def conv_transpose1d(x, w, bias=None, lens=None, in_slope=1.0, y=None):
    lib = _require_gpu()
    x = x.contiguous().float()
    w = w.contiguous().float()
    B, cin, lin = x.shape
    cin2, cout, kt = w.shape
    assert cin == cin2 and kt % 2 == 0
    u = kt // 2
    if y is None:
        y = torch.zeros(B, cout, lin * u, dtype=torch.float32, device=x.device)
    assert tuple(y.shape) == (B, cout, lin * u) and y.is_contiguous() and y.dtype == torch.float32
    if lens is not None:
        lens = lens.to(device=x.device, dtype=torch.int64).contiguous()
    packed = torch.empty(max(int(lib.ttsamd_convt_packed_floats(cin, cout, u)), 1), dtype=torch.float32, device=x.device)
    with torch.cuda.device(x.device):
        L.check(lib.ttsamd_conv_transpose1d(_ptr(x), _ptr(w), _ptr(bias), _ptr(lens), B, cin, cout, u, lin, float(in_slope), _ptr(y),
                                            _ptr(packed), _stream()), 'conv_transpose1d')
    return y


def resblock_pair(x, w1, b1, w2, b2, dil, lens=None, len_mul=1, y=None, mode=0, div=1.0, slope=0.1, variant=2):
    lib = _require_gpu()
    x = x.contiguous().float()
    w1, w2, b1, b2 = (t.contiguous().float() for t in (w1, w2, b1, b2))
    B, Cc, Lx = x.shape
    k = w1.shape[2]
    assert tuple(w1.shape) == tuple(w2.shape) == (Cc, Cc, k)
    if y is None:
        assert mode == 0
        y = torch.zeros_like(x)
    if lens is not None:
        lens = lens.to(device=x.device, dtype=torch.int64).contiguous()
    n_packed = int(lib.ttsamd_resblock_pair_packed_floats(Cc, k, int(variant)))
    packed = torch.empty(max(n_packed, 1), dtype=torch.float32, device=x.device)
    with torch.cuda.device(x.device):
        L.check(lib.ttsamd_resblock_pair(_ptr(x), _ptr(y), _ptr(w1), _ptr(b1), _ptr(w2), _ptr(b2), Cc, k, int(dil), _ptr(lens),
                                         int(len_mul), Lx, B, int(mode), float(div), float(slope), int(variant), _ptr(packed),
                                         n_packed, _stream()), 'resblock_pair')
    return y


def resblock2(x, w1, b1, w2, b2, dil1, dil2, lens=None, len_mul=1, y=None, mode=0, div=1.0, slope=0.1, variant=2):
    lib = _require_gpu()
    x = x.contiguous().float()
    w1, w2, b1, b2 = (t.contiguous().float() for t in (w1, w2, b1, b2))
    B, Cc, Lx = x.shape
    k = w1.shape[2]
    assert tuple(w1.shape) == tuple(w2.shape) == (Cc, Cc, k)
    if y is None:
        assert mode == 0
        y = torch.zeros_like(x)
    if lens is not None:
        lens = lens.to(device=x.device, dtype=torch.int64).contiguous()
    n_packed = int(lib.ttsamd_resblock2_packed_floats(Cc, k, int(variant)))
    packed = torch.empty(max(n_packed, 1), dtype=torch.float32, device=x.device)
    with torch.cuda.device(x.device):
        L.check(lib.ttsamd_resblock2(_ptr(x), _ptr(y), _ptr(w1), _ptr(b1), _ptr(w2), _ptr(b2), Cc, k, int(dil1), int(dil2), _ptr(lens),
                                     int(len_mul), Lx, B, int(mode), float(div), float(slope), int(variant), _ptr(packed), n_packed,
                                     _stream()), 'resblock2')
    return y


def length_regulate(enc, reps, t_max):
    lib = _require_gpu()
    enc = enc.contiguous().float()
    reps = reps.contiguous().to(torch.int64)
    B, Cc, Lt = enc.shape
    out = torch.empty(B, Cc, t_max, dtype=torch.float32, device=enc.device)
    idx = torch.empty(B, t_max, dtype=torch.int32, device=enc.device)
    with torch.cuda.device(enc.device):
        L.check(lib.ttsamd_length_regulate(_ptr(enc), _ptr(reps), B, Lt, Cc, t_max, _ptr(out), _ptr(idx), _stream()),
                'length_regulate')
    return out, idx


OVERSMOOTH_KEYS = ('HQER', 'CSlope', 'CCentroid', 'CRoll95')
OVERSMOOTH_MAX_FRAMES = 4096
_dtw_ws = _Workspace()


def _dev_f32(t, ndim, what):
    if not isinstance(t, torch.Tensor) or t.device.type != 'cuda':
        raise L.TtsAmdError(f'{what}: expected a tensor on the ROCm device (there is no CPU fallback)')
    if t.dim() != ndim:
        raise L.TtsAmdError(f'{what}: expected {ndim} dimensions, got shape {tuple(t.shape)}')
    return t.to(torch.float32).contiguous()


def _dev_lens(lens, B, T, device):
    if lens is None:
        return torch.full((B,), T, dtype=torch.int64, device=device)
    lens = torch.as_tensor(lens).to(device=device, dtype=torch.int64).contiguous()
    if lens.shape != (B,):
        raise L.TtsAmdError(f'lens of shape {tuple(lens.shape)} for a batch of {B}')
    return lens


def cepstral_series(mel, lens=None, center=True, hann=True, q_c=None, hqer_scale=100.0, return_power=False):
    lib = _require_gpu()
    mel = _dev_f32(mel, 3, 'cepstral_series: mel')
    B, M, T = mel.shape
    lens = _dev_lens(lens, B, T, mel.device)
    out = torch.empty(B, 4, T, dtype=torch.float32, device=mel.device)
    power = torch.empty(B, M // 2 + 1, T, dtype=torch.float32, device=mel.device) if return_power else None
    if B:
        with torch.cuda.device(mel.device):
            L.check(lib.ttsamd_cepstral_series(_ptr(mel), _ptr(lens), B, M, T, int(bool(center)), int(bool(hann)),
                                               -1 if q_c is None else int(q_c), float(hqer_scale), _ptr(power), _ptr(out), _stream()),
                    'cepstral_series')
    return (out, power) if return_power else out


def cepstral_series_from_power(power, lens=None, q_c=None, q1=1, q2=None, eps=1e-8, roll_p=0.95, hqer_scale=1.0):
    lib = _require_gpu()
    power = _dev_f32(power, 3, 'cepstral_series_from_power: power')
    B, Q, T = power.shape
    lens = _dev_lens(lens, B, T, power.device)
    out = torch.empty(B, 4, T, dtype=torch.float32, device=power.device)
    if B:
        with torch.cuda.device(power.device):
            L.check(lib.ttsamd_cepstral_series_from_power(_ptr(power), _ptr(lens), B, Q, T, -1 if q_c is None else int(q_c), int(q1),
                                                          Q - 1 if q2 is None else int(q2), float(eps), float(roll_p), float(hqer_scale),
                                                          _ptr(out), _stream()), 'cepstral_series_from_power')
    return out


def series_summary(series, lens=None):
    lib = _require_gpu()
    series = _dev_f32(series, 3, 'series_summary: series')
    B, K, T = series.shape
    lens = _dev_lens(lens, B, T, series.device)
    stats = torch.empty(B, K, 3, dtype=torch.float32, device=series.device)
    feat = torch.empty(B, K, T, dtype=torch.float32, device=series.device)
    if B and K:
        with torch.cuda.device(series.device):
            L.check(lib.ttsamd_series_summary(_ptr(series), _ptr(lens), B, K, T, _ptr(stats), _ptr(feat), _stream()), 'series_summary')
    return stats, feat


def dtw(a, b, lens_a=None, lens_b=None, metric='l2', window=None, workspace=None):
    lib = _require_gpu()
    a, b = _dev_f32(a, 3, 'dtw: a'), _dev_f32(b, 3, 'dtw: b')
    if a.shape[0] != b.shape[0] or a.shape[1] != b.shape[1]:
        raise L.TtsAmdError(f'dtw: a {tuple(a.shape)} and b {tuple(b.shape)} differ in batch or channels')
    m = str(metric).lower()
    if m not in ('l2', 'cosine'):
        raise L.TtsAmdError(f'dtw: metric {metric!r} (l2 | cosine)')
    B, M, Ta = a.shape
    Tb = b.shape[2]
    lens_a, lens_b = _dev_lens(lens_a, B, Ta, a.device), _dev_lens(lens_b, B, Tb, a.device)
    cost = torch.empty(B, dtype=torch.float32, device=a.device)
    path = torch.empty(B, Ta + Tb, 2, dtype=torch.int32, device=a.device)
    plen = torch.empty(B, dtype=torch.int32, device=a.device)
# ... 699 lines not shown
```

tts-arabic-pytorch_amd/ttsamd/lib.py:

```python
import ctypes as C
import os

_HERE = os.path.dirname(os.path.abspath(__file__))
LIB_PATH = os.environ.get('TTSAMD_LIB') or os.path.join(_HERE, 'lib', 'libttsamd.so')


class TtsAmdError(RuntimeError):
    pass


class Tensor(C.Structure):
    _fields_ = [('name', C.c_char_p), ('data', C.POINTER(C.c_float)), ('ndim', C.c_int32),
                ('shape', C.c_int64 * 4)]


class HifiGanCfg(C.Structure):
    _fields_ = [('num_mels', C.c_int32), ('upsample_initial_channel', C.c_int32), ('n_ups', C.c_int32),
                ('upsample_rates', C.c_int32 * 8), ('upsample_kernel_sizes', C.c_int32 * 8),
                ('n_kernels', C.c_int32), ('resblock_kernel_sizes', C.c_int32 * 8),
                ('n_dilations', C.c_int32), ('resblock_dilations', (C.c_int32 * 8) * 8), ('resblock', C.c_int32)]


class FastPitchCfg(C.Structure):
    _fields_ = [(n, C.c_int32) for n in (
        'n_mel_channels', 'n_symbols', 'padding_idx', 'd_model',
        'in_fft_n_layers', 'in_fft_n_heads', 'in_fft_d_head', 'in_fft_kernel', 'in_fft_filter',
        'out_fft_n_layers', 'out_fft_n_heads', 'out_fft_d_head', 'out_fft_kernel', 'out_fft_filter',
        'dur_kernel', 'dur_filter', 'dur_n_layers',
        'pitch_kernel', 'pitch_filter', 'pitch_n_layers', 'pitch_emb_kernel',
        'energy_conditioning', 'energy_kernel', 'energy_filter', 'energy_n_layers', 'energy_emb_kernel',
        'n_speakers')] + [('speaker_emb_weight', C.c_float)]


class Tacotron2Cfg(C.Structure):
    _fields_ = [(n, C.c_int32) for n in (
        'n_symbol', 'num_speakers', 'speaker_embedding_dim', 'symbol_embedding_dim', 'encoder_embedding_dim',
        'encoder_n_convolution', 'encoder_kernel_size', 'n_mels', 'prenet_dim', 'attention_rnn_dim',
        'decoder_rnn_dim', 'attention_hidden_dim', 'attention_location_n_filter',
        'attention_location_kernel_size', 'postnet_n_convolution', 'postnet_kernel_size',
        'postnet_embedding_dim')] + [('gate_threshold', C.c_float), ('decoder_early_stopping', C.c_int32)]


class TaggerCfg(C.Structure):
    _fields_ = [('n_vocab', C.c_int32), ('emb_dim', C.c_int32), ('n_lstm', C.c_int32), ('lstm_hidden', C.c_int32 * 4),
                ('hard_sigmoid', C.c_int32), ('bn_after_lstm0', C.c_int32), ('bn_eps', C.c_float),
                ('n_dense', C.c_int32), ('dense_dim', C.c_int32 * 4)]


class AlignerCfg(C.Structure):
    _fields_ = [(n, C.c_int32) for n in ('n_mel', 'd_text', 'n_att', 'n_symbols', 'padding_idx')]


class PyinCfg(C.Structure):
    _fields_ = [('sample_rate', C.c_int32), ('frame_length', C.c_int32), ('win_length', C.c_int32), ('hop_length', C.c_int32),
                ('fmin', C.c_double), ('fmax', C.c_double), ('n_thresholds', C.c_int32), ('beta_a', C.c_int32), ('beta_b', C.c_int32),
                ('boltzmann', C.c_double), ('resolution', C.c_double), ('max_transition_rate', C.c_double),
                ('switch_prob', C.c_double), ('no_trough_prob', C.c_double), ('pad_mode', C.c_int32)]


_P, _I32, _I64, _F = C.c_void_p, C.c_int32, C.c_int64, C.c_float
SYMBOLS = {
    'ttsamd_last_error': (C.c_char_p, []),
    'ttsamd_version': (_I32, []),
    'ttsamd_set_option': (_I32, [C.c_char_p, C.c_char_p]),
    'ttsamd_get_option': (_I32, [C.c_char_p, C.c_char_p, _I32]),
    'ttsamd_option_name': (C.c_char_p, [_I32]),
    'ttsamd_options_check': (_I32, []),
    'ttsamd_device_ok': (_I32, []),
    'ttsamd_hifigan_create': (_I32, [C.POINTER(Tensor), _I32, C.POINTER(HifiGanCfg), C.POINTER(_P)]),
    'ttsamd_hifigan_destroy': (_I32, [_P]),
    'ttsamd_hifigan_workspace_bytes': (_I64, [_P, _I32, _I32]),
    'ttsamd_hifigan_forward': (_I32, [_P, _P, _P, _I32, _I32, _P, _P, _I64, _P]),
    'ttsamd_hifigan_halo_frames': (_I32, [_P, C.POINTER(_I32), C.POINTER(_I32)]),
    'ttsamd_denoiser_halo_frames': (_I32, []),
    'ttsamd_stream_gather': (_I32, [_P, _I32, _I32, _I32, _P, _P, _P, _I32, _I32, _P, _P, _P]),
    'ttsamd_stream_emit': (_I32, [_P, _I32, _I32, _I32, _P, _P, _I32, _I32, _P, _P]),
    'ttsamd_stream_emit_resampled': (_I32, [_P, _P, _I32, _I32, _I32, _P, _P, _P, _P, _P, _I32, _I32, _P, _P, _P]),
    'ttsamd_vocos_halo_frames': (_I32, [_P, C.POINTER(_I32), C.POINTER(_I32)]),
    'ttsamd_vocos_forward_windows': (_I32, [_P, _P, _P, _I32, _I32, _P, _P, _P, _P, _P, _P, _I64, _P]),
    'ttsamd_wave_encode': (_I32, [_P, _I64, _P, _I32, _I32, _P, _I64, _P]),
    'ttsamd_fastpitch_create': (_I32, [C.POINTER(Tensor), _I32, C.POINTER(FastPitchCfg), C.POINTER(_P)]),
    'ttsamd_fastpitch_destroy': (_I32, [_P]),
    'ttsamd_fastpitch_encode_workspace_bytes': (_I64, [_P, _I32, _I32]),
    'ttsamd_fastpitch_decode_workspace_bytes': (_I64, [_P, _I32, _I32]),
    'ttsamd_fastpitch_encode': (_I32, [_P, _P, _I32, _I32, _I32, _F, _P, _P, _P, _F, _F, _F,
                                       _P, _P, _P, _P, _P, _P, _P, _I64, _P]),
    'ttsamd_length_regulate': (_I32, [_P, _P, _I32, _I32, _I32, _I32, _P, _P, _P]),
    'ttsamd_fastpitch_decode': (_I32, [_P, _P, _P, _I32, _I32, _P, _P, _I64, _P]),
    'ttsamd_fastpitch_set_batch_mode': (_I32, [_P, _I32]),
    'ttsamd_fastpitch_encode_rows': (_I32, [_P, _P, _I32, _I32, _I32, _F, _P, _P, _P, _F, _F, _F,
                                            _P, _P, _P, _P, _P, _P, _P, _I64, _P, _P, _P, _P, _I32, _P]),
    'ttsamd_fastpitch_decode_rows': (_I32, [_P, _P, _P, _I32, _I32, _P, _P, _I64, _I32, _P]),
    'ttsamd_denoiser_create': (_I32, [C.POINTER(_P)]),
    'ttsamd_denoiser_destroy': (_I32, [_P]),
    'ttsamd_denoiser_workspace_bytes': (_I64, [_I32, _I32]),
    'ttsamd_denoiser_bias_spec': (_I32, [_P, _P, _P, _I32, _P, _P, _I64, _P]),
    'ttsamd_denoise': (_I32, [_P, _P, _I64, _P, _I32, _I32, _P, _F, _P, _I64, _P]),
    'ttsamd_denoise_rows': (_I32, [_P, _P, _I64, _P, _I32, _I32, _P, _P, _P, _I64, _P]),
    'ttsamd_vocos_create': (_I32, [C.POINTER(Tensor), _I32, _I32, _I32, _I32, _I32, C.POINTER(_P)]),
    'ttsamd_vocos_destroy': (_I32, [_P]),
    'ttsamd_vocos_workspace_bytes': (_I64, [_P, _I32, _I32]),
    'ttsamd_vocos_bias_vec': (_I32, [_P, _P, _P, _I64, _P]),
    'ttsamd_vocos_forward': (_I32, [_P, _P, _P, _I32, _I32, _F, _P, _P, _P, _I64, _P]),
    'ttsamd_vocos_forward_rows': (_I32, [_P, _P, _P, _I32, _I32, _P, _P, _P, _P, _I64, _P]),
    'ttsamd_vocos_set_padding': (_I32, [_P, _I32]),
    'ttsamd_melspec_create': (_I32, [_P, _I32, _I32, _I32, _I32, _I32, _F, C.POINTER(_P)]),
    'ttsamd_melspec_destroy': (_I32, [_P]),
    'ttsamd_melspec_forward': (_I32, [_P, _P, _I64, _P, _I32, _I32, _P, _P, _P]),
    'ttsamd_cepstral_series': (_I32, [_P, _P, _I32, _I32, _I32, _I32, _I32, _I32, _F, _P, _P, _P]),
    'ttsamd_cepstral_series_from_power': (_I32, [_P, _P, _I32, _I32, _I32, _I32, _I32, _I32, C.c_double, C.c_double, _F, _P, _P]),
    'ttsamd_series_summary': (_I32, [_P, _P, _I32, _I32, _I32, _P, _P, _P]),
    'ttsamd_dtw_workspace_bytes': (_I64, [_I32, _I32, _I32, _I32]),
    'ttsamd_dtw': (_I32, [_P, _P, _P, _P, _I32, _I32, _I32, _I32, _I32, _I32, _P, _P, _P, _P, _I64, _P]),
    'ttsamd_dtw_aligned_mae': (_I32, [_P, _P, _I32, _I32, _I32, _P, _P, _P, _P]),
    'ttsamd_mel_cepstrum': (_I32, [_P, _P, _I32, _I32, _I32, _I32, _P, _P]),
    'ttsamd_dtw_aligned_eval': (_I32, [_P, _P, _I32, _I32, _P, _P, _I32, _P, _P, _I32, _I32, _I32, _P, _P, C.c_double, _P, _P]),
    'ttsamd_aligner_create': (_I32, [C.POINTER(Tensor), _I32, C.POINTER(AlignerCfg), C.POINTER(_P)]),
    'ttsamd_aligner_destroy': (_I32, [_P]),
    'ttsamd_aligner_workspace_bytes': (_I64, [_P, _I32, _I32, _I32]),
    'ttsamd_aligner_forward': (_I32, [_P, _P, _P, _P, _P, _P, _I32, _I32, _I32, _P, _P, _P, _I64, _P]),
    'ttsamd_mas_workspace_bytes': (_I64, [_I32, _I32, _I32]),
    'ttsamd_mas': (_I32, [_P, _I32, _P, _P, _I32, _I32, _I32, _P, _P, _P, _I64, _P]),
    'ttsamd_average_pitch': (_I32, [_P, _P, _I32, _I32, _I32, _I32, _P, _P]),
    'ttsamd_attn_prior': (_I32, [_P, _P, _I32, _I32, _I32, _I32, C.c_double, _P, _P]),
    'ttsamd_attn_prior_tables': (_I32, [_I32, _P]),
    'ttsamd_attn_ctc_loss_workspace_bytes': (_I64, [_I32, _I32, _I32]),
    'ttsamd_attn_ctc_loss': (_I32, [_P, _P, _P, _I32, _I32, _I32, C.c_double, _P, _P, _I64, _P]),
    'ttsamd_attn_bin_loss': (_I32, [_P, _P, _I32, _I32, _I32, C.c_double, _P, _P, _P]),
    'ttsamd_pyin_tables': (_I32, [C.POINTER(PyinCfg), _P, _P, _P, _P, _P, _P, _P]),
    'ttsamd_pyin_create': (_I32, [C.POINTER(PyinCfg), C.POINTER(_P)]),
    'ttsamd_pyin_destroy': (_I32, [_P]),
    'ttsamd_pyin_workspace_bytes': (_I64, [_P, _I32, _I32]),
    'ttsamd_pyin_obs_offsets': (_I32, [_P, _I32, _I32, _P]),
    'ttsamd_pyin_forward': (_I32, [_P, _P, _I64, _P, _I32, _I32, _P, _P, _P, _P, _P, _P, _I64, _P]),
    'ttsamd_resample_create': (_I32, [_P, _I32, _I32, _I32, C.POINTER(_P)]),
    'ttsamd_resample_destroy': (_I32, [_P]),
    'ttsamd_resample_out_len': (_I64, [_P, _I64]),
    'ttsamd_resample_mfma_eligible': (_I32, [_P]),
    'ttsamd_resample_forward': (_I32, [_P, _P, _I64, _P, _I32, _P, _I64, _P, _I32, _P]),
    'ttsamd_trim_workspace_bytes': (_I64, [_I32, _I64, _I32]),
    'ttsamd_trim_bounds': (_I32, [_P, _I64, _P, _I32, _F, _I32, _I32, _F, _P, _P, _P, _I64, _P]),
    'ttsamd_trim_apply': (_I32, [_P, _I64, _P, _P, _F, _I64, _I32, _P, _I64, _P, _P]),
    'ttsamd_frames_compact': (_I32, [_P, _P, _P, _I32, _I32, _I32, _I32, _F, _P, _P, _P, _P]),
    'ttsamd_loudness_coefficients': (_I32, [_I32, C.POINTER(C.c_double)]),
    'ttsamd_loudness_workspace_bytes': (_I64, [_I32, _I64, _I32]),
    'ttsamd_loudness_measure': (_I32, [_P, _I64, _P, _I32, _I32, _P, _P, _P, _I64, _P]),
    'ttsamd_wave_level': (_I32, [_P, _I64, _P, _I32, _P, _P, _F, _P, _P, _P, _P]),
    'ttsamd_tacotron2_create': (_I32, [C.POINTER(Tensor), _I32, C.POINTER(Tacotron2Cfg), C.POINTER(_P)]),
    'ttsamd_tacotron2_destroy': (_I32, [_P]),
    'ttsamd_tacotron2_workspace_bytes': (_I64, [_P, _I32, _I32, _I32]),
    'ttsamd_tacotron2_infer': (_I32, [_P, _P, _P, _P, _I32, _I32, _I32, _I64, _P, _P, _P, _P,
                                      C.POINTER(_I32), _P, _I64, _P]),
    'ttsamd_tagger_create': (_I32, [C.POINTER(Tensor), _I32, C.POINTER(TaggerCfg), C.POINTER(_P)]),
    'ttsamd_tagger_destroy': (_I32, [_P]),
    'ttsamd_tagger_workspace_bytes': (_I64, [_P, _I32, _I32]),
    'ttsamd_tagger_forward': (_I32, [_P, _P, _I32, _I32, _P, _P, _I64, _P]),
    'ttsamd_conv1d_packed_floats': (_I64, [_I32, _I32, _I32]),
    'ttsamd_conv1d': (_I32, [_P, _P, _P, _P, _I32, _I32, _I32, _I32, _I32, _I32, _F, _I32, _P, _P, _P]),
    'ttsamd_conv1d_ex': (_I32, [_P, _P, _P, _P, _P, _I32, _I32, _I32, _I32, _I32, _I32, _F, _I32, _I32, _F, _P, _P, _P]),
    'ttsamd_conv1d_splitk': (_I32, [_P, _P, _P, _P, _P, _I32, _I32, _I32, _I32, _I32, _I32, _F, _I32, _I32, _F, _P, _P, _P, _I64, _P]),
    'ttsamd_conv_last_launch': (_I32, [C.POINTER(_I32), C.POINTER(_I32)]),
    'ttsamd_convt_packed_floats': (_I64, [_I32, _I32, _I32]),
    'ttsamd_conv_transpose1d': (_I32, [_P, _P, _P, _P, _I32, _I32, _I32, _I32, _I32, _F, _P, _P, _P]),
    'ttsamd_resblock_pair_packed_floats': (_I64, [_I32, _I32, _I32]),
    'ttsamd_resblock_pair': (_I32, [_P, _P, _P, _P, _P, _P, _I32, _I32, _I32, _P, _I32, _I32, _I32, _I32, _F, _F, _I32, _P, _I64, _P]),
    'ttsamd_resblock2_packed_floats': (_I64, [_I32, _I32, _I32]),
    'ttsamd_resblock2': (_I32, [_P, _P, _P, _P, _P, _P, _I32, _I32, _I32, _I32, _P, _I32, _I32, _I32, _I32, _F, _F, _I32, _P, _I64, _P]),
    'ttsamd_set_precision': (_I32, [_I32]),
    'ttsamd_get_precision': (_I32, []),
    'ttsamd_dp_unique_id': (_I32, [_P]),
    'ttsamd_dp_init': (_I32, [_I32, _I32, _P, C.POINTER(_P)]),
    'ttsamd_dp_destroy': (_I32, [_P]),
    'ttsamd_dp_rank': (_I32, [_P]),
    'ttsamd_dp_world': (_I32, [_P]),
    'ttsamd_dp_broadcast': (_I32, [_P, _P, _I64, _I32, _P]),
    'ttsamd_dp_broadcast_weights': (_I32, [_P, _I32, _P, _I32, _P]),
    'ttsamd_dp_allgather': (_I32, [_P, _P, _P, _I64, _P]),
    'ttsamd_dp_pack_audio': (_I32, [_P, _I64, _P, _I32, _I64, _P, _P]),
    'ttsamd_dp_gather_audio': (_I32, [_P, _P, _P, C.POINTER(_I64), C.POINTER(_I64), _I32, _P]),
    'ttsamd_profile_enable': (_I32, [_I32]),
    'ttsamd_profile_read': (_I32, [C.POINTER(C.c_double)]),
}
_BFO = {
    'pack': (_I32, [_P, _I32, _I32, _I32, _F, _P, _P]),
    'unpack': (_I32, [_P, _I32, _I32, _I32, _F, _P, _P]),
    'weight_elems': (_I64, [_I32, _I32, _I32, _I32]),
    'pack_weight': (_I32, [_P, _I32, _I32, _I32, _I32, _P]),
    'conv1d': (_I32, [_P, _P, _P, _P, _P, _P, _I32, _I32, _I32, _I32, _I32, _I32, _I32, _I32, _I32, _F, _F, _F, _P, _P, _P, _P]),
    'resblock_pair': (_I32, [_P, _P, _P, _P, _P, _P, _P, _I32, _I32, _I32, _I32, _I32, _I32, _I32, _F, _F, _F, _F, _P, _P]),
    'resblock_chain': (_I32, [_P, _P, _P, _P, _P, _P, _P, _P, _I32, _I32, _I32, _I32, _I32, _F, _F, _F, _F, _P, _P, _I32]),
    'conv_post': (_I32, [_P, _P, _P, _P, _I32, _I32, _I32, _I32, _P, _I64, _P]),
}
for _prefix in ('bfo', 'bfo3'):
    for _name, (_res, _args) in _BFO.items():
        SYMBOLS[f'ttsamd_{_prefix}_{_name}'] = (_res, _args[:-1] if (_prefix, _name) == ('bfo3', 'resblock_chain') else _args)

_lib = None
ABI_VERSION = 8


def load():
    global _lib
    if _lib is not None:
        return _lib
    if not os.path.exists(LIB_PATH):
        raise TtsAmdError(f'{LIB_PATH} is missing: build it with `make -C tts-arabic-pytorch_amd/csrc` '
                          '(hipcc --offload-arch=gfx950); there is no CPU/PyTorch fallback')
    import torch
    lib = C.CDLL(LIB_PATH)
    for name, (res, args) in SYMBOLS.items():
        fn = getattr(lib, name)
        fn.restype, fn.argtypes = res, args
    got = lib.ttsamd_version()
    if got != ABI_VERSION:
        raise TtsAmdError(f'{LIB_PATH} was built from another revision of include/ttsamd.h (library ABI {got}, this binding '
                          f'{ABI_VERSION}): rebuild it with `make -C tts-arabic-pytorch_amd/csrc`')
    if lib.ttsamd_options_check() != 0:
        msg = lib.ttsamd_last_error()
        raise TtsAmdError(f'bad routing option in the environment: {msg.decode() if msg else "?"}')
    _lib = lib
    return lib


def set_option(name, value):
    v = None if value is None else str(value).encode()
    check(load().ttsamd_set_option(name.encode(), v), f'set_option({name}={value})')


def get_option(name):
    buf = C.create_string_buffer(64)
    check(load().ttsamd_get_option(name.encode(), buf, 64), f'get_option({name})')
    return buf.value.decode() or None


def option_names():
    lib, out, i = load(), [], 0
    while True:
        n = lib.ttsamd_option_name(i)
        if not n:
            return out
        out.append(n.decode())
        i += 1


class options:

    def __init__(self, **kv):
        self.kv = kv

    def __enter__(self):
        self.old = {k: get_option(k) for k in self.kv}
        for k, v in self.kv.items():
            set_option(k, v)
        return self

    def __exit__(self, *a):
        for k, v in self.old.items():
            set_option(k, v)


def check(rc, what):
    if rc != 0:
        msg = load().ttsamd_last_error()
        raise TtsAmdError(f'{what} failed ({rc}): {msg.decode() if msg else "?"}')


def make_tensors(state_dict):
    import numpy as np
    keep, items = [], []
    for name, v in state_dict.items():
        if hasattr(v, 'detach'):
            if not v.is_floating_point():
                continue
            v = v.detach().cpu().float().numpy()
        a = np.ascontiguousarray(v, dtype=np.float32)
        if a.ndim > 4:
            continue
        t = Tensor()
        nb = name.encode()
        t.name = nb
        t.data = a.ctypes.data_as(C.POINTER(C.c_float))
        t.ndim = a.ndim
        for i, s in enumerate(a.shape):
            t.shape[i] = s
        keep += [a, nb]
        items.append(t)
    arr = (Tensor * len(items))(*items)
    return arr, keep
```

Measured before the change: 76.80 million.

## Add 128-row output-channel blocks for seven-point Winograd conv, dilation 1

Adds a WM=4 variant of the wino4 seven-point kernel that covers 128 output channels per block with 32 time tuples per wave layout. Each block processes two input-channel octets per chunk, with the input loads split across the kk halves, so the input tile is reused across more output rows. The variant is enabled by default through a new bit in the WINO4 option when CoutP is divisible by 128 and Cin by 16, and it exits through the register epilogue. The trade is a narrower time tile, higher register and LDS pressure per block, and fewer blocks per launch. A small profiling script update and a block-rows query API are also added.

```diff
diff --git a/include/ttsamd.h b/include/ttsamd.h
--- a/include/ttsamd.h
+++ b/include/ttsamd.h
@@ -297,6 +297,7 @@
                              int32_t relu_out, int32_t mode, float div, float* y, float* packed, float* splitk_ws, int64_t splitk_floats,
                              void* stream);
 int32_t ttsamd_conv_last_launch(int32_t* route, int32_t* ksplit);
+int32_t ttsamd_conv_last_block_rows(void);
 int64_t ttsamd_convt_packed_floats(int32_t cin, int32_t cout, int32_t u);
 int32_t ttsamd_conv_transpose1d(const float* x, const float* w, const float* bias, const int64_t* lens, int32_t batch, int32_t cin,
                                 int32_t cout, int32_t u, int32_t lin, float in_slope, float* y, float* packed, void* stream);
diff --git a/profiles/launch_classes.py b/profiles/launch_classes.py
--- a/profiles/launch_classes.py
+++ b/profiles/launch_classes.py
@@ -3,34 +3,79 @@
 import sys
 from collections import defaultdict
 
+PAT = re.compile(r'conv1d_wino4_f32<(\d+), (\d+), (\d+), (\d+), (\d+), (\d+)(?:, (\d+))?>')
 
-def classes(path):
-    d = defaultdict(lambda: [0, 0])
-    other = 0
+
+def launches(path):
+    out, other = [], 0
     with open(path) as f:
         for r in csv.DictReader(f):
             dur = int(r['End_Timestamp']) - int(r['Start_Timestamp'])
-            m = re.search(r'conv1d_wino4_f32<(\d+), (\d+), (\d+), (\d+), (\d+), (\d+)>', r['Kernel_Name'])
+            m = PAT.search(r['Kernel_Name'])
             if not m:
                 other += dur
                 continue
-            k, noct, nst, epi, lp, pt = map(int, m.groups())
-            key = (pt, k, lp, 'residual' if epi == 3 else 'plain', int(r['Grid_Size_X']) // int(r['Workgroup_Size_X']))
-            d[key][0] += 1
-            d[key][1] += dur
-    return d, other
+            k, noct, nst, epi, lp, pt = map(int, m.groups()[:6])
+            rows = 32 * int(m.group(7) or 2)
+            blocks = int(r['Grid_Size_X']) // int(r['Workgroup_Size_X'])
+            out.append((int(r['Start_Timestamp']), (pt, k, lp, 'residual' if epi == 3 else 'plain', blocks), rows, dur))
+    out.sort(key=lambda t: t[0])
+    return out, other
 
 
-a, oa = classes(sys.argv[1])
-b, ob = classes(sys.argv[2])
-print(f'{"groups":>6} {"k":>3} {"window":>7} {"epilogue":>9} {"blocks":>7} {"calls":>6} {"us parent":>10} {"us tree":>9} {"ratio":>6}')
+def mfma_util(path):
+    d = defaultdict(lambda: [None, 0.0, 0.0])
+    for r in csv.DictReader(open(path)):
+        m = PAT.search(r['Kernel_Name'])
+        if not m:
+            continue
+        k, noct, nst, epi, lp, pt = map(int, m.groups()[:6])
+        e = d[int(r['Dispatch_Id'])]
+        e[0] = ((pt, k, lp, 'residual' if epi == 3 else 'plain', int(r['Grid_Size']) // int(r['Workgroup_Size'])), 32 * int(m.group(7) or 2))
+        if r['Counter_Name'] == 'SQ_VALU_MFMA_BUSY_CYCLES':
+            e[1] += float(r['Counter_Value'])
+        elif r['Counter_Name'] == 'SQ_BUSY_CU_CYCLES':
+            e[2] += float(r['Counter_Value'])
+    return [(d[i][0][0], d[i][0][1], d[i][1], d[i][2]) for i in sorted(d)]
+
+
+def paired(la, lb):
+    t = defaultdict(lambda: [0, 0, 0, 0])
+    if len(la) == len(lb) and all(x[1][:4] == y[1][:4] for x, y in zip(la, lb)):
+        for x, y in zip(la, lb):
+            e = t[x[1] + (y[2],)]
+            e[0] += 1; e[1] += 1; e[2] += x[3]; e[3] += y[3]
+        return t, True
+    for x in la:
+        e = t[x[1] + (x[2],)]
+        e[0] += 1; e[2] += x[3]
+    for y in lb:
+        e = t[y[1] + (y[2],)]
+        e[1] += 1; e[3] += y[3]
+    return t, False
+
+
+a, oa = launches(sys.argv[1])
+b, ob = launches(sys.argv[2])
+t, ok = paired(a, b)
+u = None
+if len(sys.argv) >= 5:
+    pa, pb = mfma_util(sys.argv[3]), mfma_util(sys.argv[4])
+    u, _ = paired([(0, x[0], x[1], x[2]) for x in pa], [(0, x[0], x[1], x[2]) for x in pb])
+    ucu, _ = paired([(0, x[0], x[1], x[3]) for x in pa], [(0, x[0], x[1], x[3]) for x in pb])
+print('launches paired by ordinal (the class of a pair carries the rows of the tree\'s launch)' if ok else
+      'launch lists differ: classes of each build by its own kernel names')
+print(f'{"groups":>6} {"k":>3} {"window":>7} {"epilogue":>9} {"blocks":>7} {"rows":>5} {"calls":>6} {"us parent":>10} {"us tree":>9} {"ratio":>6}'
+      + ('  MfmaUtil % parent -> tree' if u else ''))
 ta = tb = 0
-for key in sorted(set(a) | set(b), key=lambda t: (-t[0], t[1], t[2], t[3], t[4])):
-    ca, da = a.get(key, (0, 0))
-    cb, db = b.get(key, (0, 0))
+for key in sorted(t, key=lambda c: (-c[0], c[1], c[2], c[3], c[4], c[5])):
+    ca, cb, da, db = t[key]
     ta += da
     tb += db
     ua, ub = (da / ca / 1e3 if ca else float('nan')), (db / cb / 1e3 if cb else float('nan'))
-    print(f'{"seven" if key[0] == 7 else "six":>6} {key[1]:3d} {"vector" if key[2] == 1 else "strip":>7} {key[3]:>9} {key[4]:7d} {max(ca, cb):6d} '
-          f'{ua:10.1f} {ub:9.1f} {ub / ua:6.3f}')
+    line = (f'{"seven" if key[0] == 7 else "six":>6} {key[1]:3d} {"vector" if key[2] == 1 else "strip":>7} {key[3]:>9} {key[4]:7d} {key[5]:5d} '
+            f'{max(ca, cb):6d} {ua:10.1f} {ub:9.1f} {ub / ua:6.3f}')
+    if u and key in u and ucu[key][2] and ucu[key][3]:
+        line += f'  {100 * u[key][2] / (4 * ucu[key][2]):5.1f} -> {100 * u[key][3] / (4 * ucu[key][3]):5.1f}'
+    print(line)
 print(f'sum over the conv1d_wino4_f32 launches: {ta / 1e6:.2f} -> {tb / 1e6:.2f} ms; every other kernel: {oa / 1e6:.2f} -> {ob / 1e6:.2f} ms (whole trace)')
diff --git a/tts-arabic-pytorch_amd/csrc/api.hip b/tts-arabic-pytorch_amd/csrc/api.hip
--- a/tts-arabic-pytorch_amd/csrc/api.hip
+++ b/tts-arabic-pytorch_amd/csrc/api.hip
@@ -225,6 +225,7 @@
     const long long x = std::strtoll(v, &end, d.kind == 1 ? 16 : 10);
     if (!(errno == 0 && end != v && *end == '\0' && x >= d.lo && x <= d.hi)) return false;
     if (&d == &kOpts[OPT_WINO4] && (((x & 32) && !(x & 2)) || ((x & 64) && !(x & 4)))) return false;
+    if (&d == &kOpts[OPT_WINO4] && (x & 128) && !(x & 96)) return false;
     return true;
 }
 void opt_init() {
@@ -856,6 +857,8 @@
     last_conv_launch(route, ksplit);
     return 0;
 }
+
+int32_t ttsamd_conv_last_block_rows(void) { return last_conv_block_rows(); }
 
 int64_t ttsamd_convt_packed_floats(int32_t cin, int32_t cout, int32_t u) {
     if (cin < 1 || cout < 1 || u < 1) return 0;
diff --git a/tts-arabic-pytorch_amd/csrc/common.hpp b/tts-arabic-pytorch_amd/csrc/common.hpp
--- a/tts-arabic-pytorch_amd/csrc/common.hpp
+++ b/tts-arabic-pytorch_amd/csrc/common.hpp
@@ -53,7 +53,7 @@
     X(HIFIGAN_STREAMS, 0, 0, 1)    \
     X(WINO, 0, 0, 1)                                              \
     X(WINO2, 0, 0, 31)             \
-    X(WINO4, 0, 0, 127)            \
+    X(WINO4, 0, 0, 255)            \
     X(FUSED_PAIR, 0, 0, 1)                   \
     X(FUSED2, 0, 0, 1)                                           \
     X(FUSED2_MASK, 1, 0, 0x1ff)               \
@@ -152,6 +152,8 @@
 int32_t launch_conv(const ConvParams& p, hipStream_t stream);
 void note_conv_launch(int32_t route, int32_t ksplit);
 void last_conv_launch(int32_t* route, int32_t* ksplit);
+void note_conv_block_rows(int32_t rows);
+int32_t last_conv_block_rows();
 bool convt_supported(const ConvParams& p);
 int32_t launch_convt(const ConvParams& p, hipStream_t stream);
 int32_t launch_upsampler(ConvParams& p, const float* x, const float* w, const void* w_bf16, const float* bias, float* y, int cin, int cout,
@@ -186,7 +188,7 @@
 void pack_wino2_weight(const float* w, int cout, int cin, int k, float* out);
 int wino4_groups(int k);
 int wino44_groups(int k);
-constexpr int kWino4Default = 127;
+constexpr int kWino4Default = 255;
 bool wino44_wanted(const ConvParams& p);
 int wino4_block_outputs(int dil);
 int wino4_ksplit(const ConvParams& p);
diff --git a/tts-arabic-pytorch_amd/csrc/conv_mfma.hip b/tts-arabic-pytorch_amd/csrc/conv_mfma.hip
--- a/tts-arabic-pytorch_amd/csrc/conv_mfma.hip
+++ b/tts-arabic-pytorch_amd/csrc/conv_mfma.hip
@@ -511,9 +511,11 @@
     *yp = v;
 }
 
-static thread_local int32_t t_last_route = -1, t_last_ksplit = 0;
-void note_conv_launch(int32_t route, int32_t ksplit) { t_last_route = route; t_last_ksplit = ksplit; }
+static thread_local int32_t t_last_route = -1, t_last_ksplit = 0, t_last_rows = 0;
+void note_conv_launch(int32_t route, int32_t ksplit) { t_last_route = route; t_last_ksplit = ksplit; t_last_rows = 0; }
 void last_conv_launch(int32_t* route, int32_t* ksplit) { *route = t_last_route; *ksplit = t_last_ksplit; }
+void note_conv_block_rows(int32_t rows) { t_last_rows = rows; }
+int32_t last_conv_block_rows() { return t_last_rows; }
 
 int32_t launch_splitk_reduce(const ConvParams& q, hipStream_t stream) {
     dim3 rg((q.Nout + 255) / 256, q.Cout, q.batch);
diff --git a/tts-arabic-pytorch_amd/csrc/conv_wino4.hip b/tts-arabic-pytorch_amd/csrc/conv_wino4.hip
--- a/tts-arabic-pytorch_amd/csrc/conv_wino4.hip
+++ b/tts-arabic-pytorch_amd/csrc/conv_wino4.hip
@@ -12,11 +12,13 @@
 typedef float w4_f32x4 __attribute__((ext_vector_type(4)));
 typedef float w4_f32x2 __attribute__((ext_vector_type(2)));
 
-template <int K, int NOCT_, int NSTAGE_, int PT_ = 6, int LP_ = 1>
+template <int K, int NOCT_, int NSTAGE_, int PT_ = 6, int LP_ = 1, int WM_ = 2>
 struct Wino4Geo {
     static constexpr bool PT7 = PT_ == 7;
     static_assert(PT_ == 6 || (PT7 && (K == 7 || K == 11)), "seven-point groups: k = 7 / 11");
-    static constexpr int WM = 2, WN = 2;
+    static_assert(WM_ == 2 || (WM_ == 4 && PT7 && LP_ == 1 && NOCT_ == 1), "128-row blocks: seven-point groups, dilation 1");
+    static constexpr int WM = WM_, WN = 4 / WM_;
+    static constexpr int NOL = WM_ == 4 ? 2 : 1;
     static constexpr int NSF = K == 1 ? 0 : (K == 3 ? 1 : (K == 7 ? 2 : (PT7 ? 3 : 4)));
     static constexpr int NL = (!PT7 && (K == 7 || K == 1)) ? 1 : 0;
     static constexpr int GSF = PT7 ? 7 : 6;
@@ -35,7 +37,7 @@
     static constexpr int CO_BLK = WM * 32;
     static constexpr int NTUP = WN * 32;
     static constexpr int NT_BLK = 4 * NTUP;
-    static constexpr int BUF4 = NOCT * 2 * NGPM * NTUP;
+    static constexpr int BUF4 = NOL * NOCT * 2 * NGPM * NTUP;
     static constexpr int PF = 4;
     static constexpr int NM = 4;
     __host__ __device__ static constexpr int glo(int ph) { return NPH == 1 ? 0 : PH0 * ph; }
@@ -61,7 +63,7 @@
     static_assert(mhi(NPH - 1) == NPOS - 1 && mlo(0) == 0, "the groups cover the window and nothing past it");
     __host__ __device__ static constexpr int npos(int ph) { return mhi(ph) - mlo(ph) + 1; }
     static constexpr int NPOSP = npos(0) > npos(NPH - 1) ? npos(0) : npos(NPH - 1);
-    __host__ __device__ static constexpr int ngap(int ph) { return NOCT * ngp(ph) * NM; }
+    __host__ __device__ static constexpr int ngap(int ph) { return NOL * NOCT * ngp(ph) * NM; }
     __host__ __device__ static constexpr int sph(int ph) { return ((ph - (NSTAGE - 1)) % NPH + NPH) % NPH; }
     __host__ __device__ static constexpr int sgap(int ph) { return ngap(sph(ph)); }
     static constexpr int JSF = 10;
@@ -93,8 +95,9 @@
     __host__ __device__ static constexpr int tw0t(int ph) { return tr_r0(ph) + nrj(ph) + 1; }
     __host__ __device__ static constexpr int wst(int ph) { return (sgap(ph) - tw0t(ph)) / nwj(ph); }
     static_assert(LP_ != 2 || (wst(0) >= 1 && wst(NPH - 1) >= 1), "one write job per gap at most (strip path)");
-    static constexpr int QX = WSHARE ? 0 : (NOCT * ngq(0)) % PF;
-    static constexpr int QMAIN = NOCT * ngq(0) - QX;
+    static constexpr int NGS = NOL * NOCT * ngq(0);
+    static constexpr int QX = WSHARE ? 0 : NGS % PF;
+    static constexpr int QMAIN = NGS - QX;
     static_assert(QX == 0 || (NPH == 1 && NOCT == 1 && QMAIN >= 2 * PF), "extra queue slots: one phase, one octet");
     static_assert((WSHARE ? NOCT : NOCT * ngq(NPH - 1)) % PF == 0 || QX != 0, "queue slots line up across steps");
     static_assert((size_t)NSTAGE * BUF4 * 16 + (LP_ == 2 ? RAW_BYTES : 0) <= 80 * 1024, "two blocks per CU");
@@ -103,11 +106,13 @@
 
 __device__ __host__ constexpr int wino4_tile(int d, int ntup) { return (4 * ntup / (4 * d)) * (4 * d); }
 
-template <int K, int NOCT_, int NSTAGE_, int EPI, int LP, int PT = 6>
+template <int K, int NOCT_, int NSTAGE_, int EPI, int LP, int PT = 6, int WM_ = 2>
 __global__ __launch_bounds__(256, kConvMinWaves) void conv1d_wino4_f32(const ConvParams p) {
     extern __shared__ __attribute__((aligned(16))) float4 smem4[];
-    using G = Wino4Geo<K, NOCT_, NSTAGE_, PT, LP>;
+    using G = Wino4Geo<K, NOCT_, NSTAGE_, PT, LP, WM_>;
     constexpr bool PT7 = G::PT7;
+    constexpr bool W4 = WM_ == 4;
+    constexpr int NOL = G::NOL;
     constexpr int WN = G::WN, NSF = G::NSF, NOCT = G::NOCT, NSTAGE = G::NSTAGE, NPL = G::NPL, NGPM = G::NGPM;
     constexpr int CO_BLK = G::CO_BLK, NTUP = G::NTUP, NT_BLK = G::NT_BLK, PF = G::PF;
     constexpr int NPH = G::NPH, NPOSP = G::NPOSP, NM = G::NM;
@@ -142,7 +147,7 @@
     if (p.lens_in) in_len = min(in_len, (int)p.lens_in[b] * p.len_in_mul);
 
     const int x_cs = p.x_cs, CoutP = p.CoutP;
-    const int chunks_all = p.Cin / (8 * NOCT);
+    const int chunks_all = p.Cin / (8 * NOCT * NOL);
     const int c_beg = (int)((int64_t)ks * chunks_all / p.ksplit), n_chunks = (int)((int64_t)(ks + 1) * chunks_all / p.ksplit);
     const int n_groups = (p.Cin / 8) * G::NGW;
     const float* __restrict__ xb = p.x + (int64_t)b * p.x_bs;
@@ -150,6 +155,7 @@
 
     constexpr bool REG = EPI >= 3, RES = EPI == 3;
     static_assert(!REG || (LP == 1 && K != 1), "register epilogue: dilation 1, k = 3 / 7 / 11");
+    static_assert(!W4 || REG, "128-row blocks leave through the register epilogue");
     float ep_bias = 0.f;
     if constexpr (!REG) {
         if (tid < CO_BLK && p.bias) ep_bias = p.bias[min(co_blk0 + tid, p.Cout - 1)];
@@ -201,7 +207,7 @@
     w4_f32x2 ta[NOCT], tb[NOCT];
     w4_f32x2 tf[PT7 ? 5 : 1], te[PT7 ? 4 : 1], td[PT7 ? 3 : 1], th[PT7 ? 2 : 1];
     const int spe = min(lane, ntup_eff - 1);
-    const int xw0 = (q0 + 4 * lane) * 4;
+    const int xw0 = (q0 + 4 * (W4 ? l31 : lane)) * 4;
     constexpr int pad_c = (K - 1) / 2;
     const int ch_off = (4 * sh + skk) * x_cs;
 
@@ -212,6 +218,14 @@
     {                                                                                                \
         TTS_VJOB_IDX(PH, J)                                                                          \
         const bfo_i4 xrs_ = bfo_rsrc(xb + ((XSO) + ch_off + (8 * ol_ + 2 * pp_) * x_cs), (unsigned)in_len * 4u);     \
+        if constexpr (W4) {    \
+                                               \
+            const bfo_i4 xr1_ = bfo_rsrc(xb + ((XSO) + ch_off + (8 + 2 * pp_) * x_cs), (unsigned)in_len * 4u);       \
+            bfo_i4 ld_;                                                                              \
+            if (kk == 0) ld_ = bfo_ld16(xrs_, xw0 + 16 * (G::vlo(PH) + vi_), 0, 0);                  \
+            else ld_ = bfo_ld16(xr1_, xw0 + 16 * (G::vlo(PH) + vi_), 0, 0);                          \
+            sv[ol_][pp_][vi_] = __builtin_bit_cast(w4_f32x4, ld_);                                   \
+        } else                                                                                       \
         sv[ol_][pp_][vi_] = __builtin_bit_cast(w4_f32x4, bfo_ld16(xrs_, xw0 + 16 * (G::vlo(PH) + vi_), 0, 0));      \
     }
 #define TTS_VACT_JOB(PH, A)                                                                          \
@@ -324,14 +338,14 @@
     }
 
     const float4* sB = smem4 + kk * NGPM * NTUP + wn * 32 + l31;
-    w4_f32x2* sW = reinterpret_cast<w4_f32x2*>(smem4 + skk * NGPM * NTUP + lane) + sh;
+    w4_f32x2* sW = reinterpret_cast<w4_f32x2*>(smem4 + skk * NGPM * NTUP + (W4 ? kk * 2 * NGPM * NTUP + l31 : lane)) + sh;
     float4 bq[2];
 
     {
 #pragma unroll
         for (int st = 0; st < NSTAGE - 1; ++st) {
             const int ph = st % NPH;
-            const int xso = min(c_beg + st / NPH, n_chunks - 1) * 8 * NOCT * x_cs;
+            const int xso = min(c_beg + st / NPH, n_chunks - 1) * 8 * NOCT * NOL * x_cs;
             if constexpr (D1) {
 #pragma unroll
                 for (int J = 0; J < G::nljv(ph); ++J) TTS_VLOAD_JOB(ph, J, xso)
@@ -362,24 +376,24 @@
             const bool peel = (LAST) && ph == NPH - 1;                                                                                                       \
                                       \
             const int tph = (ph + NSTAGE - 1) % NPH;                                                                                                         \
-            const int xso = min((C) + (ph + NSTAGE - 1) / NPH, n_chunks - 1) * 8 * NOCT * x_cs;                                                                \
+            const int xso = min((C) + (ph + NSTAGE - 1) / NPH, n_chunks - 1) * 8 * NOCT * NOL * x_cs;                                                              \
             const int stage_next = (stage + 1 == NSTAGE) ? 0 : stage + 1;                                                                                    \
             const int stage_fill = (stage == 0) ? NSTAGE - 1 : stage - 1;                                                                                    \
             w4_f32x2* wr = sW + 2 * stage_fill * G::BUF4;                                                                                                    \
             const float4* rd = sB + stage * G::BUF4;                                                                                                         \
             const int sn = ((C) + 1 < n_chunks || ph + 1 < NPH) ? stage_next : stage;                                                                          \
         _Pragma("unroll")                                                                                                                                    \
-            for (int gs = 0; gs < NOCT * G::ngq(ph); ++gs) {                                                                                                 \
+            for (int gs = 0; gs < NOL * NOCT * G::ngq(ph); ++gs) {                                                                                           \
                 const int ol = gs / G::ngq(ph), gl = gs % G::ngq(ph);                                                                                        \
                 const int qs = G::WSHARE ? ol % PF : ((G::QX && gs >= G::QMAIN) ? PF + gs - G::QMAIN : gs % PF);                                             \
                 const w4_f32x4 a4 = aq[qs];                                                                                                                  \
                                           \
                 if constexpr (G::QX != 0) {                                                                                                                  \
                                             \
-                    const int nx = gs < G::QMAIN - PF ? gs + PF : (gs < G::QMAIN ? G::NGQ + gs + PF - G::QMAIN : G::NGQ + gs);                               \
-                    if (!peel || nx < G::NGQ) aq[qs] = __builtin_bit_cast(w4_f32x4, bfo_ld16(wrs, wv, min(wso + nx * wstep, wlast), 0));                     \
-                    if (gs == G::NGQ - 1) wso += G::NGQ * wstep;                                                                                             \
-                } else if ((!G::WSHARE || gl == G::ngq(ph) - 1) && (!peel || gs + PF < NOCT * G::ngq(ph))) {                                                 \
+                    const int nx = gs < G::QMAIN - PF ? gs + PF : (gs < G::QMAIN ? G::NGS + gs + PF - G::QMAIN : G::NGS + gs);                               \
+                    if (!peel || nx < G::NGS) aq[qs] = __builtin_bit_cast(w4_f32x4, bfo_ld16(wrs, wv, min(wso + nx * wstep, wlast), 0));                     \
+                    if (gs == G::NGS - 1) wso += G::NGS * wstep;                                                                                             \
+                } else if ((!G::WSHARE || gl == G::ngq(ph) - 1) && (!peel || gs + PF < NOL * NOCT * G::ngq(ph))) {                                           \
                     aq[qs] = __builtin_bit_cast(w4_f32x4, bfo_ld16(wrs, wv, wso, 0));                                                                        \
                     wso = min(wso + wstep, wlast);                                                                                                           \
                 }                                                                                                                                            \
@@ -388,7 +402,7 @@
                 const int cur = r & 1, nxt = cur ^ 1;                                                                                                        \
                 const int plane = G::plane(G::glo(ph) + gl);                                                                                                 \
                                                     \
-                if (r + 1 < NOCT * G::ngp(ph)) bq[nxt] = rd[(((r + 1) / G::ngp(ph)) * 2 * NGPM + (r + 1) % G::ngp(ph)) * NTUP];                              \
+                if (r + 1 < NOL * NOCT * G::ngp(ph)) bq[nxt] = rd[(((r + 1) / G::ngp(ph)) * 2 * NGPM + (r + 1) % G::ngp(ph)) * NTUP];                              \
                 else if (NSTAGE >= 3 && !peel) bq[nxt] = sB[sn * G::BUF4];        \
                 __builtin_amdgcn_sched_barrier(0);                                                                                                           \
                 const float bv[4] = {bq[cur].x, bq[cur].y, bq[cur].z, bq[cur].w};                                                                            \
@@ -419,7 +433,7 @@
             if (peel) break;                                                                                                                                 \
             __syncthreads();                                                                                                                                 \
             if (NSTAGE < 3) bq[0] = sB[sn * G::BUF4];                                      \
-            else if ((NOCT * G::ngp(ph)) % 2 != 0) bq[0] = bq[1];                                                                                            \
+            else if ((NOL * NOCT * G::ngp(ph)) % 2 != 0) bq[0] = bq[1];                                                                                            \
             stage = stage_next;                                                                                                                              \
         }
     for (int c = c_beg; c < n_chunks - (REG ? 1 : 0); ++c) {
@@ -513,7 +527,7 @@
     }
     constexpr int LDS_F = CO_BLK * NT_BLK + CO_BLK;
     constexpr int LPR = NT_BLK / 4;
-    static_assert(LPR == 64, "one wave instruction per row");
+    static_assert(REG || LPR == 64, "one wave instruction per row");
     float* ep = reinterpret_cast<float*>(smem4);
     float* epb = ep + LDS_F - CO_BLK;
     const float* __restrict__ rb = p.res ? p.res + (int64_t)b * p.r_bs : nullptr;
@@ -630,9 +644,9 @@
     }
 }
 
-template <int K, int NOCT, int NSTAGE, int EPI, int LP, int PT = 6>
+template <int K, int NOCT, int NSTAGE, int EPI, int LP, int PT = 6, int WM = 2>
 static int32_t launch_wino4_epi(const ConvParams& p, hipStream_t stream) {
-    using G = Wino4Geo<K, NOCT, NSTAGE, PT, LP>;
+    using G = Wino4Geo<K, NOCT, NSTAGE, PT, LP, WM>;
     constexpr size_t ring = (size_t)G::NSTAGE * G::BUF4 * sizeof(float4);
     constexpr size_t epi = ((size_t)G::CO_BLK * G::NT_BLK + G::CO_BLK) * sizeof(float);
     constexpr size_t strip = LP == 2 ? (size_t)G::RAW_BYTES : 0;
@@ -640,12 +654,13 @@
     static_assert(lds <= 80 * 1024, "two blocks per CU");
     static_assert(EPI < 3 || lds == ring, "register epilogue: the ring sets the LDS size");
     static std::atomic<uint64_t> lds_done{0};
-    const auto kern = conv1d_wino4_f32<K, NOCT, NSTAGE, EPI, LP, PT>;
+    const auto kern = conv1d_wino4_f32<K, NOCT, NSTAGE, EPI, LP, PT, WM>;
     TTS_CHECK_HIP(lds_opt_in((const void*)kern, (int)lds, lds_done));
     const int nt = wino4_tile(p.dil, G::NTUP);
     ConvParams q = p;
     q.ksplit = EPI == 0 ? wino4_ksplit(p) : 1;
     note_conv_launch(PT == 7 ? 4 : 3, q.ksplit);
+    note_conv_block_rows(G::CO_BLK);
     const int64_t n_tiles = (int64_t)((p.Nout + nt - 1) / nt) * p.batch;
     const int64_t n_blocks = ((n_tiles + 7) / 8) * 8 * (p.CoutP / G::CO_BLK) * q.ksplit;
     TTS_REQUIRE(n_blocks < ((int64_t)1 << 31), "wino4: %lld blocks", (long long)n_blocks);
@@ -671,6 +686,10 @@
 static int32_t launch_wino44_cfg(const ConvParams& p, hipStream_t stream) {
     if (p.dil == 1) {
         if (wino4_ksplit(p) != 1) return launch_wino4_epi<K, 1, 2, 0, 1, 7>(p, stream);
+        if (((int)opt_int(OPT_WINO4, kWino4Default) & 128) && p.CoutP % 128 == 0 && p.Cin % 16 == 0) {
+            if (p.res != nullptr) return launch_wino4_epi<K, 1, 2, 3, 1, 7, 4>(p, stream);
+            return launch_wino4_epi<K, 1, 2, 4, 1, 7, 4>(p, stream);
+        }
         if (p.res != nullptr) return launch_wino4_epi<K, 1, 2, 3, 1, 7>(p, stream);
         return launch_wino4_epi<K, 1, 2, 4, 1, 7>(p, stream);
     }
diff --git a/tts-arabic-pytorch_amd/ttsamd/engine.py b/tts-arabic-pytorch_amd/ttsamd/engine.py
--- a/tts-arabic-pytorch_amd/ttsamd/engine.py
+++ b/tts-arabic-pytorch_amd/ttsamd/engine.py
@@ -554,6 +554,10 @@
     return route.value, ksplit.value
 
 
+def last_conv_block_rows():
+    return int(L.load().ttsamd_conv_last_block_rows())
+
+
 def conv_transpose1d(x, w, bias=None, lens=None, in_slope=1.0, y=None):
     lib = _require_gpu()
     x = x.contiguous().float()
diff --git a/tts-arabic-pytorch_amd/ttsamd/lib.py b/tts-arabic-pytorch_amd/ttsamd/lib.py
--- a/tts-arabic-pytorch_amd/ttsamd/lib.py
+++ b/tts-arabic-pytorch_amd/ttsamd/lib.py
@@ -160,6 +160,7 @@
     'ttsamd_conv1d_ex': (_I32, [_P, _P, _P, _P, _P, _I32, _I32, _I32, _I32, _I32, _I32, _F, _I32, _I32, _F, _P, _P, _P]),
     'ttsamd_conv1d_splitk': (_I32, [_P, _P, _P, _P, _P, _I32, _I32, _I32, _I32, _I32, _I32, _F, _I32, _I32, _F, _P, _P, _P, _I64, _P]),
     'ttsamd_conv_last_launch': (_I32, [C.POINTER(_I32), C.POINTER(_I32)]),
+    'ttsamd_conv_last_block_rows': (_I32, []),
     'ttsamd_convt_packed_floats': (_I64, [_I32, _I32, _I32]),
     'ttsamd_conv_transpose1d': (_I32, [_P, _P, _P, _P, _I32, _I32, _I32, _I32, _I32, _F, _P, _P, _P]),
     'ttsamd_resblock_pair_packed_floats': (_I64, [_I32, _I32, _I32]),
```

After: 76.95 million (median of 6 runs). Within noise of the previous version (+0.2%).
